# arnold117/PrimeKG-RGCN-LinkPrediction

Hardware: AMD Instinct MI355X
Metric: edges/sec per RGCN layer (fwd+bwd), PrimeKG 30.9k nodes/849k edges/3 rels (higher is better)
Workload: dtype f32; 1 GPU; C2: PrimeKG-shaped synthetic graph, 30926 nodes / 849456 edge columns / 3 relations, encoder 64->128->128, 2 layers fwd+bwd, full graph per step, dropout 0; parallelism=1 GPU, launch=hipGraph replay

## Files before the change

include/rgcn_hip.h:

```cpp
#ifndef RGCN_HIP_H
#define RGCN_HIP_H

#include <stddef.h>
#include <stdint.h>

#ifdef __cplusplus
extern "C" {
#endif

#define RGCN_ABI_VERSION 38

enum {
  RGCN_OK = 0,
  RGCN_ERR_ARG = -1,
  RGCN_ERR_RANGE = -2,
  RGCN_ERR_HIP = -3,
  RGCN_ERR_UNSUPPORTED = -4,
  RGCN_ERR_WORKSPACE = -5,
  RGCN_ERR_ALIGN = -6
};

int rgcn_abi_version(void);
const char* rgcn_strerror(int code);

typedef struct rgcn_graph rgcn_graph;

int rgcn_graph_create(const int64_t* edge_index, const int64_t* edge_type, int64_t num_edges,
                      int64_t num_nodes, int64_t num_relations, void* stream,
                      rgcn_graph** out);
int rgcn_graph_create_bipartite(const int64_t* key_node, const int64_t* other_node,
                                const int64_t* edge_type, int64_t num_edges, int64_t num_key_nodes,
                                int64_t num_other_nodes, int64_t num_relations,
                                const float* edge_weight, void* stream, rgcn_graph** out);
void rgcn_graph_destroy(rgcn_graph* g);

int64_t rgcn_graph_num_edges(const rgcn_graph* g);
int64_t rgcn_graph_num_nodes(const rgcn_graph* g);
int64_t rgcn_graph_num_relations(const rgcn_graph* g);
float rgcn_graph_weight_bound(const rgcn_graph* g, int transposed);
int rgcn_graph_num_levels(const rgcn_graph* g, int transposed);

const uint32_t* rgcn_graph_tile_mask(const rgcn_graph* g, int transposed, int64_t* num_row_tiles);

int rgcn_graph_arrays(const rgcn_graph* g, int transposed, const int32_t** rowptr,
                      const int32_t** col, const int64_t** perm, const float** val);
int rgcn_graph_export(const rgcn_graph* g, int transposed, int32_t* rowptr, int32_t* col,
                      int64_t* perm, float* val, void* stream);

int rgcn_graph_import(int64_t num_edges, int64_t num_nodes, int64_t num_relations,
                      const int32_t* rowptr, const int32_t* col, const int64_t* perm, const float* cnt,
                      const int32_t* rowptr_t, const int32_t* col_t, const int64_t* perm_t,
                      const float* w_t, void* stream, rgcn_graph** out);

typedef struct rgcn_slab_job {
  const float* slab;
  const float* bias_part;
  int32_t splits, K1, Kc, N;
  float* grad_weight;
  float* grad_root;
  float* grad_bias;
} rgcn_slab_job;

#define RGCN_AMAX_FLOATS 2048
size_t rgcn_aggregate_workspace_bytes(const rgcn_graph* g, int transposed, int64_t d);
int rgcn_aggregate_deferrable(const rgcn_graph* g, int transposed, int64_t d);
int rgcn_aggregate(const rgcn_graph* g, int transposed, const float* x, int64_t d, float* agg,
                   void* workspace, size_t workspace_bytes, void* stream);
int rgcn_aggregate_ex(const rgcn_graph* g, int transposed, const void* x, int x_f16, int64_t d, float* agg,
                      void* workspace, size_t workspace_bytes, int first_level, int last_level ,
                      const rgcn_slab_job* job , float* amax , void* stream);

int rgcn_transform_fwd(const float* agg, const float* x, const float* weight, const float* root,
                       const float* bias, int relu, const uint32_t* tile_mask, int64_t num_nodes,
                       int64_t num_relations, int64_t d_in, int64_t d_out, float* out, void* stream);

size_t rgcn_transform_fwd_f16_workspace_bytes(int64_t num_relations, int64_t d_in, int64_t d_out);
int rgcn_transform_fwd_f16(const float* agg, const float* x, const float* weight, const float* root,
                           const float* bias, int relu, const uint32_t* tile_mask, int64_t num_nodes,
                           int64_t num_relations, int64_t d_in, int64_t d_out, float* out,
                           void* workspace, size_t workspace_bytes, void* stream);

int rgcn_transform_bwd_input(const float* gagg, const float* g, const float* weight,
                             const float* root, const float* relu_mask, const uint32_t* tile_mask,
                             int64_t num_nodes, int64_t num_relations, int64_t d_in, int64_t d_out,
                             float* grad_x, void* stream);

size_t rgcn_transform_bwd_params_workspace_bytes(int64_t num_nodes, int64_t num_relations,
                                                 int64_t d_in, int64_t d_out);
int rgcn_transform_bwd_params(const float* agg, const float* x, const float* g,
                              const uint32_t* tile_mask, int64_t num_nodes, int64_t num_relations,
                              int64_t d_in, int64_t d_out, float* grad_weight, float* grad_root,
                              float* grad_bias, void* workspace, size_t workspace_bytes, void* stream);

int rgcn_transform_bwd_params_begin(const float* agg, const float* x, const float* g,
                                    const uint32_t* tile_mask, int64_t num_nodes, int64_t num_relations,
                                    int64_t d_in, int64_t d_out, float* grad_weight, float* grad_root,
                                    float* grad_bias, void* workspace, size_t workspace_bytes, void* stream,
                                    rgcn_slab_job* job);
int rgcn_slab_reduce(const rgcn_slab_job* job, void* stream);

int rgcn_absmax(const float* x, int64_t n, float* out, float* zero_buffers, int zero_count, void* stream);
int rgcn_absmax_multi(int count, const float* const* tensors, const int64_t* numels, float* const* outs,
                      float* zero_buffers, int zero_count, void* stream);
size_t rgcn_weights_split_bytes(int64_t num_relations, int64_t d_in, int64_t d_out);
int rgcn_weights_split_pack(const float* weight, const float* root, int64_t num_relations, int64_t d_in,
                            int64_t d_out, void* packed, size_t packed_bytes, void* stream);
int rgcn_weights_split_pack_multi(int count, const float* const* weights, const float* const* roots,
                                  const int64_t* num_relations, const int64_t* d_in, const int64_t* d_out,
                                  const float* const* w_amax, const float* const* r_amax, void* const* packed,
                                  const size_t* packed_bytes, float* zero_buffers, int zero_count, void* stream);
int rgcn_absmax_pack(const float* x, int64_t numel, float* x_amax, float* zero_buffers, int zero_count, int count,
                     const float* const* weights, const float* const* roots, const int64_t* num_relations,
                     const int64_t* d_in, const int64_t* d_out, void* const* packed, const size_t* packed_bytes,
                     void* stream);
size_t rgcn_transform_split_workspace_bytes(int64_t num_relations, int64_t d_in, int64_t d_out);
int rgcn_transform_fwd_split(const float* agg, const float* x, const float* weight, const float* root,
// ... 145 lines not shown
```

primekg_rgcn_linkprediction_amd/_lib.py:

```python
from __future__ import annotations

import ctypes
import os
from ctypes import c_double, c_float, POINTER, c_char_p, c_int, c_int64, c_size_t, c_void_p

import torch

ABI_VERSION = 38
LIB_NAME = "librgcn_hip.so"
LIB_PATH = os.path.join(os.path.dirname(os.path.abspath(__file__)), LIB_NAME)

RGCN_OK = 0
RGCN_ERR_ARG = -1
RGCN_ERR_RANGE = -2
RGCN_ERR_HIP = -3
RGCN_ERR_UNSUPPORTED = -4
RGCN_ERR_WORKSPACE = -5
RGCN_ERR_ALIGN = -6

_P = c_void_p
_I64 = c_int64

class SlabJob(ctypes.Structure):
    _fields_ = [("slab", c_void_p), ("bias_part", c_void_p), ("splits", ctypes.c_int32), ("K1", ctypes.c_int32),
# ... 131 lines not shown
    "rgcn_kmeans_update": (c_int, [_P, _I64, _I64, _P, _I64, _I64,
                                   _P, _P, _P, _P, _P, _P, c_float, _P, c_size_t, _P]),
    "rgcn_kmeans_inertia": (c_int, [_P, _I64, _I64, _P, _I64, _I64, _P, _P, _P, c_size_t, _P]),
    "rgcn_silhouette_workspace_bytes": (c_size_t, [_I64, _I64, _I64, _I64]),
    "rgcn_silhouette_samples": (c_int, [_P, _P, _P, _P, _P, _P, _I64, _I64, _I64, _I64, _I64, _P, _P, _P, c_size_t, _P]),
}

TSNE_PROTOTYPES = {
    "rgcn_knn_refine": (c_int, [_P, _I64, _I64, _P, _I64, _P, _P, _P]),
    "rgcn_tsne_affinities": (c_int, [_P, _I64, _I64, c_double, _P, _P, _P]),
    "rgcn_tsne_workspace_bytes": (c_size_t, [_I64, _I64]),
    "rgcn_tsne_gradient": (c_int, [_P, _I64, _P, _P, _P, _I64, c_float, _I64, c_int,
                                   _P, _P, _P, _P, c_size_t, _P]),
    "rgcn_tsne_update": (c_int, [_P, _I64, c_float, c_float, c_float, _P, _P, _P, _P, _P, c_size_t, _P]),
}

NEIGHBORHOOD_PROTOTYPES = {
    "rgcn_neighborhood_max_nodes": (_I64, []),
    "rgcn_pair_neighborhood": (c_int, [_P, _P, _P, _P, _I64, _I64,
                                       _P, _P, _I64, c_int,
                                       _P, c_int, c_int,
                                       _P, _P, _P, _P, _P, _P, _P, _P]),
}

TRANSE_PROTOTYPES = {
    "rgcn_transe_step_workspace_bytes": (c_size_t, [_I64, _I64, _I64]),
    "rgcn_transe_step": (c_int, [_P, _I64, _P, _I64, _I64,
                                 _P, _P, _P, _I64, c_float, c_float,
                                 _P, _P, _P, _P, c_size_t, _P]),
}

RESAMPLE_PROTOTYPES = {
    "rgcn_resample_weights": (c_int, [_I64, _I64, _I64, _P, _P]),
    "rgcn_resample_curves": (c_int, [_P, _P, _P, _I64, _I64, _I64, _I64, _I64,
                                     _P, _P, _P, _P, _P, _P, _P]),
    "rgcn_resample_ranks": (c_int, [_P, _P, _I64, _P, c_int, _I64, _I64, _I64,
                                    _P, _P, _P, _P, _P]),
}
RESAMPLE_TILE = 1024
RESAMPLE_MAX_SAMPLES = 1 << 28
RESAMPLE_MAX_REPLICATES = 65535
RESAMPLE_MAX_K = 8

COMPLEX_PROTOTYPES = {
    "complex_fwd": (c_int, [_P, _P, _I64, _P, _P, _I64, _P, _P, _I64, _I64, _I64, _P, _P]),
    "complex_bce_fwd": (c_int, [_P, _P, _I64, _P, _P, _I64, _P, _P, _I64, _P, _I64, _I64, _P, _P, _P]),
    "complex_bwd_workspace_bytes": (c_size_t, [_I64, _I64, _I64]),
    "complex_bwd": (c_int, [_P, _P, _P, _I64, _P, _P, _I64, _P, _P, _I64, _I64, _I64, _P, _P, _P, _P, c_size_t, c_int, _P]),
    "complex_bce_bwd": (c_int, [_P, _P, _P, _P, _P, _I64, _P, _P, _I64, _P, _P, _I64, _I64, _I64, _P, _P, _P, _P,
                                c_size_t, c_int, _P]),
    "rgcn_complex_query": (c_int, [c_int, _P, _P, _I64, _P, _P, _I64, _I64, _I64, _P, _P]),
}

_lib = None


class RGCNLibraryError(RuntimeError):
    """The HIP library is missing / unloadable / of the wrong ABI."""


def load() -> ctypes.CDLL:
    global _lib
    if _lib is not None:
        return _lib
    if not os.path.exists(LIB_PATH):
        raise RGCNLibraryError(
            f"{LIB_PATH} not found: build it with `python -c 'import __graft_entry__ as g; "
            f"g.build()'` (or `make -C primekg_rgcn_linkprediction_amd/csrc`). There is no "
            f"CPU/PyTorch fallback for the R-GCN path.")
    try:
        lib = ctypes.CDLL(LIB_PATH, mode=ctypes.RTLD_GLOBAL)
    except OSError as exc:
        raise RGCNLibraryError(f"cannot load {LIB_PATH}: {exc}") from exc
    for name, (restype, argtypes) in list(PROTOTYPES.items()) + list(SAMPLING_PROTOTYPES.items()) + list(PATHS_PROTOTYPES.items()) + list(CLUSTER_PROTOTYPES.items()) + list(TSNE_PROTOTYPES.items()) + list(NEIGHBORHOOD_PROTOTYPES.items()) + list(TRANSE_PROTOTYPES.items()) + list(RESAMPLE_PROTOTYPES.items()) + list(COMPLEX_PROTOTYPES.items()):
        try:
            fn = getattr(lib, name)
        except AttributeError as exc:
            raise RGCNLibraryError(f"{LIB_PATH} does not export {name}") from exc
        fn.restype = restype
        fn.argtypes = argtypes
    got = lib.rgcn_abi_version()
    if got != ABI_VERSION:
        raise RGCNLibraryError(f"{LIB_PATH} has ABI version {got}, host code expects {ABI_VERSION}")
    _lib = lib
    return lib


def available() -> bool:
    try:
        load()
        return True
    except RGCNLibraryError:
        return False


def strerror(code: int) -> str:
    return load().rgcn_strerror(code).decode()


def check(code: int, what: str) -> None:
    if code == RGCN_OK:
        return
    msg = f"{what}: {strerror(code)} (code {code})"
    if code == RGCN_ERR_RANGE:
        raise IndexError(msg)
    if code in (RGCN_ERR_ARG, RGCN_ERR_UNSUPPORTED):
        raise ValueError(msg)
    if code == RGCN_ERR_ALIGN:
        raise ValueError(f"{what}: a tensor's base address is not aligned: {strerror(code)} (code {code}). Every tensor "
                         f"torch allocates qualifies, and so do row slices of a table whose width is a multiple of 4; a "
                         f"view that starts some elements into a flat buffer does not - pass tensor.clone()")
    raise RuntimeError(msg)
```

primekg_rgcn_linkprediction_amd/conv.py:

```python
from __future__ import annotations

import math
from typing import Optional, Tuple, Union

import torch
import torch.nn as nn
from torch import Tensor

from . import ops


def _glorot(t: Optional[Tensor]) -> None:
    if t is not None:
        bound = math.sqrt(6.0 / (t.size(-2) + t.size(-1)))
        t.data.uniform_(-bound, bound)


def _table(x: Tensor, gather_dtype) -> Tensor:
    if gather_dtype in (None, torch.float32):
        return x
    ops.guard_torch_op("fp16 copy of the feature table")
    return x.to(gather_dtype)


# ... 5 lines not shown
        ctx.save_for_backward(comp, basis)
        return ops.basis_compose(comp, basis)

    @staticmethod
    def backward(ctx, gw: Tensor):
        comp, basis = ctx.saved_tensors
        return ops.basis_compose_bwd(gw.contiguous(), comp, basis, ctx.needs_input_grad[0], ctx.needs_input_grad[1])


class _Scales:

    def __init__(self, t: Tensor, slots: int = 2, layers=(), given=None):
        self._own, self._next, self.first = None, 0, None
        self.packed = [None] * len(layers)
        if ops.GEMM_PRECISION == "split":
            if given is not None:
                self.first = given[0]
                if slots > 1:
                    self._own = ops._empty(slots - 1, ops.AMAX_FLOATS, dtype=torch.float32, device=t.device)
                self.packed = ops.split_weights_many(list(layers), amax=list(given[1]), clear=self._own)
                return
            buf = ops._empty(slots, ops.AMAX_FLOATS, dtype=torch.float32, device=t.device)
            self.first, self._own = buf[0], buf[1:slots]
            if layers:
                self.packed = ops.absmax_and_split(t, self.first, self._own, list(layers))
            else:
                ops.absmax(t, self.first, self._own)

    def slot(self) -> Optional[Tensor]:
        if self._own is None:
            return None
        self._next += 1
        return self._own[self._next - 1]


import os as _os
_TRANSFORM_FIRST_RATIO = 2.0


def _fused_backward(graph, g, r, d_in, d_out, g_amax, packed, precision) -> bool:
    fused = _TRAIN_FUSED == "1" or (_TRAIN_FUSED == "auto" and g.size(0) * r * d_out * 4 >= _TRAIN_FUSED_MIN_BYTES)
    return (fused and precision is None and packed is not None and g_amax is not None and not graph.bipartite
            and ops.GEMM_PRECISION == "split" and ops.fused_bwd_supported(r, d_in, d_out))


def _from_packed(weight: Tensor, packed, precision) -> bool:
    return packed is not None and ops.GEMM_PRECISION == "split" and precision is None and weight.size(2) % 32 == 0


def _transform_first(graph: "ops.BucketedGraph", weight: Tensor, root: Optional[Tensor], packed, precision) -> bool:
    r, d_in, d_out = weight.shape
    ratio = _TRANSFORM_FIRST_RATIO if _from_packed(weight, packed, precision) else max(_TRANSFORM_FIRST_RATIO, 4.0)
    return d_out >= ratio * d_in and root is not None and not graph.bipartite


def _gagg_scale(graph: "ops.BucketedGraph", gagg_amax: Optional[Tensor], g_amax: Optional[Tensor]):
    if gagg_amax is not None:
        return (gagg_amax, g_amax), 1.0
    return (g_amax, g_amax), graph.weight_bound(True)


def _input_grad(graph: "ops.BucketedGraph", g: Tensor, weight: Tensor, root: Optional[Tensor],
                tail: Optional["ops.PendingParamGrads"] = None, g_amax: Optional[Tensor] = None,
                scales: Optional[_Scales] = None, packed: Optional["ops.SplitWeights"] = None,
                precision: Optional[str] = None, t_first: Optional[Tensor] = None, *,
                relu_mask: Optional[Tensor] = None, out_scale: float = 1.0, amax_out: Optional[Tensor] = None,
                lower=None):
    r, d_in, d_out = weight.shape
    extras = relu_mask is not None or amax_out is not None or out_scale != 1.0
    merged = (graph.merged_transposed()
              if not extras and _transform_first(graph, weight, root, packed, precision) else None)
    t = None
    if merged is not None:
        if t_first is None and _from_packed(weight, packed, precision):
            t_first = ops.transform_first(g.contiguous(), packed, g_amax)
        elif t_first is None:
            ops.guard_torch_op("weight concatenation of the transform-first input gradient")
            wcat = torch.cat([weight.reshape(r * d_in, d_out), root]).view(1, (r + 1) * d_in, d_out)
            t_first = ops.transform_bwd_input(g, g, wcat, None, amax=(g_amax, None), precision=precision)
        gx = ops.aggregate(merged, t_first.view(-1, d_in), tail=tail)
    else:
        gagg_amax = scales.slot() if scales is not None else None
        if _fused_backward(graph, g, r, d_in, d_out, g_amax, packed, precision):
            gx = ops.layer_bwd_input_fused(graph, g, packed, relu_mask, g_amax, amax_out=amax_out, tail=tail,
                                           inline_limit=_EVAL_INLINE_LIMIT, out_scale=out_scale, gagg_amax=gagg_amax)
        else:
            gagg = ops.aggregate(graph, g, transposed=True, tail=tail, amax_out=gagg_amax)
            amax, mul = _gagg_scale(graph, gagg_amax, g_amax)
            if (lower is not None and packed is not None and g_amax is not None
                    and _from_packed(lower[0], lower[2], precision) and _transform_first(graph, *lower, precision)
                    and ops.chain_supported(weight, lower[0])):
                gx, t = ops.transform_bwd_input_chain(gagg, g, weight, root, relu_mask, packed, lower[2], graph=graph,
                                                      amax=amax, amax_mul=mul, amax_out=amax_out, out_scale=out_scale)
            else:
                gx = ops.transform_bwd_input(gagg, g, weight, root, relu_mask=relu_mask, graph=graph, amax=amax,
                                             amax_mul=mul, amax_out=amax_out, packed=packed, precision=precision,
                                             out_scale=out_scale)
    return (gx, t) if lower is not None else gx


def _backward_scales(g: Tensor, layers: int) -> _Scales:
    return _Scales(g, slots=2 * layers)


def _deferred_params(graph: "ops.BucketedGraph", agg, x, g, x_amax, g_amax, has_root: bool, has_bias: bool, prec):
    return ops.transform_bwd_params(agg, x, g, graph.num_relations, want_root=has_root, want_bias=has_bias, graph=graph,
                                    defer=True, amax=(x_amax, x_amax, g_amax), precision=prec)


_TRAIN_FUSED = _os.environ.get("RGCN_TRAIN_FUSED", "auto")
_TRAIN_FUSED_MIN_BYTES = 256 << 20


def _defer_hubs(half: bool, packed, amax, k: int, n_out: int) -> bool:
    return (_DEFER_HUBS and not half and packed is not None and amax is not None and ops.GEMM_PRECISION == "split"
            and k in (64, 128) and n_out <= 128)


_DEFER_HUBS = True


def _train_fused(graph, n, r, d_in, d_out, half) -> bool:
    fused = _TRAIN_FUSED == "1" or (_TRAIN_FUSED == "auto" and n * r * d_in * 4 >= _TRAIN_FUSED_MIN_BYTES)
    return bool(fused and not half and not graph.weighted_shard and n == graph.num_other_nodes
                and ops.GEMM_PRECISION == "split" and ops.fused_supported(r, d_in, d_out))


def _layer_train_forward(graph: "ops.BucketedGraph", x: Tensor, gather_dtype, weight, root, bias, relu: bool,
                         half: bool, x_amax, amax_out, packed):
    n, r, d_in, d_out = x.size(0), graph.num_relations, x.size(1), weight.size(2)
    if (_train_fused(graph, n, r, d_in, d_out, half) and packed is not None and x_amax is not None):
        agg = ops._empty(n, r * d_in, dtype=torch.float32, device=x.device)
        out = ops.layer_fwd_fused(graph, x, packed, bias, relu, x_amax, amax_out, inline_limit=_EVAL_INLINE_LIMIT,
                                  agg_out=agg)
        return agg, out
    if _defer_hubs(half, packed, x_amax, d_in, d_out):
        agg, hubs = ops.aggregate_deferred(graph, x)
    else:
        agg, hubs = ops.aggregate(graph, _table(x, gather_dtype)), None
    out = ops.transform_fwd(agg, x, weight, root, bias, relu=relu, graph=graph, half=half, amax=(x_amax, x_amax),
                            amax_out=amax_out, packed=packed, hubs=hubs)
    return agg, out


def _packs(bufs, layers):
    return [ops.SplitWeights(b, w, root) if b is not None else None for b, (w, root) in zip(bufs, layers)]


def _conv_forward(x, weight, root, bias, *, graph, relu, gather_dtype, half):
    scales = _Scales(x, slots=1, layers=[(weight, root)])
    x_amax = scales.first
    packed = scales.packed[0]
    agg, out = _layer_train_forward(graph, x, gather_dtype, weight, root, bias, relu, half, x_amax, None,
                                    packed)
    return out, agg, x_amax, (packed.buf if packed is not None else None)


def _conv_backward(x, agg, weight, root, x_amax, pkbuf, g, *, graph, has_root, has_bias, need_x, need_p, prec):
    packed = _packs([pkbuf], [(weight, root)])[0]
    scales = _backward_scales(g, 1)
    pending = _deferred_params(graph, agg, x, g, x_amax, scales.first, has_root, has_bias, prec) if need_p else None
    gx = _input_grad(graph, g, weight, root, pending, scales.first, scales, packed, prec) if need_x else None
    if pending is None:
        return gx, None, None, None
    pending.finish()
    return (gx, *pending.grads)


_R_CONV_FORWARD = ops.Region("conv.forward", _conv_forward)
_R_CONV_BACKWARD = ops.Region("conv.backward", _conv_backward)


def _contiguous(*tensors):
    return tuple(t.contiguous() if t is not None else None for t in tensors)


def _bwd_precision(gather_dtype, half_backward: bool) -> Optional[str]:
    return "half" if (gather_dtype == torch.float16 and half_backward and ops.GEMM_PRECISION == "split") else None


class _RGCNConvFunction(torch.autograd.Function):

    @staticmethod
    def forward(ctx, x: Tensor, weight: Tensor, root: Optional[Tensor], bias: Optional[Tensor],
                graph: ops.BucketedGraph, relu: bool = False, gather_dtype=None, half_backward: bool = False) -> Tensor:
        x, weight, root, bias = _contiguous(x, weight, root, bias)
        ctx.bwd_precision = _bwd_precision(gather_dtype, half_backward)
        key = (tuple(x.shape), tuple(weight.shape), root is not None, bias is not None, gather_dtype, bool(relu),
               _policy_key())
        out, agg, x_amax, pkbuf = _R_CONV_FORWARD.run(graph, key, (x, weight, root, bias),
                                                      dict(graph=graph, relu=relu, gather_dtype=gather_dtype,
                                                           half=gather_dtype == torch.float16), want={0})
        ctx.graph, ctx.relu, ctx.key = graph, relu, key
        ctx.has_root, ctx.has_bias = root is not None, bias is not None
        ctx.save_for_backward(x, weight, root, out if relu else None)
        ctx.kept = (agg, x_amax, pkbuf)
        return out

    @staticmethod
    def backward(ctx, g: Tensor):
        x, weight, root, out = ctx.saved_tensors
        agg, x_amax, pkbuf = ctx.kept
        if ctx.relu:
            g = g * (out > 0)
        g = g.contiguous()
        need_x, need_w, need_root, need_bias = ctx.needs_input_grad[:4]
        need_p = bool(need_w or (need_root and ctx.has_root) or (need_bias and ctx.has_bias))
        static = dict(graph=ctx.graph, has_root=ctx.has_root, has_bias=ctx.has_bias, need_x=bool(need_x), need_p=need_p,
                      prec=ctx.bwd_precision)
        gx, gw, groot, gbias = _R_CONV_BACKWARD.run(ctx.graph, (ctx.key, bool(need_x), need_p, ctx.bwd_precision),
                                                    (x, agg, weight, root, x_amax, pkbuf, g), static,
                                                    want={0, 1, 2, 3})
        return gx, gw, groot, gbias, None, None, None, None


def _enc2_layer1(x, w1, root1, b1, w2, root2, xa=None, w1a=None, r1a=None, w2a=None, r2a=None, *, graph, gather_dtype, half):
    given = (xa, [(w1a, r1a), (w2a, r2a)]) if xa is not None else None
    scales = _Scales(x, layers=[(w1, root1), (w2, root2)], given=given)
    x_amax, h_amax = scales.first, scales.slot()
    pk1, pk2 = scales.packed
    agg1, h = _layer_train_forward(graph, x, gather_dtype, w1, root1, b1, True, half, x_amax, h_amax, pk1)
    return h, agg1, x_amax, h_amax, (pk1.buf if pk1 is not None else None), (pk2.buf if pk2 is not None else None)


def _enc2_layer2(h, w2, root2, b2, h_amax, pk2buf, *, graph, gather_dtype, half):
    pk2 = _packs([pk2buf], [(w2, root2)])[0]
    agg2, out = _layer_train_forward(graph, h, gather_dtype, w2, root2, b2, False, half, h_amax, None, pk2)
    return out, agg2


def _enc2_forward(x, w1, root1, b1, w2, root2, b2, xa=None, w1a=None, r1a=None, w2a=None, r2a=None, *, graph, gather_dtype,
                  half):
    h, agg1, x_amax, h_amax, pk1buf, pk2buf = _enc2_layer1(x, w1, root1, b1, w2, root2, xa, w1a, r1a, w2a, r2a, graph=graph,
                                                           gather_dtype=gather_dtype, half=half)
    out, agg2 = _enc2_layer2(h, w2, root2, b2, h_amax, pk2buf, graph=graph, gather_dtype=gather_dtype, half=half)
    return out, h, agg1, agg2, x_amax, h_amax, pk1buf, pk2buf


def _enc2_backward(x, agg1, h, agg2, w1, root1, w2, root2, x_amax, h_amax, pk1buf, pk2buf, g, *, graph, flags, p,
                   prec, need_x):
    has_root1, has_b1, has_root2, has_b2 = flags
    pk1, pk2 = _packs([pk1buf, pk2buf], [(w1, root1), (w2, root2)])
    scales = _backward_scales(g, 2)
    g_amax, gz_amax = scales.first, scales.slot()
    red2 = _deferred_params(graph, agg2, h, g, h_amax, g_amax, has_root2, has_b2, prec)
    gz = _input_grad(graph, g, w2, root2, red2, g_amax, scales, pk2, prec, relu_mask=h,
                     out_scale=1.0 / (1.0 - p) if p > 0 else 1.0, amax_out=gz_amax,
                     lower=(w1, root1, pk1) if need_x else None)
    gz, t_first = gz if need_x else (gz, None)
    red1 = _deferred_params(graph, agg1, x, gz, x_amax, gz_amax, has_root1, has_b1, prec)
    gx = _input_grad(graph, gz, w1, root1, red1, gz_amax, scales, pk1, prec, t_first) if need_x else None
    red2.finish()
    red1.finish()
    return (gx, *red1.grads, *red2.grads)


_R_LAYER1 = ops.Region("encoder2.layer1", _enc2_layer1)
_R_LAYER2 = ops.Region("encoder2.layer2", _enc2_layer2)
_R_FORWARD = ops.Region("encoder2.forward", _enc2_forward)
_R_BACKWARD = ops.Region("encoder2.backward", _enc2_backward)


def _policy_key():
    return (_TRAIN_FUSED, _DEFER_HUBS, _TRANSFORM_FIRST_RATIO, _EVAL_INLINE_LIMIT, _TRAIN_FUSED_MIN_BYTES)


def _enc2_train_forward(graph, params, gather_dtype, half_backward: bool, hints, p: float = 0.0):
    x, w1, root1, b1, w2, root2, b2 = params = _contiguous(*params)
    hinted = hints is not None and ops.GEMM_PRECISION == "split"
    hint_list = list(hints) if hinted else []
    key = (tuple(x.shape), tuple(w1.shape), tuple(w2.shape), root1 is not None, b1 is not None, root2 is not None,
           b2 is not None, gather_dtype, hinted, _policy_key())
    static = dict(graph=graph, gather_dtype=gather_dtype, half=gather_dtype == torch.float16)
    if p > 0:
        h, agg1, x_amax, h_amax, pk1buf, pk2buf = _R_LAYER1.run(graph, key, [x, w1, root1, b1, w2, root2] + hint_list,
                                                                static, want={0, 3})
        h = torch.native_dropout(h, p, True)[0]
        h_amax = ops.materialize(h_amax) * (1.0 / (1.0 - p)) if h_amax is not None else None
        out, agg2 = _R_LAYER2.run(graph, key, (h, w2, root2, b2, h_amax, pk2buf), static, want={0})
    else:
        out, h, agg1, agg2, x_amax, h_amax, pk1buf, pk2buf = _R_FORWARD.run(graph, key, list(params) + hint_list, static,
                                                                            want={0})
    flags = (root1 is not None, b1 is not None, root2 is not None, b2 is not None)
    kept = (agg1, h, agg2, x_amax, h_amax, pk1buf, pk2buf)
    return out, params, (graph, key, flags, p, _bwd_precision(gather_dtype, half_backward), kept)


def _enc2_train_backward(state, inputs, g: Tensor, need_x: bool):
    graph, key, flags, p, prec, (agg1, h, agg2, x_amax, h_amax, pk1buf, pk2buf) = state
    x, w1, root1, w2, root2 = inputs
    return _R_BACKWARD.run(graph, (key, p, need_x, prec),
                           (x, agg1, h, agg2, w1, root1, w2, root2, x_amax, h_amax, pk1buf, pk2buf, g.contiguous()),
                           dict(graph=graph, flags=flags, p=p, prec=prec, need_x=need_x), want={0, 1, 2, 3, 4, 5, 6})


class _Encoder2Function(torch.autograd.Function):

    @staticmethod
    def forward(ctx, x, w1, root1, b1, w2, root2, b2, graph, gather_dtype=None, p: float = 0.0,
                half_backward: bool = False, hints=None):
        out, (x, w1, root1, _, w2, root2, _), ctx.state = _enc2_train_forward(
            graph, (x, w1, root1, b1, w2, root2, b2), gather_dtype, half_backward, hints, p)
        ctx.save_for_backward(x, w1, root1, w2, root2)
        return out

    @staticmethod
    def backward(ctx, g):
        grads = _enc2_train_backward(ctx.state, ctx.saved_tensors, g, bool(ctx.needs_input_grad[0]))
        return (*grads, None, None, None, None, None)


_EVAL_BLOCK_BYTES = 1 << 30


_EVAL_FUSED = _os.environ.get("RGCN_EVAL_FUSED", "auto")


# ... 210 lines not shown
```

primekg_rgcn_linkprediction_amd/csrc/rgcn_aggregate.hip:

```cpp
#include <algorithm>
#include <cstdlib>
#include <type_traits>

#include <hip/hip_fp16.h>

#include "rgcn_common.h"
#include "rgcn_slab_reduce.h"
#include "rgcn_hub_finish.h"

namespace {

constexpr int kThreads = 256;
constexpr int kUnroll = RGCN_HEAD;
#ifndef RGCN_REDUCE_UNROLL
#define RGCN_REDUCE_UNROLL 16
#endif
#ifndef RGCN_ZERO_ROWS
#define RGCN_ZERO_ROWS 64
#endif

__device__ inline float4 f4zero() { return make_float4(0.f, 0.f, 0.f, 0.f); }
__device__ inline float f4amax(const float4& a) { return fmaxf(fmaxf(fabsf(a.x), fabsf(a.y)), fmaxf(fabsf(a.z), fabsf(a.w))); }

__device__ inline void f4add(float4& a, const float4& b) { a.x += b.x; a.y += b.y; a.z += b.z; a.w += b.w; }
// ... 254 lines not shown
      for (int u = 0; u < kUnroll; ++u) {
        v[u] = make_uint4(0u, 0u, 0u, 0u);
        if (idx[u] >= 0) v[u] = *reinterpret_cast<const uint4*>(src + (size_t)idx[u] * d + c8);
      }
#pragma unroll
      for (int u = 0; u < kUnroll; ++u) {
        const int en = e + kUnroll + u;
        const bool ok = en < it.end;
        idx_n[u] = ok ? col[en] : -1;
        wt_n[u] = (WEIGHTED && ok) ? w[en] : 0.f;
      }
      accumulate(v, wt);
    }
  }
  if (has_packs) {
    red[2 * threadIdx.x] = make_float4(acc[0], acc[1], acc[2], acc[3]);
    red[2 * threadIdx.x + 1] = make_float4(acc[4], acc[5], acc[6], acc[7]);
    __syncthreads();
    if (it.flags & (RGCN_ITEM_MEMBER | RGCN_ITEM_SKIP)) return;
    const int followers = (it.flags >> RGCN_ITEM_FOLLOW_SHIFT) & (RGCN_PACK - 1);
    for (int f = 1; f <= followers; ++f) {
      const float4 a = red[2 * (threadIdx.x + f * G)], b = red[2 * (threadIdx.x + f * G) + 1];
      acc[0] += a.x; acc[1] += a.y; acc[2] += a.z; acc[3] += a.w;
      acc[4] += b.x; acc[5] += b.y; acc[6] += b.z; acc[7] += b.w;
    }
  }
  if (!live) return;
  float* out = (it.flags & RGCN_ITEM_FINAL) ? agg : partial;
  if ((it.flags & RGCN_ITEM_FINAL) && cnt) {
    const float c = cnt[it.dst];
#pragma unroll
    for (int k = 0; k < 8; ++k) acc[k] /= c;
  }
  float4* o4 = reinterpret_cast<float4*>(out + (size_t)it.dst * d + c8);
  o4[0] = make_float4(acc[0], acc[1], acc[2], acc[3]);
  o4[1] = make_float4(acc[4], acc[5], acc[6], acc[7]);
}

template <int G>
__global__ __launch_bounds__(kThreads) void k_reduce_partials(const rgcn_item* __restrict__ items,
                                                              const float* __restrict__ cnt,
                                                              float* __restrict__ agg, float* partial, int d,
                                                              unsigned* __restrict__ amax_out) {
  __shared__ float4 red[kThreads];
  const float lmax = rgcn_reduce_item<G>(items[blockIdx.x], cnt, agg, partial, d, (int)blockIdx.y * G, red);
  if (amax_out && (int)threadIdx.x < G && (((int)threadIdx.x + (int)blockIdx.y * G) * 4 < d) &&
      (items[blockIdx.x].flags & RGCN_ITEM_FINAL))
    rgcn_amax_publish(amax_out, lmax);
}

template <int G>
void launch_level(const rgcn_csr* c, int level, bool weighted, const float* x, const float* cnt, float* agg,
                  float* partial, int d, hipStream_t stream, const rgcn_slab_job* tail = nullptr,
                  unsigned* amax_out = nullptr) {
  const int64_t nitems = c->num_items[level];
  if (nitems == 0) return;
  const unsigned gy = (unsigned)ceil_div64(d, 4 * G);
  if (level == 0) {
    const int64_t slots = kThreads / G;
    const int64_t walked = gy == 1 ? std::min(nitems, ceil_div64(nitems - c->empty_items0, slots) * slots) : nitems;
    const unsigned gather_blocks = (unsigned)ceil_div64(walked, slots);
    const unsigned zero_blocks = (unsigned)ceil_div64(nitems - walked, zero_rows<G>());
    const rgcn_slab_job job = tail ? *tail : rgcn_slab_job{};
    dim3 grid(gather_blocks + zero_blocks + (tail ? (unsigned)rgcn_slab_reduce_blocks(job) : 0u), gy);
    if (weighted)
      k_aggregate<G, true><<<grid, kThreads, 0, stream>>>(x, c->items[0], nitems, c->col, c->val, cnt, agg, partial, d,
                                                          c->head_col, c->head_w, job, (int)gather_blocks,
                                                          (int)zero_blocks, amax_out);
    else
      k_aggregate<G, false><<<grid, kThreads, 0, stream>>>(x, c->items[0], nitems, c->col, nullptr, cnt, agg, partial, d,
                                                           c->head_col, nullptr, job, (int)gather_blocks,
                                                           (int)zero_blocks, amax_out);
  } else {
    dim3 grid((unsigned)nitems, gy);
    k_reduce_partials<G><<<grid, kThreads, 0, stream>>>(c->items[level], cnt, agg, partial, d, amax_out);
  }
}

template <int G>
void launch_level0_h(const rgcn_csr* c, bool weighted, const __half* x, const float* cnt, float* agg, float* partial,
                     int d, hipStream_t stream) {
  const int64_t nitems = c->num_items[0];
  if (nitems == 0) return;
  dim3 grid((unsigned)ceil_div64(nitems, kThreads / G), (unsigned)ceil_div64(d, 8 * G));
  if (weighted)
    k_aggregate_h<G, true><<<grid, kThreads, 0, stream>>>(x, c->items[0], nitems, c->col, c->val, cnt, agg, partial, d,
                                                            c->head_col, c->head_w);
  else
    k_aggregate_h<G, false><<<grid, kThreads, 0, stream>>>(x, c->items[0], nitems, c->col, nullptr, cnt, agg, partial, d,
                                                             c->head_col, nullptr);
}

int aggregate_levels(const rgcn_graph* g, int transposed, int first, int last, const float* x, int64_t d,
                     float* agg, void* workspace, size_t workspace_bytes, void* stream_, bool half_in,
                     const rgcn_slab_job* tail, float* amax) {
  if (!g) return RGCN_ERR_ARG;
  const rgcn_csr* c = &g->dir[transposed ? 1 : 0];
  hipStream_t stream = (hipStream_t)stream_;
  if (!tail || !tail->slab) tail = nullptr;
  if (tail && (!tail->grad_weight || tail->splits <= 0 || tail->Kc <= 0 || tail->N <= 0 || (tail->N & 3)))
    return RGCN_ERR_ARG;
  if (tail && c->rowptr && c->n_key == 0) {
    RGCN_ALIGN_TRY(16, tail->slab, tail->bias_part, tail->grad_weight, tail->grad_root, tail->grad_bias);
    k_slab_reduce<<<(unsigned)rgcn_slab_reduce_blocks(*tail), 256, 0, stream>>>(*tail);
    RGCN_HIP_TRY(hipGetLastError());
    return RGCN_OK;
  }
  if (!agg || d <= 0 || (d & 3) || (half_in && (d & 7))) return RGCN_ERR_ARG;
  if (!c->rowptr) return RGCN_ERR_ARG;
  if (c->n_key == 0) return RGCN_OK;
  if (!x) return RGCN_ERR_ARG;
  if (d > (1 << 20)) return RGCN_ERR_UNSUPPORTED;
  if (first < 0 || last > c->num_levels || first > last) return RGCN_ERR_ARG;
  if (c->num_partials > 0 &&
      (!workspace || workspace_bytes < (size_t)c->num_partials * (size_t)d * sizeof(float)))
    return RGCN_ERR_WORKSPACE;
  float* partial = (float*)workspace;
  unsigned* amax_out = reinterpret_cast<unsigned*>(amax);
  if (amax && half_in) return RGCN_ERR_UNSUPPORTED;
  RGCN_ALIGN_TRY(16, x, agg, workspace);
  RGCN_ALIGN_TRY(4, amax);
  if (tail) RGCN_ALIGN_TRY(16, tail->slab, tail->bias_part, tail->grad_weight, tail->grad_root, tail->grad_bias);
  const float* cnt = c->weighted ? nullptr : c->val;
  const bool weighted = c->weighted;
  const int q = (int)(d / 4);
  const bool can_ride = !half_in && first == 0 && last > 0 && d <= 256 && c->num_items[0] > 0;
  if (tail && !can_ride) {
    k_slab_reduce<<<(unsigned)rgcn_slab_reduce_blocks(*tail), 256, 0, stream>>>(*tail);
    tail = nullptr;
  }
  for (int l = first; l < last; ++l) {
    const rgcn_slab_job* t0 = l == 0 ? tail : nullptr;
    if (l == 0 && half_in) {
      const __half* xh = reinterpret_cast<const __half*>(x);
      const int q8 = (int)(d / 8);
      if (q8 <= 1) launch_level0_h<1>(c, weighted, xh, cnt, agg, partial, (int)d, stream);
      else if (q8 <= 2) launch_level0_h<2>(c, weighted, xh, cnt, agg, partial, (int)d, stream);
      else if (q8 <= 4) launch_level0_h<4>(c, weighted, xh, cnt, agg, partial, (int)d, stream);
      else if (q8 <= 8) launch_level0_h<8>(c, weighted, xh, cnt, agg, partial, (int)d, stream);
      else if (q8 <= 16) launch_level0_h<16>(c, weighted, xh, cnt, agg, partial, (int)d, stream);
      else if (q8 <= 32) launch_level0_h<32>(c, weighted, xh, cnt, agg, partial, (int)d, stream);
      else launch_level0_h<64>(c, weighted, xh, cnt, agg, partial, (int)d, stream);
      continue;
    }
    if (q <= 1) launch_level<1>(c, l, weighted, x, cnt, agg, partial, (int)d, stream, t0, amax_out);
    else if (q <= 2) launch_level<2>(c, l, weighted, x, cnt, agg, partial, (int)d, stream, t0, amax_out);
    else if (q <= 4) launch_level<4>(c, l, weighted, x, cnt, agg, partial, (int)d, stream, t0, amax_out);
    else if (q <= 8) launch_level<8>(c, l, weighted, x, cnt, agg, partial, (int)d, stream, t0, amax_out);
    else if (q <= 16) launch_level<16>(c, l, weighted, x, cnt, agg, partial, (int)d, stream, t0, amax_out);
    else if (q <= 32) launch_level<32>(c, l, weighted, x, cnt, agg, partial, (int)d, stream, t0, amax_out);
    else launch_level<64>(c, l, weighted, x, cnt, agg, partial, (int)d, stream, t0, amax_out);
  }
  RGCN_HIP_TRY(hipGetLastError());
  return RGCN_OK;
}

}

extern "C" {

size_t rgcn_aggregate_workspace_bytes(const rgcn_graph* g, int transposed, int64_t d) {
  if (!g || d <= 0) return 0;
  return (size_t)g->dir[transposed ? 1 : 0].num_partials * (size_t)d * sizeof(float);
}

int rgcn_aggregate_ex(const rgcn_graph* g, int transposed, const void* x, int x_f16, int64_t d, float* agg,
                      void* workspace, size_t workspace_bytes, int first_level, int last_level, const rgcn_slab_job* job,
                      float* amax, void* stream) {
  if (!g) return RGCN_ERR_ARG;
  return aggregate_levels(g, transposed, first_level, last_level < 0 ? g->dir[transposed ? 1 : 0].num_levels : last_level,
                          reinterpret_cast<const float*>(x), d, agg, workspace, workspace_bytes, stream, x_f16 != 0, job,
                          amax);
}

int rgcn_aggregate(const rgcn_graph* g, int transposed, const float* x, int64_t d, float* agg,
                   void* workspace, size_t workspace_bytes, void* stream) {
  return rgcn_aggregate_ex(g, transposed, x, 0, d, agg, workspace, workspace_bytes, 0, -1, nullptr, nullptr, stream);
}

int rgcn_aggregate_deferrable(const rgcn_graph* g, int transposed, int64_t d) {
  if (!g) return 0;
  const rgcn_csr& c = g->dir[transposed ? 1 : 0];
  return (c.num_levels == 2 && c.fin_ptr && (d == 64 || d == 128 || d == 256)) ? 1 : 0;
}

}
```

primekg_rgcn_linkprediction_amd/csrc/rgcn_common.h:

```cpp
#pragma once
#include <hip/hip_runtime.h>
#include <stddef.h>
#include <stdint.h>
#include "../../include/rgcn_hip.h"
#include "rgcn_plan.h"

#define RGCN_HIP_TRY(expr)                       \
  do {                                           \
    hipError_t err__ = (expr);                   \
    if (err__ != hipSuccess) return RGCN_ERR_HIP; \
  } while (0)

template <class... P>
static inline bool rgcn_aligned(uintptr_t a, P... p) {
  uintptr_t bits = 0;
  ((bits |= (uintptr_t)(const void*)p), ...);
  return (bits & (a - 1)) == 0;
}
#define RGCN_ALIGN_TRY(a, ...)                                       \
  do {                                                               \
    if (!rgcn_aligned((a), __VA_ARGS__)) return RGCN_ERR_ALIGN;      \
  } while (0)

constexpr int kCUs = 256;
// ... 6 lines not shown
static inline rgcn_slicing rgcn_slice_tiles(int64_t tiles, int64_t want, int64_t cap) {
  const int64_t most = tiles < cap ? tiles : cap;
  want = want < most ? want : most;
  want = want > 1 ? want : 1;
  const int64_t per = (tiles + want - 1) / want;
  return {(int)per, (int)((tiles + per - 1) / per)};
}

template <class K>
static inline int raise_lds(K kernel, int bytes, bool (&raised)[64]) {
  int dev = 0;
  RGCN_HIP_TRY(hipGetDevice(&dev));
  if (dev < 0 || dev >= 64 || !raised[dev]) {
    RGCN_HIP_TRY(hipFuncSetAttribute(reinterpret_cast<const void*>(kernel), hipFuncAttributeMaxDynamicSharedMemorySize, bytes));
    if (dev >= 0 && dev < 64) raised[dev] = true;
  }
  return RGCN_OK;
}

static inline int rgcn_zero_param_grads(float* grad_weight, float* grad_root, float* grad_bias, int64_t R, int64_t d_in,
                                        int64_t d_out, hipStream_t stream) {
  RGCN_HIP_TRY(hipMemsetAsync(grad_weight, 0, (size_t)(R * d_in) * d_out * sizeof(float), stream));
  if (grad_root) RGCN_HIP_TRY(hipMemsetAsync(grad_root, 0, (size_t)d_in * d_out * sizeof(float), stream));
  if (grad_bias) RGCN_HIP_TRY(hipMemsetAsync(grad_bias, 0, (size_t)d_out * sizeof(float), stream));
  return RGCN_OK;
}

constexpr int RGCN_HEAD = 8;

struct rgcn_csr {
  int32_t* rowptr = nullptr;
  int32_t* col = nullptr;
  int64_t* perm = nullptr;
  float* val = nullptr;
  bool weighted = false;
  int64_t n_key = 0;
  int64_t n_other = 0;
  int num_levels = 0;
  int32_t empty_items0 = 0;
  rgcn_item* items[RGCN_MAX_LEVELS] = {};
  int64_t num_items[RGCN_MAX_LEVELS] = {};
  int64_t num_partials = 0;
  int32_t* head_col = nullptr;
  float* head_w = nullptr;
  uint32_t* tile_mask = nullptr;
  int64_t num_row_tiles = 0;
  int32_t* fin_ptr = nullptr;
  int64_t num_fin_tiles = 0;
  float weight_bound = 1.f;
};

static_assert(offsetof(rgcn_csr, items) == offsetof(rgcn_csr, num_levels) + 8, "empty_items0 sits behind num_levels");

struct rgcn_graph {
  int64_t E = 0, N = 0, R = 0;
  rgcn_csr dir[2];
};

__attribute__((visibility("hidden"))) int* rgcn_index_error_flag();

constexpr int RGCN_AMAX_SLOTS = 64, RGCN_AMAX_STRIDE = 32;
constexpr int RGCN_AMAX_HEADS = 256, RGCN_AMAX_HEAD_STRIDE = 8;
static_assert(RGCN_AMAX_SLOTS * RGCN_AMAX_STRIDE == RGCN_AMAX_FLOATS, "amax buffer layout (include/rgcn_hip.h)");
static_assert(RGCN_AMAX_HEADS * RGCN_AMAX_HEAD_STRIDE == RGCN_AMAX_FLOATS && RGCN_AMAX_STRIDE % RGCN_AMAX_HEAD_STRIDE == 0,
              "amax buffer layout");

#if defined(__HIPCC__)
__device__ inline int64_t clamp64(int64_t v, int64_t lo, int64_t hi) { return v < lo ? lo : (v > hi ? hi : v); }
__device__ inline int lane_int(int v, int src) { return __builtin_amdgcn_readfirstlane(__shfl(v, src)); }
__device__ inline float lane_float(float v, int src) { return __int_as_float(lane_int(__float_as_int(v), src)); }
__device__ inline int64_t lane_i64(int64_t v, int src) {
  const unsigned lo = (unsigned)lane_int((int)(unsigned)(v & 0xffffffffll), src);
  const int hi = lane_int((int)(v >> 32), src);
  return ((int64_t)hi << 32) | (int64_t)lo;
}
__device__ inline float rgcn_relu(float v) {
  const float r = fmaxf(v, 0.f);
  return v != v ? v : r;
}
extern "C" __device__ unsigned __ockl_wfred_max_u32(unsigned);
__device__ inline unsigned rgcn_amax_peek(const unsigned* __restrict__ amax) {
  return amax ? amax[(blockIdx.x & (RGCN_AMAX_SLOTS - 1)) * RGCN_AMAX_STRIDE] : 0u;
}
__device__ inline void rgcn_amax_publish(unsigned* __restrict__ amax, float lane_max, unsigned seen = 0u) {
  const unsigned m = __ockl_wfred_max_u32(__float_as_uint(fmaxf(lane_max, 0.f)));
  if (m <= seen) return;
  unsigned* slot = amax + (blockIdx.x & (RGCN_AMAX_SLOTS - 1)) * RGCN_AMAX_STRIDE;
  const unsigned long long act = __ballot(1);
  if ((int)(threadIdx.x & 63) == __ffsll((long long)act) - 1) atomicMax(slot, m);
}
__device__ inline float rgcn_amax_value(const float* __restrict__ amax, int lane) {
  float v[RGCN_AMAX_HEADS / 64];
#pragma unroll
  for (int j = 0; j < RGCN_AMAX_HEADS / 64; ++j) v[j] = amax[(lane + 64 * j) * RGCN_AMAX_HEAD_STRIDE];
  float m = v[0];
#pragma unroll
  for (int j = 1; j < RGCN_AMAX_HEADS / 64; ++j) m = fmaxf(m, v[j]);
#pragma unroll
  for (int o = 32; o > 0; o >>= 1) m = fmaxf(m, __shfl_xor(m, o));
  return m;
}
__device__ inline float rgcn_partials_max(const float* __restrict__ p, int count, int lane) {
  float v[4];
#pragma unroll
  for (int j = 0; j < 4; ++j) v[j] = (lane + 64 * j < count) ? p[lane + 64 * j] : 0.f;
  float m = fmaxf(fmaxf(v[0], v[1]), fmaxf(v[2], v[3]));
// ... 6 lines not shown
```

primekg_rgcn_linkprediction_amd/csrc/rgcn_graph.hip:

```cpp
#include <hipcub/hipcub.hpp>

#include <algorithm>
#include <cmath>
#include <new>
#include <vector>

#include "rgcn_common.h"

namespace {

constexpr int kThreads = 256;

__global__ void k_validate(const int64_t* __restrict__ key_node, const int64_t* __restrict__ other_node,
                           const int64_t* __restrict__ edge_type, int64_t E, int64_t n_key, int64_t n_other,
                           int64_t R, int* __restrict__ flag) {
  int64_t e = (int64_t)blockIdx.x * blockDim.x + threadIdx.x;
  if (e >= E) return;
  int64_t k = key_node[e], o = other_node[e], t = edge_type[e];
  if (k < 0 || k >= n_key || o < 0 || o >= n_other || t < 0 || t >= R) atomicOr(flag, 1);
}

__global__ void k_make_keys(const int64_t* __restrict__ key_node, const int64_t* __restrict__ edge_type,
                            int64_t E, int64_t R, uint32_t* __restrict__ keys, uint32_t* __restrict__ ids) {
  int64_t e = (int64_t)blockIdx.x * blockDim.x + threadIdx.x;
  if (e >= E) return;
  keys[e] = (uint32_t)(key_node[e] * R + edge_type[e]);
  ids[e] = (uint32_t)e;
}

__global__ void k_rowptr(const uint32_t* __restrict__ skeys, int64_t E, int64_t NR,
                         int32_t* __restrict__ rowptr) {
  int64_t e = (int64_t)blockIdx.x * blockDim.x + threadIdx.x;
  if (e > E) return;
  int64_t lo = (e == 0) ? 0 : (int64_t)skeys[e - 1] + 1;
  int64_t hi = (e == E) ? NR : (int64_t)skeys[e];
  for (int64_t k = lo; k <= hi; ++k) rowptr[k] = (int32_t)e;
}

__global__ void k_fill_edges(const int64_t* __restrict__ other_node, int64_t E,
                             const uint32_t* __restrict__ sids, int32_t* __restrict__ col,
                             int64_t* __restrict__ perm) {
  int64_t e = (int64_t)blockIdx.x * blockDim.x + threadIdx.x;
  if (e >= E) return;
  uint32_t p = sids[e];
  perm[e] = (int64_t)p;
  col[e] = (int32_t)other_node[p];
}

__global__ void k_counts(const int32_t* __restrict__ rowptr, int64_t NR, float* __restrict__ cnt) {
  int64_t s = (int64_t)blockIdx.x * blockDim.x + threadIdx.x;
  if (s >= NR) return;
  int deg = rowptr[s + 1] - rowptr[s];
  cnt[s] = (float)(deg < 1 ? 1 : deg);
}

__global__ void k_edge_weights(const uint32_t* __restrict__ skeys_t, const int32_t* __restrict__ col_t,
                               const float* __restrict__ cnt, int64_t E, int64_t R,
                               float* __restrict__ w) {
  int64_t e = (int64_t)blockIdx.x * blockDim.x + threadIdx.x;
  if (e >= E) return;
// ... 90 lines not shown
                    int64_t n_key, int64_t n_other, int64_t R, int slot, Scratch& sc, hipStream_t stream,
                    rgcn_csr* c) {
  const int64_t NR = n_key * R;
  c->n_key = n_key;
  c->n_other = n_other;
  RGCN_HIP_TRY(hipMalloc((void**)&c->rowptr, (NR + 1) * sizeof(int32_t)));
  if (E <= 0) {
    RGCN_HIP_TRY(hipMemsetAsync(c->rowptr, 0, (NR + 1) * sizeof(int32_t), stream));
    return RGCN_OK;
  }
  int end_bit = 1;
  while (end_bit < 32 && ((int64_t)1 << end_bit) < NR) ++end_bit;
  RGCN_HIP_TRY(hipMalloc((void**)&c->col, E * sizeof(int32_t)));
  RGCN_HIP_TRY(hipMalloc((void**)&c->perm, E * sizeof(int64_t)));
  k_make_keys<<<grid_for(E), kThreads, 0, stream>>>(key_node, edge_type, E, R, sc.keys, sc.ids);
  size_t tmp_bytes = 0;
  RGCN_HIP_TRY(hipcub::DeviceRadixSort::SortPairs(nullptr, tmp_bytes, sc.keys, sc.skeys[slot], sc.ids, sc.sids,
                                                   (int)E, 0, end_bit, stream));
  if (tmp_bytes > sc.sort_tmp_bytes) {
    RGCN_HIP_TRY(hipStreamSynchronize(stream));
    (void)hipFree(sc.sort_tmp);
    sc.sort_tmp = nullptr;
    RGCN_HIP_TRY(hipMalloc(&sc.sort_tmp, tmp_bytes + 256));
    sc.sort_tmp_bytes = tmp_bytes;
  }
  RGCN_HIP_TRY(hipcub::DeviceRadixSort::SortPairs(sc.sort_tmp, tmp_bytes, sc.keys, sc.skeys[slot], sc.ids, sc.sids,
                                                   (int)E, 0, end_bit, stream));
  k_rowptr<<<grid_for(E + 1), kThreads, 0, stream>>>(sc.skeys[slot], E, NR, c->rowptr);
  k_fill_edges<<<grid_for(E), kThreads, 0, stream>>>(other_node, E, sc.sids, c->col, c->perm);
  return RGCN_OK;
}

#define TRY_PLAN(expr) do { int rc__ = (expr); if (rc__ != RGCN_OK) return rc__; } while (0)

__global__ void k_item_heads(const rgcn_item* __restrict__ items, int64_t nitems, const int32_t* __restrict__ col,
                             const float* __restrict__ w, int32_t* __restrict__ head_col,
                             float* __restrict__ head_w) {
  const int64_t i = (int64_t)blockIdx.x * blockDim.x + threadIdx.x;
  if (i >= nitems * RGCN_HEAD) return;
  const rgcn_item it = items[i / RGCN_HEAD];
  const int e = it.begin + (int)(i % RGCN_HEAD);
  const bool ok = e < it.end;
  head_col[i] = ok ? col[e] : -1;
  if (head_w) head_w[i] = ok ? w[e] : 0.f;
}

int plan_structure(rgcn_csr* c, int64_t R, hipStream_t stream) {
  const int64_t NR = c->n_key * R;
  std::vector<int32_t> rp((size_t)NR + 1);
  RGCN_HIP_TRY(hipMemcpyAsync(rp.data(), c->rowptr, (NR + 1) * sizeof(int32_t), hipMemcpyDeviceToHost, stream));
  RGCN_HIP_TRY(hipStreamSynchronize(stream));
  if (R <= 32 && c->n_key > 0) {
    c->num_row_tiles = ceil_div64(c->n_key, 32);
    std::vector<uint32_t> mask((size_t)c->num_row_tiles, 0u);
    for (int64_t i = 0; i < c->n_key; ++i)
      for (int64_t r = 0; r < R; ++r)
        if (rp[i * R + r + 1] > rp[i * R + r]) mask[(size_t)(i >> 5)] |= 1u << r;
    RGCN_HIP_TRY(hipMalloc((void**)&c->tile_mask, mask.size() * sizeof(uint32_t)));
    RGCN_HIP_TRY(hipMemcpy(c->tile_mask, mask.data(), mask.size() * sizeof(uint32_t), hipMemcpyHostToDevice));
  }
  TRY_PLAN(build_plan(rp, NR, R, c));
  c->weight_bound = 1.f;
  if (c->weighted && NR > 0 && rp[(size_t)NR] > 0) {
    std::vector<float> w((size_t)rp[(size_t)NR]);
    RGCN_HIP_TRY(hipMemcpyAsync(w.data(), c->val, w.size() * sizeof(float), hipMemcpyDeviceToHost, stream));
    RGCN_HIP_TRY(hipStreamSynchronize(stream));
    double best = 0.0;
    for (int64_t s = 0; s < NR; ++s) {
      double sum = 0.0;
      for (int32_t e = rp[(size_t)s]; e < rp[(size_t)s + 1]; ++e) sum += std::fabs((double)w[(size_t)e]);
      best = std::max(best, sum);
    }
    c->weight_bound = (float)(best * (1.0 + 1e-6)) + 1e-30f;
  }
  const int64_t n0 = c->num_items[0];
  if (n0 > 0) {
    RGCN_HIP_TRY(hipMalloc((void**)&c->head_col, (size_t)n0 * RGCN_HEAD * sizeof(int32_t)));
    if (c->weighted) RGCN_HIP_TRY(hipMalloc((void**)&c->head_w, (size_t)n0 * RGCN_HEAD * sizeof(float)));
    k_item_heads<<<grid_for(n0 * RGCN_HEAD), kThreads, 0, stream>>>(c->items[0], n0, c->col,
                                                                   c->weighted ? c->val : nullptr, c->head_col,
                                                                   c->head_w);
    RGCN_HIP_TRY(hipGetLastError());
  }
  return RGCN_OK;
}

int mean_counts(rgcn_csr* c, int64_t R, hipStream_t stream) {
  const int64_t NR = c->n_key * R;
  RGCN_HIP_TRY(hipMalloc((void**)&c->val, std::max<int64_t>(NR, 1) * sizeof(float)));
  if (NR > 0) k_counts<<<grid_for(NR), kThreads, 0, stream>>>(c->rowptr, NR, c->val);
  c->weighted = false;
  return RGCN_OK;
}

#define TRY_RC(expr) do { int rc__ = (expr); if (rc__ != RGCN_OK) return rc__; } while (0)

int create_impl(const int64_t* edge_index, const int64_t* edge_type, int64_t E, int64_t N, int64_t R,
                hipStream_t stream, rgcn_graph* g) {
  g->E = E; g->N = N; g->R = R;
  const int64_t* src = edge_index;
  const int64_t* dst = edge_index + E;
  Scratch sc;
  TRY_RC(sc.alloc(E));
  TRY_RC(validate(dst, src, edge_type, E, N, N, R, sc, stream));
  TRY_RC(build_structure(dst, src, edge_type, E, N, N, R, 0, sc, stream, &g->dir[0]));
  TRY_RC(build_structure(src, dst, edge_type, E, N, N, R, 1, sc, stream, &g->dir[1]));
  TRY_RC(mean_counts(&g->dir[0], R, stream));
  g->dir[1].weighted = true;
  if (E > 0) {
    RGCN_HIP_TRY(hipMalloc((void**)&g->dir[1].val, E * sizeof(float)));
// ... 149 lines not shown
  if (num_nodes * num_relations > 0 && !cnt) return RGCN_ERR_ARG;
  if (num_edges > 0 && (!col || !perm || !col_t || !perm_t || !w_t)) return RGCN_ERR_ARG;
  if (too_big(num_nodes, num_nodes, num_relations, num_edges)) return RGCN_ERR_UNSUPPORTED;
  RGCN_ALIGN_TRY(8, perm, perm_t);
  RGCN_ALIGN_TRY(4, rowptr, col, cnt, rowptr_t, col_t, w_t);
  hipStream_t stream = (hipStream_t)stream_;
  rgcn_graph* g = new (std::nothrow) rgcn_graph();
  if (!g) return RGCN_ERR_HIP;
  g->E = num_edges; g->N = num_nodes; g->R = num_relations;
  int* flag = nullptr;
  int rc = hipMalloc((void**)&flag, sizeof(int)) == hipSuccess ? RGCN_OK : RGCN_ERR_HIP;
  if (rc == RGCN_OK)
    rc = import_csr(rowptr, col, perm, cnt, false, num_edges, num_nodes, num_relations, flag, stream, &g->dir[0]);
  if (rc == RGCN_OK)
    rc = import_csr(rowptr_t, col_t, perm_t, w_t, true, num_edges, num_nodes, num_relations, flag, stream,
                    &g->dir[1]);
  if (rc == RGCN_OK && hipStreamSynchronize(stream) != hipSuccess) rc = RGCN_ERR_HIP;
  (void)hipFree(flag);
  if (rc != RGCN_OK) {
    rgcn_graph_destroy(g);
    return rc;
  }
  *out = g;
  return RGCN_OK;
}

void rgcn_graph_destroy(rgcn_graph* g) {
  if (!g) return;
  free_csr(&g->dir[0]);
  free_csr(&g->dir[1]);
  delete g;
}

int64_t rgcn_graph_num_edges(const rgcn_graph* g) { return g ? g->E : -1; }
int64_t rgcn_graph_num_nodes(const rgcn_graph* g) { return g ? g->N : -1; }
int64_t rgcn_graph_num_relations(const rgcn_graph* g) { return g ? g->R : -1; }
float rgcn_graph_weight_bound(const rgcn_graph* g, int transposed) {
  if (!g) return 0.f;
  const rgcn_csr* c = &g->dir[transposed ? 1 : 0];
  return c->rowptr ? c->weight_bound : 0.f;
}

int rgcn_graph_num_levels(const rgcn_graph* g, int transposed) {
  return g ? g->dir[transposed ? 1 : 0].num_levels : -1;
}

const uint32_t* rgcn_graph_tile_mask(const rgcn_graph* g, int transposed, int64_t* num_row_tiles) {
  if (!g) return nullptr;
  const rgcn_csr* c = &g->dir[transposed ? 1 : 0];
  if (num_row_tiles) *num_row_tiles = c->num_row_tiles;
  return c->tile_mask;
}

int rgcn_graph_arrays(const rgcn_graph* g, int transposed, const int32_t** rowptr, const int32_t** col,
                      const int64_t** perm, const float** val) {
  if (!g) return RGCN_ERR_ARG;
  const rgcn_csr* c = &g->dir[transposed ? 1 : 0];
  if (rowptr) *rowptr = c->rowptr;
  if (col) *col = c->col;
  if (perm) *perm = c->perm;
  if (val) *val = c->val;
  return RGCN_OK;
}

int rgcn_graph_export(const rgcn_graph* g, int transposed, int32_t* rowptr, int32_t* col, int64_t* perm,
                      float* val, void* stream_) {
  if (!g) return RGCN_ERR_ARG;
  hipStream_t stream = (hipStream_t)stream_;
  const rgcn_csr* c = &g->dir[transposed ? 1 : 0];
  if (!c->rowptr) return RGCN_ERR_ARG;
  RGCN_ALIGN_TRY(8, perm);
  RGCN_ALIGN_TRY(4, rowptr, col, val);
  const size_t nr = (size_t)(c->n_key * g->R), e = (size_t)g->E;
  if (rowptr) RGCN_HIP_TRY(hipMemcpyAsync(rowptr, c->rowptr, (nr + 1) * sizeof(int32_t), hipMemcpyDeviceToDevice, stream));
  if (col && e) RGCN_HIP_TRY(hipMemcpyAsync(col, c->col, e * sizeof(int32_t), hipMemcpyDeviceToDevice, stream));
  if (perm && e) RGCN_HIP_TRY(hipMemcpyAsync(perm, c->perm, e * sizeof(int64_t), hipMemcpyDeviceToDevice, stream));
  const size_t nval = c->weighted ? e : nr;
  if (val && nval) RGCN_HIP_TRY(hipMemcpyAsync(val, c->val, nval * sizeof(float), hipMemcpyDeviceToDevice, stream));
  return RGCN_OK;
}

}
```

primekg_rgcn_linkprediction_amd/csrc/rgcn_transform_split.hip:

```cpp
#include <algorithm>
#include <cstdlib>
#include <type_traits>

#include <hip/hip_fp16.h>

#include "rgcn_common.h"
#include "rgcn_slab_reduce.h"
#include "rgcn_hub_finish.h"
#include "rgcn_split.h"
#include "rgcn_transform_host.h"

#ifdef RGCN_STAMPS
__device__ unsigned long long g_rgcn_stamps[8192 * 4];
#define RGCN_STAMP(i)                                                                                               \
  do {                                                                                                              \
    if (threadIdx.x == 0) g_rgcn_stamps[((blockIdx.y * gridDim.x + blockIdx.x) & 8191) * 4 + (i)] = __builtin_amdgcn_s_memrealtime(); \
  } while (0)
#else
#define RGCN_STAMP(i)
#endif

#include "rgcn_prep.h"


// ... 62 lines not shown
  }
  return q;
}
#define RGCN_AMAX_WAIT(a, b, c, younger)                                                                             \
  asm volatile("s_waitcnt vmcnt(%12)"                                                                                 \
               : "+v"(a.v[0]), "+v"(a.v[1]), "+v"(a.v[2]), "+v"(a.v[3]), "+v"(b.v[0]), "+v"(b.v[1]), "+v"(b.v[2]),     \
                 "+v"(b.v[3]), "+v"(c.v[0]), "+v"(c.v[1]), "+v"(c.v[2]), "+v"(c.v[3])                                  \
               : "n"(younger)                                                                                         \
               : "memory")
#define RGCN_AMAX_WAIT2(a, b, younger)                                                                                \
  asm volatile("s_waitcnt vmcnt(%8)"                                                                                  \
               : "+v"(a.v[0]), "+v"(a.v[1]), "+v"(a.v[2]), "+v"(a.v[3]), "+v"(b.v[0]), "+v"(b.v[1]), "+v"(b.v[2]),     \
                 "+v"(b.v[3])                                                                                         \
               : "n"(younger)                                                                                         \
               : "memory")
__device__ inline float amax_reduce(const amax_loads& q) {
  float m = fmaxf(fmaxf(q.v[0], q.v[1]), fmaxf(q.v[2], q.v[3]));
#pragma unroll
  for (int o = 32; o > 0; o >>= 1) m = fmaxf(m, __shfl_xor(m, o));
  return m;
}

constexpr int kPackThreads = 1024, kPackJobs = RGCN_PACK_JOBS;
using pack_job = rgcn_pack_job;
using pack_jobs = rgcn_pack_jobs;
__device__ inline void pack_body(const pack_job& J, float* red, int nblocks, int bid) {
  rgcn_pack_body<kPackThreads>(J, red, nblocks, bid);
}

__global__ __launch_bounds__(kPackThreads) void k_pack_split(const pack_jobs JJ, float* __restrict__ zero, int zero_count) {
  __shared__ float red[kPackThreads / 64];
  if (blockIdx.y == 0 && (int)threadIdx.x < zero_count)
    for (int h = (int)blockIdx.x; h < RGCN_AMAX_HEADS; h += (int)gridDim.x)
      zero[(size_t)threadIdx.x * RGCN_AMAX_FLOATS + h * RGCN_AMAX_HEAD_STRIDE] = 0.f;
  pack_body(JJ.j[blockIdx.y], red, (int)gridDim.x, (int)blockIdx.x);
}

struct hub_fin {
  const int32_t* ptr;
  const rgcn_item* items;
  const float* cnt;
  float* partial;
  int d, tiles;
};

struct nt_chain {
  const __half* Ch;
  const __half* Cl;
  const float* c_inv_scale;
  float* T;
  int N2;
};

template <int WM, int WN, int TN, int EPI, bool LO, bool CHAIN = false>
__global__ __launch_bounds__(64 * WM * WN) void k_gemm_nt_split(const float* __restrict__ A1, int K1,
                                                            const float* __restrict__ A2, int K2,
                                                            const __half* __restrict__ Bh,
                                                            const __half* __restrict__ Bl,
                                                            const float* __restrict__ b_inv_scale,
                                                            amax_ref amax1, float a1_mul, amax_ref amax2,
                                                            const float* __restrict__ bias,
                                                            const float* __restrict__ mask, float* __restrict__ C,
                                                            int M, int N, const uint32_t* __restrict__ tile_mask,
                                                            int kseg, unsigned* __restrict__ amax_out,
                                                            const hub_fin fin, float out_scale, const nt_chain chain) {
  static_assert(!CHAIN || (WM == 2 && WN == 2 && TN == 2 && LO), "the chained product is built for the 64 x 128 tile");
  constexpr int WAVES = WM * WN;
  constexpr int BM = 32 * WM, BN = 32 * TN * WN, NBUF = WM == 2 ? 3 : 4, D = NBUF - 1;
  constexpr int PARTS = LO ? 2 : 1;
  constexpr int A_BYTES = BM * BK * 4, B_BYTES = BN * BK * 2, BUF_BYTES = A_BYTES + PARTS * B_BYTES;
  constexpr int A_PW = BM / (8 * WAVES);
  constexpr int B_PW = BN / (16 * WAVES);
  constexpr int P = A_PW + PARTS * B_PW;
  static_assert(A_PW >= 1 && B_PW >= 1 && A_PW * 8 * WAVES == BM && B_PW * 16 * WAVES == BN, "tile / wave layout");
  __shared__ __attribute__((aligned(16))) char lds[NBUF * BUF_BYTES];

  const int K = K1 + K2;
  const int m0 = blockIdx.x * BM, n0 = blockIdx.y * BN;
  const int tid = threadIdx.x, lane = tid & 63;
  const int wave = __builtin_amdgcn_readfirstlane(tid >> 6);
  const int wm = wave / WN, wn = wave % WN;
  const int li = lane & 31, lh = lane >> 5;
  RGCN_STAMP(0);
  amax_loads q1 = amax_request(amax1, lane), q2 = amax_request(amax2.slots ? amax2 : amax1, lane);
  const unsigned seen = rgcn_amax_peek(amax_out);
  unsigned rel_mask = 0xffffffffu;
  if (tile_mask) {
    const int t32 = m0 >> 5;
    rel_mask = 0u;
#pragma unroll
    for (int q = 0; q < WM; ++q)
      if ((t32 + q) * 32 < M) rel_mask |= tile_mask[t32 + q];
    rel_mask = __builtin_amdgcn_readfirstlane(rel_mask);
  }
  int fin_b = 0, fin_e = 0;
  if (WAVES == 4 && fin.ptr) {
    fin_b = fin.ptr[min(m0 >> 5, fin.tiles)];
    fin_e = fin.ptr[min((m0 >> 5) + WM, fin.tiles)];
  }
  RGCN_AMAX_WAIT2(q1, q2, 0);
  const float amax1_v = amax_reduce(q1) * a1_mul;
  const float amax2_v = amax2.slots ? amax_reduce(q2) : 0.f;

  if (WAVES == 4 && fin.ptr) {
    const int jb = __builtin_amdgcn_readfirstlane(fin_b), je = __builtin_amdgcn_readfirstlane(fin_e);
    if (je > jb) {
      float4* red = reinterpret_cast<float4*>(lds);
      float* agg = const_cast<float*>(A1);
      for (int j = jb; j < je; ++j) {
        float4* scratch = red + ((j - jb) & 1) * 256;
        const rgcn_item it = fin.items[j];
        if (fin.d == 64) rgcn_reduce_item<16>(it, fin.cnt, agg, fin.partial, 64, 0, scratch);
        else if (fin.d == 128) rgcn_reduce_item<32>(it, fin.cnt, agg, fin.partial, 128, 0, scratch);
        else rgcn_reduce_item<64>(it, fin.cnt, agg, fin.partial, 256, 0, scratch);
      }
      __threadfence_block();
      asm volatile("s_waitcnt vmcnt(0)" ::: "memory");
      __syncthreads();
    }
  }

  floatx16 acc[TN];
#pragma unroll
  for (int b = 0; b < TN; ++b)
#pragma unroll
    for (int r = 0; r < 16; ++r) acc[b][r] = 0.f;

  int a_m[A_PW], a_c4[A_PW];
#pragma unroll
  for (int j = 0; j < A_PW; ++j) {
    const int row = (wave * A_PW + j) * 8 + (lane >> 3);
    a_m[j] = min(m0 + row, M - 1);
    a_c4[j] = ((lane & 7) ^ ((row >> 1) & 7)) * 4;
  }
  size_t b_off[B_PW];
#pragma unroll
  for (int j = 0; j < B_PW; ++j) {
    const int row = (wave * B_PW + j) * 16 + (lane >> 2);
    const int n = min(n0 + row, N - 1);
    const int chunk = (lane & 3) ^ ((row >> 1) & 3);
    b_off[j] = (size_t)n * K + chunk * 8;
  }

  auto stage = [&](int kt, int buf) {
    char* sA = lds + buf * BUF_BYTES;
    char* sBh = sA + A_BYTES;
    char* sBl = sBh + B_BYTES;
    const bool first = kt < K1;
    const float* abase = first ? A1 + kt : A2 + (kt - K1);
    const int lda = first ? K1 : K2;
#pragma unroll
    for (int j = 0; j < A_PW; ++j)
      glds16(abase + ((size_t)a_m[j] * lda + a_c4[j]), sA + (wave * A_PW + j) * 8 * BK * 4);
#pragma unroll
    for (int j = 0; j < B_PW; ++j) {
      glds16(Bh + kt + b_off[j], sBh + (wave * B_PW + j) * 16 * BK * 2);
      if (LO) glds16(Bl + kt + b_off[j], sBl + (wave * B_PW + j) * 16 * BK * 2);
    }
  };

  auto next_kt = [&](int kt) {
    kt += BK;
    while (kt < K1 && !((rel_mask >> (kt / kseg)) & 1u)) kt = (kt / kseg + 1) * kseg;
    return min(kt, K);
  };
  int ktq[D];
  ktq[0] = next_kt(-BK);
#pragma unroll
  for (int j = 1; j < D; ++j) ktq[j] = ktq[j - 1] < K ? next_kt(ktq[j - 1]) : K;
#pragma unroll
  for (int j = 0; j < D; ++j)
    if (ktq[j] < K) stage(ktq[j], j);

  const int ea1 = scale_exponent(amax1_v);
  const int ea2 = amax2.slots ? scale_exponent(amax2_v) : ea1;
  const float sa1 = pow2f(ea1), sa2 = pow2f(ea2);

  const int arow = wm * 32 + li;
  unsigned a_addr[2][2], b_addr[TN][2];
#pragma unroll
  for (int s = 0; s < 2; ++s) {
#pragma unroll
    for (int h = 0; h < 2; ++h)
      a_addr[s][h] = (unsigned)(arow * BK * 4 + (((4 * s + 2 * lh + h) ^ ((arow >> 1) & 7)) << 4));
#pragma unroll
    for (int b = 0; b < TN; ++b) {
      const int brow = (wn * TN + b) * 32 + li;
      b_addr[b][s] = (unsigned)(A_BYTES + brow * BK * 2 + (((2 * s + lh) ^ ((brow >> 1) & 3)) << 4));
    }
  }

  int t = 0;
  auto k_tile = [&](const float sa) {
    if (D == 3 && ktq[D - 1] < K) asm volatile("s_waitcnt vmcnt(%0)" ::"n"(2 * P) : "memory");
    else if (ktq[1] < K) asm volatile("s_waitcnt vmcnt(%0)" ::"n"(P) : "memory");
    else asm volatile("s_waitcnt vmcnt(0)" ::: "memory");
    __builtin_amdgcn_s_barrier();
    const unsigned buf = (unsigned)((t % NBUF) * BUF_BYTES);
    f32x4 fa[2][2], fh[2][TN], fl[2][TN];
#pragma unroll
    for (int s = 0; s < 2; ++s) {
      asm volatile("ds_read_b128 %0, %1" : "=v"(fa[s][0]) : "v"(a_addr[s][0] + buf));
      asm volatile("ds_read_b128 %0, %1" : "=v"(fa[s][1]) : "v"(a_addr[s][1] + buf));
#pragma unroll
      for (int b = 0; b < TN; ++b) {
        asm volatile("ds_read_b128 %0, %1" : "=v"(fh[s][b]) : "v"(b_addr[b][s] + buf));
// ... 263 lines not shown
          if (EPI == EPI_RELU) v = rgcn_relu(v);
          if (EPI == EPI_MASK) v = mask[(size_t)m * N + n] > 0.f ? v : 0.f;
          cmax = fmaxf(cmax, fabsf(v));
          C[(size_t)m * N + n] = v;
        }
      }
    }
  }
  if (amax_out) rgcn_amax_publish(amax_out, cmax, seen);
#ifdef RGCN_STAMPS
  asm volatile("s_waitcnt vmcnt(0)" ::: "memory");
#endif
  RGCN_STAMP(3);
}

constexpr int kPrepTensors = RGCN_PREP_TENSORS;
using absmax_multi_job = rgcn_absmax_multi_job;
template <int THREADS>
__device__ inline void absmax_body(const absmax_multi_job& J, float* __restrict__ zero, int zero_count, float* red,
                                   int bid, int nblocks) {
  rgcn_absmax_body<THREADS>(J, zero, zero_count, red, bid, nblocks);
}

__global__ __launch_bounds__(kPackThreads) void k_absmax_multi(const absmax_multi_job J, float* __restrict__ zero,
                                                               int zero_count) {
  __shared__ float red[kPackThreads / 64];
  absmax_body<kPackThreads>(J, zero, zero_count, red, (int)blockIdx.x, (int)gridDim.x);
}

__global__ __launch_bounds__(kPackThreads) void k_absmax_pack(const absmax_multi_job J, float* __restrict__ zero,
                                                              int zero_count, const pack_jobs JJ, int pack_blocks,
                                                              int layers) {
  __shared__ float red[kPackThreads / 64];
  const int b = (int)blockIdx.x, npack = pack_blocks * layers;
  RGCN_STAMP(0);
  if (b < npack) pack_body(JJ.j[b / pack_blocks], red, pack_blocks, b % pack_blocks);
  else absmax_body<kPackThreads>(J, zero, zero_count, red, b - npack, RGCN_AMAX_HEADS);
#ifdef RGCN_STAMPS
  if (b >= npack) { RGCN_STAMP(1); RGCN_STAMP(2); }
  asm volatile("s_waitcnt vmcnt(0)" ::: "memory");
#endif
  RGCN_STAMP(3);
}

constexpr int TN_TKC = 128;
template <bool LO>
__global__ __launch_bounds__(2 * kThreads) void k_gemm_tn_coop(const float* __restrict__ A1, int K1,
                                                               const float* __restrict__ A2, int K2,
                                                               const float* __restrict__ G, int M, int N,
                                                               int n_tiles, int rows_per_split,
                                                               amax_ref amax1, float a1_mul, amax_ref amax2, amax_ref gmax,
                                                               float* __restrict__ slab,
                                                               float* __restrict__ bias_part,
                                                               const uint32_t* __restrict__ tile_mask, int kseg) {
  constexpr int TKC = TN_TKC, RING = 3, A_FLOATS = 32 * TKC, G_FLOATS = 32 * 128;
  constexpr int SLOT_BYTES = (A_FLOATS + G_FLOATS) * 4;
  constexpr int PLANE = 4 * 128 * 16;
  constexpr int PBUF_BYTES = 4 * PLANE;
  constexpr int A_PW = 2, G_PW = 2, P = A_PW + G_PW;
  __shared__ __attribute__((aligned(16))) char lds[RING * SLOT_BYTES + 2 * PBUF_BYTES];
  const int Kc = K1 + K2;
  int bx = blockIdx.x, split = blockIdx.y;
  {
    const int gx = (int)gridDim.x, full = ((int)gridDim.y >> 3) << 3;
    const int lin = blockIdx.y * gx + blockIdx.x;
    if (lin < gx * full) {
      const int q = lin >> 3;
      bx = q % gx;
      split = (q / gx) * 8 + (lin & 7);
    }
  }
  const int kc_tile = bx / n_tiles, kc_tiles = (int)gridDim.x / n_tiles;
  const int kc0 = kc_tile * TKC, n0 = (bx % n_tiles) * 128;
  const int mbeg = split * rows_per_split;
  const int mend = min(M, mbeg + rows_per_split);
  const int tid = threadIdx.x, lane = tid & 63;
  const int wave = __builtin_amdgcn_readfirstlane(tid >> 6);
  const int wk = wave >> 1, wn = wave & 1;
  const int li = lane & 31, lh = lane >> 5;
  const bool bias_block = (bias_part != nullptr) && (kc_tile == (K2 > 0 ? kc_tiles - 1 : 0));
  const bool do_bias = bias_block && (tid < 128);
  RGCN_STAMP(0);
  amax_loads q1 = amax_request(amax1, lane), q2 = amax_request(amax2.slots ? amax2 : amax1, lane),
             qg = amax_request(gmax, lane);
  unsigned rel_bits = 0u;
  if (tile_mask != nullptr && !bias_block && kc0 + TKC <= K1)
    for (int c = kc0; c < kc0 + TKC; c += kseg) rel_bits |= 1u << (c / kseg);
  const bool sparse = rel_bits != 0u;
  auto next_mt = [&](int mt) {
    mt += 32;
    while (sparse && mt < mend && !(tile_mask[mt >> 5] & rel_bits)) mt += 32;
    return min(mt, mend + 31);
  };

  floatx16 acc[2];
#pragma unroll
  for (int b = 0; b < 2; ++b)
#pragma unroll
    for (int r = 0; r < 16; ++r) acc[b][r] = 0.f;
  float bsum = 0.f;

  const int d_row = lane >> 5, d_col = (lane & 31) * 4;
  const int acol = min(kc0 + d_col, Kc - 4);
  const bool a_first = acol < K1;
  const float* a_src = a_first ? A1 + acol : A2 + (acol - K1);
  const int lda = a_first ? K1 : K2;
  const int gcol = min(n0 + d_col, N - 4);
  auto stage = [&](int mt, int slot) {
    char* sA = lds + slot * SLOT_BYTES;
    char* sG = sA + A_FLOATS * 4;
#pragma unroll
    for (int j = 0; j < A_PW; ++j) {
      const int r0 = (wave * A_PW + j) * 2;
      const int m = min(mt + r0 + d_row, M - 1);
      glds16(a_src + (size_t)m * lda, sA + r0 * TKC * 4);
    }
#pragma unroll
    for (int j = 0; j < G_PW; ++j) {
      const int r0 = (wave * G_PW + j) * 2;
      const int m = min(mt + r0 + d_row, M - 1);
      glds16(G + (size_t)m * N + gcol, sG + r0 * 128 * 4);
    }
  };

  int cur = next_mt(mbeg - 32);
  stage(cur, 0);
  int nxt = cur < mend ? next_mt(cur) : mend;
  stage(nxt, 1);
  int aft = nxt < mend ? next_mt(nxt) : mend;
  stage(aft, 2);

  const bool conv_a = wave < 4;
  const int cp = tid & 63, mg = (tid >> 6) & 3;
  RGCN_AMAX_WAIT(q1, q2, qg, 3 * P);
  const float amax_a1 = amax_reduce(q1) * a1_mul;
  const float amax_a2 = amax2.slots ? amax_reduce(q2) : amax_a1;
  const int ea1 = scale_exponent(amax_a1), ea2 = scale_exponent(amax_a2), eg = scale_exponent(amax_reduce(qg));
  const bool cfirst = kc0 + 2 * cp < K1 || !amax2.slots;
  const float sconv = conv_a ? pow2f(cfirst ? ea1 : ea2) : pow2f(eg);
  const bool w_first = kc0 + wk * 32 < K1 || !amax2.slots;
  const int ea = w_first ? ea1 : ea2;

  const unsigned cv_src = (unsigned)((conv_a ? 0 : A_FLOATS * 4) + (8 * mg * 128 + 2 * cp) * 4);
  const unsigned cv_dst = (unsigned)((conv_a ? 0 : 2 * PLANE) + (mg * 128 + 2 * cp) * 16);
  const unsigned fa = (unsigned)((lh * 128 + wk * 32 + li) * 16);
  const unsigned fg = (unsigned)(2 * PLANE + (lh * 128 + wn * 64 + li) * 16);
  constexpr unsigned kPlanes = RING * SLOT_BYTES;

  auto convert = [&](int mt, int slot, int pb) {
    const unsigned src = (unsigned)(slot * SLOT_BYTES) + cv_src;
    float2v v[8];
#pragma unroll
    for (int j = 0; j < 8; ++j) asm volatile("ds_read_b64 %0, %1 offset:%2" : "=v"(v[j]) : "v"(src), "n"(j * 128 * 4));
    float bv[32];
    if (do_bias) {
      const unsigned baddr = (unsigned)(slot * SLOT_BYTES + A_FLOATS * 4) + (unsigned)tid * 4u;
#pragma unroll
      for (int mm = 0; mm < 32; ++mm) asm volatile("ds_read_b32 %0, %1 offset:%2" : "=v"(bv[mm]) : "v"(baddr), "n"(mm * 128 * 4));
    }
    asm volatile("s_waitcnt lgkmcnt(0)"
                 : "+v"(v[0]), "+v"(v[1]), "+v"(v[2]), "+v"(v[3]), "+v"(v[4]), "+v"(v[5]), "+v"(v[6]), "+v"(v[7]));
    if (do_bias) {
      asm volatile("" : "+v"(bv[0]), "+v"(bv[1]), "+v"(bv[2]), "+v"(bv[3]), "+v"(bv[4]), "+v"(bv[5]), "+v"(bv[6]), "+v"(bv[7]),
                        "+v"(bv[8]), "+v"(bv[9]), "+v"(bv[10]), "+v"(bv[11]), "+v"(bv[12]), "+v"(bv[13]), "+v"(bv[14]), "+v"(bv[15]));
      asm volatile("" : "+v"(bv[16]), "+v"(bv[17]), "+v"(bv[18]), "+v"(bv[19]), "+v"(bv[20]), "+v"(bv[21]), "+v"(bv[22]), "+v"(bv[23]),
                        "+v"(bv[24]), "+v"(bv[25]), "+v"(bv[26]), "+v"(bv[27]), "+v"(bv[28]), "+v"(bv[29]), "+v"(bv[30]), "+v"(bv[31]));
#pragma unroll
      for (int mm = 0; mm < 32; ++mm) bsum += (mt + mm < mend) ? bv[mm] : 0.f;
    }
    half8 h0, l0, h1, l1;
#pragma unroll
    for (int j = 0; j < 8; ++j) {
      const bool live = mt + 8 * mg + j < mend;
      const float x0 = live ? v[j][0] * sconv : 0.f, x1 = live ? v[j][1] * sconv : 0.f;
      const _Float16 a = (_Float16)x0, b = (_Float16)x1;
      h0[j] = a;
      h1[j] = b;
      if (LO) {
        l0[j] = (_Float16)(x0 - (float)a);
        l1[j] = (_Float16)(x1 - (float)b);
      }
    }
    const unsigned dst = kPlanes + (unsigned)(pb * PBUF_BYTES) + cv_dst;
    asm volatile("ds_write_b128 %0, %1" ::"v"(dst), "v"(__builtin_bit_cast(f32x4, h0)) : "memory");
    asm volatile("ds_write_b128 %0, %1 offset:16" ::"v"(dst), "v"(__builtin_bit_cast(f32x4, h1)) : "memory");
    if (LO) {
      asm volatile("ds_write_b128 %0, %1 offset:%2" ::"v"(dst), "v"(__builtin_bit_cast(f32x4, l0)), "n"(PLANE) : "memory");
      asm volatile("ds_write_b128 %0, %1 offset:%2" ::"v"(dst), "v"(__builtin_bit_cast(f32x4, l1)), "n"(PLANE + 16) : "memory");
    }
  };

  int t = 0;
  if (cur < mend) {
    asm volatile("s_waitcnt vmcnt(%0)" ::"n"(2 * P) : "memory");
    __builtin_amdgcn_s_barrier();
    convert(cur, 0, 0);
  }
  RGCN_STAMP(1);
  for (; cur < mend; ++t) {
    if (aft < mend) asm volatile("s_waitcnt vmcnt(%0) lgkmcnt(0)" ::"n"(P) : "memory");
    else asm volatile("s_waitcnt vmcnt(0) lgkmcnt(0)" ::: "memory");
    __builtin_amdgcn_s_barrier();
    const int fut = aft < mend ? next_mt(aft) : mend;
    if (fut < mend) stage(fut, t % RING);
    const unsigned pl = kPlanes + (unsigned)((t & 1) * PBUF_BYTES);
    f32x4 qa[2][2], qg[2][2][2];
#pragma unroll
    for (int s = 0; s < 2; ++s) {
      asm volatile("ds_read_b128 %0, %1 offset:%2" : "=v"(qa[s][0]) : "v"(pl + fa), "n"(s * 2 * 128 * 16));
      if (LO) asm volatile("ds_read_b128 %0, %1 offset:%2" : "=v"(qa[s][1]) : "v"(pl + fa), "n"(s * 2 * 128 * 16 + PLANE));
#pragma unroll
      for (int b = 0; b < 2; ++b) {
        asm volatile("ds_read_b128 %0, %1 offset:%2" : "=v"(qg[s][b][0]) : "v"(pl + fg), "n"(s * 2 * 128 * 16 + b * 32 * 16));
        if (LO) asm volatile("ds_read_b128 %0, %1 offset:%2" : "=v"(qg[s][b][1]) : "v"(pl + fg), "n"(s * 2 * 128 * 16 + b * 32 * 16 + PLANE));
      }
    }
    if (LO) {
      asm volatile("s_waitcnt lgkmcnt(0)"
                   : "+v"(qa[0][0]), "+v"(qa[0][1]), "+v"(qg[0][0][0]), "+v"(qg[0][0][1]), "+v"(qg[0][1][0]), "+v"(qg[0][1][1]),
                     "+v"(qa[1][0]), "+v"(qa[1][1]), "+v"(qg[1][0][0]), "+v"(qg[1][0][1]), "+v"(qg[1][1][0]), "+v"(qg[1][1][1]));
    } else {
      asm volatile("s_waitcnt lgkmcnt(0)"
                   : "+v"(qa[0][0]), "+v"(qg[0][0][0]), "+v"(qg[0][1][0]), "+v"(qa[1][0]), "+v"(qg[1][0][0]), "+v"(qg[1][1][0]));
    }
#pragma unroll
    for (int s = 0; s < 2; ++s) {
      const half8 ah = __builtin_bit_cast(half8, qa[s][0]);
#pragma unroll
      for (int b = 0; b < 2; ++b) {
        const half8 gh = __builtin_bit_cast(half8, qg[s][b][0]);
        if (LO) {
          const half8 al = __builtin_bit_cast(half8, qa[s][1]);
          const half8 gl = __builtin_bit_cast(half8, qg[s][b][1]);
          acc[b] = __builtin_amdgcn_mfma_f32_32x32x16_f16(al, gh, acc[b], 0, 0, 0);
          acc[b] = __builtin_amdgcn_mfma_f32_32x32x16_f16(ah, gl, acc[b], 0, 0, 0);
        }
        acc[b] = __builtin_amdgcn_mfma_f32_32x32x16_f16(ah, gh, acc[b], 0, 0, 0);
      }
    }
    if (nxt < mend) convert(nxt, (t + 1) % RING, (t + 1) & 1);
    cur = nxt;
    nxt = aft;
    aft = fut;
  }

  RGCN_STAMP(2);
  asm volatile("s_waitcnt vmcnt(0)" ::: "memory");
  const float ia = pow2f(-ea), ig = pow2f(-eg);
  float* out = slab + (size_t)split * Kc * N;
  if (kc0 + TKC <= Kc && n0 + 128 <= N) {
    __builtin_amdgcn_s_barrier();
    float* tr = reinterpret_cast<float*>(lds) + wave * (32 * 64);
#pragma unroll
    for (int b = 0; b < 2; ++b)
#pragma unroll
      for (int r = 0; r < 16; ++r) tr[((r & 3) + 8 * (r >> 2) + 4 * lh) * 64 + b * 32 + li] = acc[b][r];
    const int trow = lane >> 4, tc4 = (lane & 15) * 4;
#pragma unroll
    for (int q = 0; q < 8; ++q) {
      const float4 a = *reinterpret_cast<const float4*>(tr + (q * 4 + trow) * 64 + tc4);
      float4 v;
      v.x = a.x * ia * ig; v.y = a.y * ia * ig; v.z = a.z * ia * ig; v.w = a.w * ia * ig;
      *reinterpret_cast<float4*>(out + (size_t)(kc0 + wk * 32 + q * 4 + trow) * N + n0 + wn * 64 + tc4) = v;
    }
  } else {
#pragma unroll
    for (int b = 0; b < 2; ++b) {
      const int nn = n0 + (wn * 2 + b) * 32 + li;
      if (nn >= N) continue;
#pragma unroll
      for (int r = 0; r < 16; ++r) {
        const int kc = kc0 + wk * 32 + (r & 3) + 8 * (r >> 2) + 4 * lh;
        if (kc < Kc) out[(size_t)kc * N + nn] = acc[b][r] * ia * ig;
      }
    }
  }
  if (do_bias && n0 + tid < N) bias_part[(size_t)split * N + n0 + tid] = bsum;
#ifdef RGCN_STAMPS
  asm volatile("s_waitcnt vmcnt(0)" ::: "memory");
#endif
  RGCN_STAMP(3);
}

struct PackedWeights {
  __half *Bh_f, *Bl_f, *Bh_b, *Bl_b;
  __half *Fh_f, *Fl_f, *Fh_b, *Fl_b;
  __half *Bh_n, *Bl_n;
  float *inv_scale, *partials;
};
size_t packed_bytes(int64_t R, int64_t d_in, int64_t d_out) {
  return 10 * align256((size_t)(R + 1) * d_in * d_out * sizeof(__half)) + 256 + 2 * kMaxSlots * sizeof(float);
}
PackedWeights packed_view(void* base, int64_t R, int64_t d_in, int64_t d_out) {
  const size_t img = align256((size_t)(R + 1) * d_in * d_out * sizeof(__half));
  char* p = (char*)base;
  PackedWeights v;
// ... 3 lines not shown
  v.Bl_b = (__half*)(p + 3 * img);
  v.Fh_f = (__half*)(p + 4 * img);
  v.Fl_f = (__half*)(p + 5 * img);
  v.Fh_b = (__half*)(p + 6 * img);
  v.Fl_b = (__half*)(p + 7 * img);
  v.Bh_n = (__half*)(p + 8 * img);
  v.Bl_n = (__half*)(p + 9 * img);
  v.inv_scale = (float*)(p + 10 * img);
  v.partials = v.inv_scale + 64;
  return v;
}

pack_job make_pack_job(const float* weight, const float* root, int64_t R, int64_t d_in, int64_t d_out, void* packed,
                       const float* w_amax, const float* r_amax) {
  const PackedWeights v = packed_view(packed, R, d_in, d_out);
  pack_job j{};
  j.W = weight; j.Rt = root;
  j.R = (int)R; j.d_in = (int)d_in; j.d_out = (int)d_out;
  j.w_amax = w_amax; j.r_amax = root ? r_amax : nullptr;
  if (root && !r_amax) j.w_amax = nullptr;
  j.Bh_f = v.Bh_f; j.Bl_f = v.Bl_f; j.Bh_b = v.Bh_b; j.Bl_b = v.Bl_b;
  j.Fh_f = v.Fh_f; j.Fl_f = v.Fl_f; j.Fh_b = v.Fh_b; j.Fl_b = v.Fl_b;
  j.Bh_n = v.Bh_n; j.Bl_n = v.Bl_n;
  j.scale_out = v.inv_scale;
  return j;
}

int pack_weights(const float* weight, const float* root, int64_t R, int64_t d_in, int64_t d_out, void* packed,
                 hipStream_t stream) {
  pack_jobs JJ{};
  JJ.j[0] = make_pack_job(weight, root, R, d_in, d_out, packed, nullptr, nullptr);
  const int64_t total = (R + (root ? 1 : 0)) * d_in * d_out;
  dim3 grid((unsigned)std::min<int64_t>(64, ceil_div64(total, kPackThreads)), 1);
  k_pack_split<<<grid, kPackThreads, 0, stream>>>(JJ, nullptr, 0);
  RGCN_HIP_TRY(hipGetLastError());
  return RGCN_OK;
}

size_t nt_workspace_bytes(int64_t R, int64_t d_in, int64_t d_out) {
  return packed_bytes(R, d_in, d_out) + 2 * kMaxSlots * sizeof(float);
}

struct nt_call {
  const float *A1 = nullptr, *A2 = nullptr;
  int K1 = 0, K2 = 0;
  const __half *Bh = nullptr, *Bl = nullptr;
  const float* b_inv = nullptr;
  const float *bias = nullptr, *mask = nullptr;
  int epi = EPI_NONE;
  float* C = nullptr;
  int M = 0, N = 0;
  const uint32_t* tile_mask = nullptr;
  int kseg = 0;
  const float *a1_amax = nullptr, *a2_amax = nullptr;
  float a1_mul = 1.f, out_scale = 1.f;
  float* c_amax = nullptr;
  float* scan_slots = nullptr;
  bool half = false;
  hub_fin fin{};
  bool chained = false;
  nt_chain chain{};
  hipStream_t stream = nullptr;
  amax_ref r1{}, r2{};
};

template <int TN, int EPI, bool LO, bool CHAIN>
void nt_launch(const nt_call& c) {
  const dim3 grid((unsigned)ceil_div64(c.M, 64), CHAIN ? 1u : (unsigned)ceil_div64(c.N, 64 * TN));
  k_gemm_nt_split<2, 2, TN, EPI, LO, CHAIN><<<grid, 256, 0, c.stream>>>(
      c.A1, c.K1, c.A2, c.K2, c.Bh, c.Bl, c.b_inv, c.r1, c.a1_mul, c.r2, c.bias, c.mask, c.C, c.M, c.N, c.tile_mask, c.kseg,
      reinterpret_cast<unsigned*>(c.c_amax), c.fin, c.out_scale, CHAIN ? c.chain : nt_chain{});
}

int launch_nt_split(nt_call c) {
  const nt_chain& chain = c.chain;
  if (c.chained && (c.half || c.N != 128 || c.bias || c.epi == EPI_RELU || !chain.Ch || !chain.Cl || !chain.c_inv_scale ||
                    !chain.T || chain.N2 <= 0 || (chain.N2 & 3)))
    return RGCN_ERR_UNSUPPORTED;
  const hub_fin& fin = c.fin;
  if (fin.ptr && fin.d != 64 && fin.d != 128 && fin.d != 256) return RGCN_ERR_UNSUPPORTED;
  if (fin.ptr && (!c.a1_amax || fin.d != c.kseg)) return RGCN_ERR_ARG;
  const int K1 = c.K1, K2 = c.K2;
  if (K1 % BK || K2 % BK || K1 + K2 <= 0) return RGCN_ERR_UNSUPPORTED;
  const bool scan1 = K1 && !c.a1_amax, scan2 = K2 && !c.a2_amax;
  if (scan1 || scan2) {
    absmax_job J{};
    if (scan1) { J.p[0] = c.A1; J.n[0] = (int64_t)c.M * K1; }
    if (scan2) { J.p[1] = c.A2; J.n[1] = (int64_t)c.M * K2; }
    k_absmax<<<kMaxSlots, kThreads, 0, c.stream>>>(J, c.scan_slots);
  }
  c.r1 = !K1 ? amax_ref{nullptr, 0} : (scan1 ? amax_ref{c.scan_slots, kMaxSlots} : amax_ref{c.a1_amax, 0});
  c.r2 = !K2 ? amax_ref{nullptr, 0} : (scan2 ? amax_ref{c.scan_slots + kMaxSlots, kMaxSlots} : amax_ref{c.a2_amax, 0});
  if (scan1 || !(c.a1_mul > 0.f)) c.a1_mul = 1.f;
  if (!c.r1.slots) { c.r1 = c.r2; c.r2 = amax_ref{nullptr, 0}; c.a1_mul = 1.f; }
  if (c.kseg <= 0 || c.kseg % BK != 0) c.tile_mask = nullptr;
  auto with_epi = [&](auto launch) {
    if (c.epi == EPI_RELU) launch(std::integral_constant<int, EPI_RELU>{});
    else if (c.epi == EPI_MASK) launch(std::integral_constant<int, EPI_MASK>{});
    else launch(std::integral_constant<int, EPI_NONE>{});
  };
  auto plain = [&](auto tn) {
    with_epi([&](auto epi) {
      if (c.half) nt_launch<decltype(tn)::value, decltype(epi)::value, false, false>(c);
      else nt_launch<decltype(tn)::value, decltype(epi)::value, true, false>(c);
    });
  };
  if (c.chained)
    with_epi([&](auto epi) {
      if constexpr (decltype(epi)::value != EPI_RELU) nt_launch<2, decltype(epi)::value, true, true>(c);
    });
  else if (c.N <= 64) plain(std::integral_constant<int, 1>{});
  else plain(std::integral_constant<int, 2>{});
  RGCN_HIP_TRY(hipGetLastError());
  return RGCN_OK;
}

int make_hub_fin(const rgcn_graph* g, int transposed, float* partial, int64_t N, int64_t R, int64_t d, hub_fin* out) {
  *out = hub_fin{};
  if (!g) return 0;
  const rgcn_csr& c = g->dir[transposed ? 1 : 0];
  if (!c.rowptr || c.n_key != N || g->R != R) return RGCN_ERR_ARG;
  if (c.num_levels < 2) return 0;
  if (!c.fin_ptr || c.num_levels != 2 || !partial) return RGCN_ERR_ARG;
  out->ptr = c.fin_ptr;
  out->items = c.items[1];
  out->cnt = c.weighted ? nullptr : c.val;
  out->partial = partial;
  out->d = (int)d;
  out->tiles = (int)c.num_fin_tiles;
  return 1;
}

int nt_prepare(nt_call* c, PackedWeights* w, const float* weight, const float* root, const void* packed, int64_t N,
               int64_t R, int64_t d_in, int64_t d_out, int64_t dk, void* workspace, size_t workspace_bytes,
// ... 103 lines not shown
  if (R <= 0 || d_in <= 0 || d_out <= 0) return 0;
  return packed_bytes(R, d_in, d_out);
}

int rgcn_weights_split_pack(const float* weight, const float* root, int64_t R, int64_t d_in, int64_t d_out,
                            void* packed, size_t packed_bytes_, void* stream_) {
  const int rc = rgcn_pack_layer_check(R, d_in, d_out, 1, weight, packed, packed_bytes_, packed_bytes(R, d_in, d_out));
  if (rc != RGCN_OK) return rc;
  RGCN_ALIGN_TRY(16, weight, root, packed);
  return pack_weights(weight, root, R, d_in, d_out, packed, (hipStream_t)stream_);
}

int rgcn_weights_split_pack_multi(int count, const float* const* weights, const float* const* roots,
                                  const int64_t* R, const int64_t* d_in, const int64_t* d_out,
                                  const float* const* w_amax, const float* const* r_amax, void* const* packed,
                                  const size_t* packed_bytes_, float* zero_buffers, int zero_count, void* stream_) {
  if (count < 1 || count > kPackJobs || !weights || !roots || !R || !d_in || !d_out || !packed || !packed_bytes_)
    return RGCN_ERR_ARG;
  if (zero_count < 0 || zero_count > kPackThreads || (zero_count > 0 && !zero_buffers)) return RGCN_ERR_ARG;
  pack_jobs JJ{};
  int64_t most = 0;
  for (int l = 0; l < count; ++l) {
    const int rc = rgcn_pack_layer_check(R[l], d_in[l], d_out[l], 4, weights[l], packed[l], packed_bytes_[l],
                                         packed_bytes(R[l], d_in[l], d_out[l]));
    if (rc != RGCN_OK) return rc;
    JJ.j[l] = make_pack_job(weights[l], roots[l], R[l], d_in[l], d_out[l], packed[l], w_amax ? w_amax[l] : nullptr,
                            r_amax ? r_amax[l] : nullptr);
    most = std::max<int64_t>(most, (R[l] + (roots[l] ? 1 : 0)) * d_in[l] * d_out[l]);
  }
  for (int l = 0; l < count; ++l) {
    RGCN_ALIGN_TRY(16, weights[l], roots[l], packed[l]);
    RGCN_ALIGN_TRY(4, w_amax ? w_amax[l] : nullptr, r_amax ? r_amax[l] : nullptr);
  }
  RGCN_ALIGN_TRY(4, zero_buffers);
  dim3 grid((unsigned)std::min<int64_t>(64, ceil_div64(most, kPackThreads)), (unsigned)count);
  k_pack_split<<<grid, kPackThreads, 0, (hipStream_t)stream_>>>(JJ, zero_buffers, zero_count);
  RGCN_HIP_TRY(hipGetLastError());
  return RGCN_OK;
}

size_t rgcn_transform_split_workspace_bytes(int64_t R, int64_t d_in, int64_t d_out) {
  if (R <= 0 || d_in <= 0 || d_out <= 0) return 0;
  return nt_workspace_bytes(R, d_in, d_out);
}

int rgcn_transform_fwd_split(const float* agg, const float* x, const float* weight, const float* root,
                             const void* packed, const float* bias, int relu, const uint32_t* tile_mask, int64_t N,
                             int64_t R, int64_t d_in, int64_t d_out, const float* agg_amax, float agg_amax_mul,
                             const float* x_amax, int half, float* out, float* out_amax, void* workspace,
                             size_t workspace_bytes, void* stream_, const rgcn_graph* hub_graph, int hub_transposed,
                             float* hub_partial) {
  if (rgcn_layer_bad_dims(N, R, d_in, d_out) || !out) return RGCN_ERR_ARG;
  if (N == 0) return RGCN_OK;
  if (!agg || !x || !weight) return RGCN_ERR_ARG;
  if (d_in % BK) return RGCN_ERR_UNSUPPORTED;
  if (rgcn_gemm_out_of_range(N, (R + 1) * d_in, d_out)) return RGCN_ERR_UNSUPPORTED;
  nt_call c;
  PackedWeights v;
  const bool aligned = rgcn_aligned(16, agg, x, bias, out) && rgcn_aligned(4, tile_mask, agg_amax, x_amax, out_amax);
  const int rc = nt_prepare(&c, &v, weight, root, packed, N, R, d_in, d_out, d_in, workspace, workspace_bytes, hub_graph,
                            hub_transposed, hub_partial, stream_, aligned);
  if (rc != RGCN_OK) return rc;
  c.A1 = agg; c.a1_amax = agg_amax; c.a1_mul = agg_amax_mul; c.tile_mask = tile_mask;
  c.A2 = x; c.a2_amax = x_amax;
  c.Bh = v.Bh_f; c.Bl = v.Bl_f; c.b_inv = v.inv_scale;
  c.bias = bias; c.epi = relu ? EPI_RELU : EPI_NONE;
  c.C = out; c.N = (int)d_out; c.c_amax = out_amax;
  c.half = half != 0;
  return launch_nt_split(c);
}

int rgcn_transform_bwd_input_split(const float* gagg, const float* g, const float* weight, const float* root,
                                   const void* packed, const float* relu_mask, const uint32_t* tile_mask, int64_t N,
                                   int64_t R, int64_t d_in, int64_t d_out, const float* gagg_amax,
                                   float gagg_amax_mul, const float* g_amax, int half, float* grad_x,
                                   float* grad_x_amax, void* workspace, size_t workspace_bytes, void* stream_,
                                   const rgcn_graph* hub_graph, int hub_transposed, float* hub_partial,
                                   float out_scale) {
  if (rgcn_layer_bad_dims(N, R, d_in, d_out) || !grad_x || !(out_scale > 0.f)) return RGCN_ERR_ARG;
  if (N == 0) return RGCN_OK;
  if (!gagg || !g || !weight) return RGCN_ERR_ARG;
  if (d_out % BK) return RGCN_ERR_UNSUPPORTED;
  if (rgcn_gemm_out_of_range(N, (R + 1) * d_out, d_in)) return RGCN_ERR_UNSUPPORTED;
  nt_call c;
  PackedWeights v;
  const bool aligned = rgcn_aligned(16, gagg, g, relu_mask, grad_x) && rgcn_aligned(4, tile_mask, gagg_amax, g_amax, grad_x_amax);
  const int rc = nt_prepare(&c, &v, weight, root, packed, N, R, d_in, d_out, d_out, workspace, workspace_bytes, hub_graph,
                            hub_transposed, hub_partial, stream_, aligned);
  if (rc != RGCN_OK) return rc;
  c.A1 = gagg; c.a1_amax = gagg_amax; c.a1_mul = gagg_amax_mul; c.tile_mask = tile_mask;
  c.A2 = g; c.a2_amax = g_amax;
  c.Bh = v.Bh_b; c.Bl = v.Bl_b; c.b_inv = v.inv_scale;
  c.mask = relu_mask; c.epi = relu_mask ? EPI_MASK : EPI_NONE;
  c.C = grad_x; c.N = (int)d_in; c.c_amax = grad_x_amax; c.out_scale = out_scale;
  c.half = half != 0;
  return launch_nt_split(c);
}

int rgcn_transform_bwd_input_chain_supported(int64_t R, int64_t d_in, int64_t d_out, int64_t R1, int64_t d_in1) {
  if (R <= 0 || R1 <= 0 || d_in != 128 || d_out <= 0 || (d_out % BK) || d_in1 <= 0 || (d_in1 & 3)) return 0;
  return 1;
}

int rgcn_transform_bwd_input_chain_split(const float* gagg, const float* g, const float* weight, const float* root,
                                         const void* packed, const float* relu_mask, const uint32_t* tile_mask, int64_t N,
                                         int64_t R, int64_t d_in, int64_t d_out, const float* gagg_amax,
                                         float gagg_amax_mul, const float* g_amax, float* grad_x, float* grad_x_amax,
                                         void* workspace, size_t workspace_bytes, void* stream_,
                                         const rgcn_graph* hub_graph, int hub_transposed, float* hub_partial,
                                         float out_scale, const void* packed1, int has_root1, int64_t R1, int64_t d_in1,
                                         float* t_out) {
  if (rgcn_layer_bad_dims(N, R, d_in, d_out) || !grad_x || !t_out || !packed || !packed1 || !(out_scale > 0.f))
    return RGCN_ERR_ARG;
  if (!rgcn_transform_bwd_input_chain_supported(R, d_in, d_out, R1, d_in1)) return RGCN_ERR_UNSUPPORTED;
  if (N == 0) return RGCN_OK;
  if (!gagg || !g || !weight || !gagg_amax || !g_amax) return RGCN_ERR_ARG;
  if (rgcn_gemm_out_of_range(N, (R + 1) * d_out, (R1 + 1) * d_in1)) return RGCN_ERR_UNSUPPORTED;
  nt_call c;
  PackedWeights v;
  const bool aligned = rgcn_aligned(16, gagg, g, relu_mask, grad_x, packed1, t_out) &&
                       rgcn_aligned(4, tile_mask, gagg_amax, g_amax, grad_x_amax);
  const int rc = nt_prepare(&c, &v, weight, root, packed, N, R, d_in, d_out, d_out, workspace, workspace_bytes, hub_graph,
                            hub_transposed, hub_partial, stream_, aligned);
  if (rc != RGCN_OK) return rc;
  const PackedWeights v1 = packed_view(const_cast<void*>(packed1), R1, d_in1, d_in);
  c.A1 = gagg; c.a1_amax = gagg_amax; c.a1_mul = gagg_amax_mul; c.tile_mask = tile_mask;
  c.A2 = g; c.a2_amax = g_amax;
  c.Bh = v.Bh_b; c.Bl = v.Bl_b; c.b_inv = v.inv_scale;
  c.mask = relu_mask; c.epi = relu_mask ? EPI_MASK : EPI_NONE;
  c.C = grad_x; c.N = (int)d_in; c.c_amax = grad_x_amax; c.out_scale = out_scale;
  c.chained = true;
  c.chain = nt_chain{v1.Bh_n, v1.Bl_n, v1.inv_scale, t_out, (int)((R1 + (has_root1 ? 1 : 0)) * d_in1)};
  return launch_nt_split(c);
}

int rgcn_transform_first_split(const float* g, const void* packed, int has_root, int64_t N, int64_t R, int64_t d_in,
                               int64_t d_out, const float* g_amax, int half, float* t_out, void* workspace,
                               size_t workspace_bytes, void* stream_) {
  if (rgcn_layer_bad_dims(N, R, d_in, d_out) || !t_out || !packed) return RGCN_ERR_ARG;
  if (N == 0) return RGCN_OK;
  if (!g) return RGCN_ERR_ARG;
  if (d_out % BK) return RGCN_ERR_UNSUPPORTED;
  const int64_t cols = (R + (has_root ? 1 : 0)) * d_in;
  if (rgcn_gemm_out_of_range(N, d_out, cols)) return RGCN_ERR_UNSUPPORTED;
  if (!workspace || workspace_bytes < 2 * kMaxSlots * sizeof(float)) return RGCN_ERR_WORKSPACE;
  RGCN_ALIGN_TRY(16, g, packed, t_out, workspace);
  RGCN_ALIGN_TRY(4, g_amax);
  const PackedWeights v = packed_view(const_cast<void*>(packed), R, d_in, d_out);
  nt_call c;
  c.A1 = g; c.K1 = (int)d_out; c.a1_amax = g_amax;
  c.Bh = v.Bh_n; c.Bl = v.Bl_n; c.b_inv = v.inv_scale;
  c.C = t_out; c.M = (int)N; c.N = (int)cols;
  c.scan_slots = (float*)workspace;
  c.half = half != 0;
  c.stream = (hipStream_t)stream_;
  return launch_nt_split(c);
}

size_t rgcn_transform_bwd_params_split_workspace_bytes(int64_t N, int64_t R, int64_t d_in, int64_t d_out) {
  if (N < 0 || R <= 0 || d_in <= 0 || d_out <= 0) return 0;
  const int64_t Kc = (R + 1) * d_in;
  return tn_workspace_bytes(rgcn_slab_layout_of(rgcn_tn_plan(N, Kc, d_out, TN_TKC, kTnBlocks), Kc, d_out));
}

int rgcn_transform_bwd_params_split_begin(const float* agg, const float* x, const float* g,
                                          const uint32_t* tile_mask, int64_t N, int64_t R, int64_t d_in,
                                          int64_t d_out, const float* agg_amax, float agg_amax_mul,
                                          const float* x_amax, const float* g_amax, int half, float* grad_weight,
                                          float* grad_root,
                                          float* grad_bias, void* workspace, size_t workspace_bytes, void* stream_,
                                          rgcn_slab_job* job) {
  const int rc = rgcn_params_begin_check(job, agg, x, g, N, R, d_in, d_out, grad_weight, 64);
  if (rc != RGCN_OK) return rc;
  rgcn_tn_split p = rgcn_tn_plan(N, (R + 1) * d_in, d_out, TN_TKC, kTnBlocks);
  const rgcn_slab_layout lay = rgcn_slab_layout_of(p, (R + 1) * d_in, d_out);
  if (!workspace || workspace_bytes < tn_workspace_bytes(lay)) return RGCN_ERR_WORKSPACE;
  RGCN_ALIGN_TRY(16, agg, x, g, grad_weight, grad_root, grad_bias, workspace);
  RGCN_ALIGN_TRY(4, tile_mask, agg_amax, x_amax, g_amax);
  hipStream_t stream = (hipStream_t)stream_;
  if (N == 0) return rgcn_zero_param_grads(grad_weight, grad_root, grad_bias, R, d_in, d_out, stream);
  const int K1 = (int)(R * d_in), K2 = grad_root ? (int)d_in : 0, Kc = K1 + K2;
  p.kc_tiles = (int)ceil_div64(Kc, TN_TKC);
  float* slab = (float*)workspace;
  float* bias_part = slab + lay.slab_floats;
  float* slots = (float*)((char*)workspace + align256(lay.bytes()));
  absmax_job J{};
  const bool scan1 = !agg_amax, scan2 = K2 && !x_amax, scang = !g_amax;
  if (scan1) { J.p[0] = agg; J.n[0] = N * (int64_t)K1; }
  if (scan2) { J.p[1] = x; J.n[1] = N * (int64_t)K2; }
  if (scang) { J.p[2] = g; J.n[2] = N * d_out; }
  if (scan1 || scan2 || scang) k_absmax<<<kMaxSlots, kThreads, 0, stream>>>(J, slots);
  const amax_ref r1 = scan1 ? amax_ref{slots, kMaxSlots} : amax_ref{agg_amax, 0};
  const amax_ref r2 = !K2 ? amax_ref{nullptr, 0} : (scan2 ? amax_ref{slots + kMaxSlots, kMaxSlots} : amax_ref{x_amax, 0});
  const amax_ref rg = scang ? amax_ref{slots + 2 * kMaxSlots, kMaxSlots} : amax_ref{g_amax, 0};
  const float a1_mul = (scan1 || !(agg_amax_mul > 0.f)) ? 1.f : agg_amax_mul;
  dim3 grid((unsigned)(p.kc_tiles * p.n_tiles), (unsigned)p.splits);
  const uint32_t* tmask = (d_in % 64 == 0) ? tile_mask : nullptr;
  float* bp = grad_bias ? bias_part : nullptr;
#define RGCN_TN_LAUNCH(KERNEL, LO_)                                                                              \
  KERNEL<LO_><<<grid, 2 * kThreads, 0, stream>>>(agg, K1, x, K2, g, (int)N, (int)d_out, p.n_tiles, p.rows_per_split, \
                                                 r1, a1_mul, r2, rg, slab, bp, tmask, (int)d_in)
  if (half) RGCN_TN_LAUNCH(k_gemm_tn_coop, false);
  else RGCN_TN_LAUNCH(k_gemm_tn_coop, true);
#undef RGCN_TN_LAUNCH
  RGCN_HIP_TRY(hipGetLastError());
  rgcn_slab_job_fill(job, workspace, lay, p.splits, K1, Kc, d_out, grad_weight, grad_root, grad_bias);
  return RGCN_OK;
}

}
```

primekg_rgcn_linkprediction_amd/ops.py:

```python
from __future__ import annotations

import ctypes
import os
import pickle
import time
from collections import OrderedDict
from typing import NamedTuple, Optional, Tuple

import torch

from . import _lib


_raw_stream = getattr(torch._C, "_cuda_getCurrentRawStream", None)
_REC = None


def _empty(*shape, dtype, device) -> torch.Tensor:
    if _REC is None:
        return torch.empty(*shape, dtype=dtype, device=device)
    return _REC.alloc(shape[0] if len(shape) == 1 and isinstance(shape[0], (tuple, list, torch.Size)) else shape, dtype, device)


def _L():
# ... 380 lines not shown

    @classmethod
    def from_state(cls, state: dict, device) -> "BucketedGraph":
        if state.get("format") != cls.SIDECAR_FORMAT:
            raise ValueError(f"not a {cls.SIDECAR_FORMAT} file")
        device = torch.device(device)
        if device.type != "cuda":
            raise RuntimeError("BucketedGraph lives on an MI355X device; no CPU fallback")
        e, n, r = int(state["num_edges"]), int(state["num_nodes"]), int(state["num_relations"])
        want = {"rowptr": (torch.int32, n * r + 1), "col": (torch.int32, e), "perm": (torch.int64, e),
                "cnt": (torch.float32, n * r), "rowptr_t": (torch.int32, n * r + 1), "col_t": (torch.int32, e),
                "perm_t": (torch.int64, e), "w_t": (torch.float32, e)}
        dev = {}
        for k, (dt, size) in want.items():
            t = state[k]
            if t.dtype != dt or t.dim() != 1 or t.numel() != size:
                raise ValueError(f"{k} must be {dt}[{size}], got {t.dtype}{tuple(t.shape)}")
            dev[k] = t.to(device).contiguous()
        self = cls.__new__(cls)
        self._handle = None
        self.device = device
        self.num_nodes, self.num_relations, self.num_other_nodes, self.num_edges = n, r, n, e
        self.bipartite = self.weighted_shard = False
        handle = ctypes.c_void_p()
        with _on(device):
            rc = _L().rgcn_graph_import(e, n, r, *(_ptr(dev[k]) for k in want), _stream(),
                                               ctypes.byref(handle))
        _lib.check(rc, "rgcn_graph_import")
        self._handle = handle
        return self

    def save(self, path) -> None:
        torch.save(self.state(), path)

    @classmethod
    def load(cls, path, device) -> "BucketedGraph":
        return cls.from_state(torch.load(path, weights_only=True), device)

    @property
    def handle(self) -> ctypes.c_void_p:
        if self._handle is None:
            raise RuntimeError("BucketedGraph was destroyed")
        return self._handle

    def tile_mask_ptr(self, transposed: bool) -> Optional[int]:
        if self.bipartite and transposed:
            raise ValueError("a shard structure has one direction only (transposed=False)")
        handle = self.handle
        cache = self.__dict__.setdefault("_mask_ptrs", {})
        if transposed not in cache:
            cache[transposed] = _L().rgcn_graph_tile_mask(handle, int(transposed), None) or None
        return cache[transposed]

    def workspace_bytes(self, transposed: bool, d: int) -> int:
        handle = self.handle
        cache = self.__dict__.setdefault("_ws_bytes", {})
        key = (bool(transposed), int(d))
        if key not in cache:
            cache[key] = _L().rgcn_aggregate_workspace_bytes(handle, int(transposed), int(d))
        return cache[key]

    def num_levels(self, transposed: bool) -> int:
        handle = self.handle
        cache = self.__dict__.setdefault("_levels", {})
        if transposed not in cache:
            cache[transposed] = _L().rgcn_graph_num_levels(handle, int(transposed))
        return cache[transposed]

    def deferrable(self, transposed: bool, d: int) -> bool:
        handle = self.handle
        cache = self.__dict__.setdefault("_deferrable", {})
        key = (bool(transposed), int(d))
        if key not in cache:
            cache[key] = bool(_L().rgcn_aggregate_deferrable(handle, int(transposed), int(d)))
        return cache[key]

    def weight_bound(self, transposed: bool) -> float:
        handle = self.handle
        cache = self.__dict__.setdefault("_wbound", {})
        key = bool(transposed and not self.bipartite)
        if key not in cache:
            cache[key] = float(_L().rgcn_graph_weight_bound(handle, int(key)))
        return cache[key]

    def arrays(self, transposed: bool) -> Tuple[torch.Tensor, torch.Tensor, torch.Tensor, torch.Tensor]:
        lib = _L()
        nr, e = self.num_nodes * self.num_relations, self.num_edges
        with _on(self.device):
            rowptr = _empty(nr + 1, dtype=torch.int32, device=self.device)
            col = _empty(e, dtype=torch.int32, device=self.device)
            perm = _empty(e, dtype=torch.int64, device=self.device)
            val = _empty(e if transposed or self.weighted_shard else nr, dtype=torch.float32, device=self.device)
            rc = lib.rgcn_graph_export(self.handle, int(transposed), _ptr(rowptr), _ptr(col), _ptr(perm),
                                       _ptr(val), _stream())
        _lib.check(rc, "rgcn_graph_export")
        return rowptr, col, perm, val

    def row_blocks(self, block_rows: int):
        if self.bipartite:
            raise ValueError("row blocks are cut from a whole graph")
        block_rows = max(32, (int(block_rows) + 31) // 32 * 32)
        cache = self.__dict__.setdefault("_row_blocks", {})
        if block_rows not in cache:
            n, r = self.num_nodes, self.num_relations
            rowptr, col, _, _ = self.arrays(False)
            rp = rowptr.long()
# ... 134 lines not shown
    _GRAPH_CACHE[key] = (g, edge_index, edge_type)
    while len(_GRAPH_CACHE) > _GRAPH_CACHE_SIZE:
        _GRAPH_CACHE.popitem(last=False)
    return g


def clear_graph_cache() -> None:
    _GRAPH_CACHE.clear()


GATHER_EVENTS = None
GEMM_EVENTS = None


class _GemmBracket:

    def __new__(cls, *info):
        return _NO_GUARD if GEMM_EVENTS is None else super().__new__(cls)

    def __init__(self, kind: str, m: int, k: int, n: int, precision: str):
        self.info = (kind, m, k, n, precision)

    def __enter__(self):
        if GEMM_EVENTS is not None:
            self.beg, self.end = torch.cuda.Event(enable_timing=True), torch.cuda.Event(enable_timing=True)
            self.beg.record()
        return self

    def __exit__(self, *exc):
        if GEMM_EVENTS is not None and exc[0] is None:
            self.end.record()
            GEMM_EVENTS.append(self.info + (self.beg, self.end))
        return False


class PendingParamGrads:

    def __init__(self, grads, job, workspace):
        self.grads, self.job, self._workspace, self.done = grads, job, workspace, False

    def finish(self) -> None:
        if not self.done:
            dev = self.grads[0].device
            with _on(dev):
                rc = _L().rgcn_slab_reduce(ctypes.byref(self.job), _stream())
            _lib.check(rc, "rgcn_slab_reduce")
            self._launched()

    def _launched(self) -> None:
        self.done, self._workspace = True, None


def _gather(graph: BucketedGraph, x: torch.Tensor, transposed: bool, tail: Optional[PendingParamGrads],
            amax_out: Optional[torch.Tensor], out: Optional[torch.Tensor], levels=(0, -1)):
    half_in = isinstance(x, torch.Tensor) and x.dtype == torch.float16
    _need_gpu("x", x, torch.float16 if half_in else torch.float32)
    if graph.bipartite and transposed:
        raise ValueError("a shard structure has one direction only (transposed=False)")
    if x.dim() != 2 or x.size(0) != graph.num_other_nodes:
        raise ValueError(f"x must be [{graph.num_other_nodes}, d], got {tuple(x.shape)}")
    if x.device != graph.device:
        raise RuntimeError("x and the bucketed graph are on different devices")
    d = x.size(1)
    if d % (8 if half_in else 4):
        raise ValueError(f"feature dim {d} must be a multiple of {8 if half_in else 4}")
    _check_amax("amax_out", amax_out, x.device)
    if amax_out is not None and half_in:
        raise ValueError("amax_out goes with the fp32 gather (the fp16 path's transform needs no scale)")
    lib = _L()
    if out is not None:
        _need_gpu("out", out, torch.float32)
        if tuple(out.shape) != (graph.num_nodes, graph.num_relations * d) or out.device != x.device:
            raise ValueError(f"out must be [{graph.num_nodes}, {graph.num_relations * d}] on x's device")
    measure = GATHER_EVENTS is not None and not half_in
    with _on(x.device):
        if out is None:
            out = _empty(graph.num_nodes, graph.num_relations * d, dtype=torch.float32, device=x.device)
        nbytes = graph.workspace_bytes(transposed, d)
        ws = _workspace(nbytes, x.device)
        if measure and tail is not None:
            tail.finish()
        job = tail.job if tail is not None and not tail.done else None
        rc = 0
        for first, last in ([(l, l + 1) for l in range(graph.num_levels(transposed))] if measure else [levels]):
            if measure and first == 0:
                beg, end = torch.cuda.Event(enable_timing=True), torch.cuda.Event(enable_timing=True)
                beg.record()
            rc = rc or lib.rgcn_aggregate_ex(graph.handle, int(transposed), _ptr(x), int(half_in), d, _ptr(out), _ptr(ws),
                                             nbytes, first, last, ctypes.byref(job) if job is not None else None,
                                             _ptr(amax_out), _stream())
            if measure and first == 0:
                end.record()
                weighted = bool(transposed) or (graph.bipartite and graph.weighted_shard)
                GATHER_EVENTS.append((weighted, d, graph.num_edges, graph.num_nodes * graph.num_relations,
                                      graph.num_other_nodes, beg, end))
        if rc == 0 and job is not None:
            tail._launched()
    _lib.check(rc, "rgcn_aggregate")
    return out, ws


def aggregate(graph: BucketedGraph, x: torch.Tensor, transposed: bool = False,
              tail: Optional[PendingParamGrads] = None, amax_out: Optional[torch.Tensor] = None,
              out: Optional[torch.Tensor] = None) -> torch.Tensor:
    return _gather(graph, x, transposed, tail, amax_out, out)[0]


def fused_bwd_supported(num_relations: int, d_in: int, d_out: int) -> bool:
    return GEMM_PRECISION != "fp32" and bool(_query("rgcn_layer_bwd_input_fused_supported", int(num_relations), int(d_in), int(d_out)))


FUSED_EVENTS = None


def layer_fwd_fused(graph: BucketedGraph, x: torch.Tensor, packed: SplitWeights, bias: Optional[torch.Tensor],
                    relu: bool, amax: torch.Tensor, amax_out: Optional[torch.Tensor] = None,
                    inline_limit: int = 16, out: Optional[torch.Tensor] = None,
                    agg_out: Optional[torch.Tensor] = None) -> torch.Tensor:
    _need_gpu("x", x, torch.float32)
    if graph.weighted_shard:
        raise ValueError("the fused layer covers mean structures only")
    if x.dim() != 2 or x.size(0) != graph.num_other_nodes or x.device != graph.device:
        raise ValueError(f"x must be [{graph.num_other_nodes}, d] on the graph's device, got {tuple(x.shape)}")
    r, d_in, d_out = packed.shape
    if r != graph.num_relations or d_in != x.size(1):
        raise ValueError(f"packed weights are [{r}, {d_in}, {d_out}]; graph has {graph.num_relations} relations, x width {x.size(1)}")
    if bias is not None:
        _need_gpu("bias", bias, torch.float32)
        if tuple(bias.shape) != (d_out,):
            raise ValueError(f"bias must be [{d_out}]")
    _check_amax("amax", amax, x.device)
    if amax is None:
        raise ValueError("amax (the amax buffer of x) is required")
    _check_amax("amax_out", amax_out, x.device)
    if agg_out is not None:
        _need_gpu("agg_out", agg_out, torch.float32)
        if tuple(agg_out.shape) != (graph.num_nodes, r * d_in) or agg_out.device != x.device or not agg_out.is_contiguous():
            raise ValueError(f"agg_out must be a contiguous [{graph.num_nodes}, {r * d_in}] on x's device")
    plan = graph.fused_plan(min(int(inline_limit), d_in // 4))
    hub_agg = aggregate(plan.hub, x) if plan.hub is not None else None
    tile_mask = graph.tile_mask_ptr(False) if graph.num_relations <= 32 else None
    lib = _L()
    with _on(x.device):
        if out is None:
            out = _empty(graph.num_nodes, d_out, dtype=torch.float32, device=x.device)
        elif tuple(out.shape) != (graph.num_nodes, d_out) or out.dtype != torch.float32 or out.device != x.device:
            raise ValueError(f"out must be float32 [{graph.num_nodes}, {d_out}] on x's device")
        if FUSED_EVENTS is not None:
            beg, end = torch.cuda.Event(enable_timing=True), torch.cuda.Event(enable_timing=True)
            beg.record()
        rc = lib.rgcn_layer_fwd_fused(_ptr(plan.rowptr), _ptr(plan.col), tile_mask, graph.num_nodes, r, _ptr(hub_agg),
                                      _ptr(x), _ptr(packed.buf), int(packed.has_root), _ptr(bias),
                                      int(bool(relu)), d_in, d_out, _ptr(amax), _ptr(out), _ptr(amax_out), _ptr(agg_out),
                                      _stream())
        if FUSED_EVENTS is not None:
            end.record()
            FUSED_EVENTS.append(("fwd+store" if agg_out is not None else "fwd", graph.num_nodes, graph.num_relations,
                                 graph.num_edges - plan.hub_edges, plan.hub_rows, d_in, d_out, beg, end))
# ... 70 lines not shown
    return hubs.graph.handle, int(hubs.transposed), _ptr(hubs.partial)


def _check_layer(agg, x, weight, root, bias):
    _need_gpu("x", x, torch.float32)
    _need_gpu("agg", agg, torch.float32)
    _need_gpu("weight", weight, torch.float32)
    if weight.dim() != 3:
        raise ValueError("weight must be [R, d_in, d_out]")
    r, d_in, d_out = weight.shape
    n = x.size(0)
    if x.dim() != 2 or x.size(1) != d_in:
        raise ValueError(f"x must be [N, {d_in}], got {tuple(x.shape)}")
    if tuple(agg.shape) != (n, r * d_in):
        raise ValueError(f"agg must be [{n}, {r * d_in}], got {tuple(agg.shape)}")
    if root is not None:
        _need_gpu("root", root, torch.float32)
        if tuple(root.shape) != (d_in, d_out):
            raise ValueError(f"root must be [{d_in}, {d_out}]")
    if bias is not None:
        _need_gpu("bias", bias, torch.float32)
        if tuple(bias.shape) != (d_out,):
            raise ValueError(f"bias must be [{d_out}]")
    if d_in % 4 or d_out % 4:
        raise ValueError("in/out channels must be multiples of 4")
    return n, r, d_in, d_out


def _check_bwd_input(gagg, g, weight, root, relu_mask):
    _need_gpu("g", g, torch.float32)
    _need_gpu("gagg", gagg, torch.float32)
    _need_gpu("weight", weight, torch.float32)
    r, d_in, d_out = weight.shape
    n = g.size(0)
    if tuple(g.shape) != (n, d_out) or tuple(gagg.shape) != (n, r * d_out):
        raise ValueError("g must be [N, d_out] and gagg [N, R*d_out]")
    if root is not None:
        _need_gpu("root", root, torch.float32)
    if relu_mask is not None:
        _need_gpu("relu_mask", relu_mask, torch.float32)
        if tuple(relu_mask.shape) != (n, d_in):
            raise ValueError(f"relu_mask must be [{n}, {d_in}]")
    return n, r, d_in, d_out


def _mask_for(graph: Optional[BucketedGraph], transposed: bool, n: int, r: int) -> Optional[int]:
    if graph is None:
        return None
    if graph.num_nodes != n or graph.num_relations != r:
        raise ValueError("graph does not match the operand shapes")
    return graph.tile_mask_ptr(transposed and not graph.bipartite)


def transform_fwd(agg, x, weight, root=None, bias=None, relu: bool = False,
                  graph: Optional[BucketedGraph] = None, half: bool = False, amax=None,
                  amax_out: Optional[torch.Tensor] = None, precision: Optional[str] = None,
                  packed: Optional[SplitWeights] = None, amax_mul: float = 1.0,
                  out: Optional[torch.Tensor] = None, hubs: Optional[DeferredHubs] = None) -> torch.Tensor:
    n, r, d_in, d_out = _check_layer(agg, x, weight, root, bias)
    lib = _L()
    _check_amax("amax_out", amax_out, x.device)
    if out is not None:
        _need_gpu("out", out, torch.float32)
        if tuple(out.shape) != (n, d_out) or out.device != x.device:
            raise ValueError(f"out must be [{n}, {d_out}] on x's device")
    split = 0 if half else _use_split(precision, d_in, 32)
    if not n:
        split = 0
    if split:
        a1, a2 = _pair(amax, 2)
        _check_amax("agg_amax", a1, x.device)
        _check_amax("x_amax", a2, x.device)
        if packed is not None and not packed.matches(weight, root):
            raise ValueError("packed does not belong to these weights")
    elif hubs is not None:
        raise ValueError("deferred hub tails need the split-precision transform (finish them with aggregate instead)")
    k = (r + (root is not None)) * d_in
    with _on(x.device):
        if out is None:
            out = _empty(n, d_out, dtype=torch.float32, device=x.device)
        if split:
            name = "rgcn_transform_fwd_split"
            nbytes = _query("rgcn_transform_split_workspace_bytes", r, d_in, d_out)
            ws = _workspace(nbytes, x.device)
            with _GemmBracket("fwd", n, k, d_out, _split_label(split)):
                rc = lib.rgcn_transform_fwd_split(_ptr(agg), _ptr(x), _ptr(weight), _ptr(root),
                                                  _ptr(packed.buf) if packed is not None else None, _ptr(bias),
                                                  int(relu), _mask_for(graph, False, n, r), n, r, d_in, d_out,
                                                  _ptr(a1), float(amax_mul), _ptr(a2), int(split == 2), _ptr(out),
                                                  _ptr(amax_out), _ptr(ws), nbytes, _stream(), *_hub_args(hubs, n, r))
        elif half and d_in % 32 == 0:
            name = "rgcn_transform_fwd_f16"
            nbytes = lib.rgcn_transform_fwd_f16_workspace_bytes(r, d_in, d_out)
            ws = _workspace(nbytes, x.device)
            with _GemmBracket("fwd", n, k, d_out, "f16"):
                rc = lib.rgcn_transform_fwd_f16(_ptr(agg), _ptr(x), _ptr(weight), _ptr(root), _ptr(bias), int(relu),
                                                _mask_for(graph, False, n, r), n, r, d_in, d_out, _ptr(out), _ptr(ws),
                                                nbytes, _stream())
        else:
            name = "rgcn_transform_fwd"
            with _GemmBracket("fwd", n, k, d_out, "fp32"):
                rc = lib.rgcn_transform_fwd(_ptr(agg), _ptr(x), _ptr(weight), _ptr(root), _ptr(bias), int(relu),
                                            _mask_for(graph, False, n, r), n, r, d_in, d_out, _ptr(out), _stream())
    _lib.check(rc, name)
    if not split and amax_out is not None:
        absmax(out, amax_out)
    return out


def transform_bwd_input(gagg, g, weight, root=None, relu_mask=None,
                        graph: Optional[BucketedGraph] = None, amax=None, amax_out: Optional[torch.Tensor] = None,
                        precision: Optional[str] = None, packed: Optional[SplitWeights] = None,
                        amax_mul: float = 1.0, hubs: Optional[DeferredHubs] = None,
                        out_scale: float = 1.0) -> torch.Tensor:
    n, r, d_in, d_out = _check_bwd_input(gagg, g, weight, root, relu_mask)
    lib = _L()
    _check_amax("amax_out", amax_out, g.device)
    if d_in % 4 or d_out % 4:
        raise ValueError("in/out channels must be multiples of 4")
    split = _use_split(precision, d_out, 32)
    if split and n > 0:
        a1, a2 = _pair(amax, 2)
        _check_amax("gagg_amax", a1, g.device)
        _check_amax("g_amax", a2, g.device)
        if packed is not None and not packed.matches(weight, root):
            raise ValueError("packed does not belong to these weights")
        with _on(g.device):
            gx = _empty(n, d_in, dtype=torch.float32, device=g.device)
            nbytes = _query("rgcn_transform_split_workspace_bytes", r, d_in, d_out)
            ws = _workspace(nbytes, g.device)
            with _GemmBracket("bwd_input", n, (r + (root is not None)) * d_out, d_in, _split_label(split)):
                rc = lib.rgcn_transform_bwd_input_split(_ptr(gagg), _ptr(g), _ptr(weight), _ptr(root),
                                                        _ptr(packed.buf) if packed is not None else None,
                                                        _ptr(relu_mask), _mask_for(graph, True, n, r), n, r, d_in,
                                                        d_out, _ptr(a1), float(amax_mul), _ptr(a2), int(split == 2),
                                                        _ptr(gx), _ptr(amax_out), _ptr(ws), nbytes, _stream(),
                                                        *_hub_args(hubs, n, r), float(out_scale))
        _lib.check(rc, "rgcn_transform_bwd_input_split")
        return gx
    if hubs is not None:
        raise ValueError("deferred hub tails need the split-precision transform (finish them with aggregate instead)")
    if out_scale != 1.0:
        weight = weight * out_scale
        root = root * out_scale if root is not None else None
    with _on(g.device):
        gx = _empty(n, d_in, dtype=torch.float32, device=g.device)
        with _GemmBracket("bwd_input", n, (r + (root is not None)) * d_out, d_in, "fp32"):
            rc = lib.rgcn_transform_bwd_input(_ptr(gagg), _ptr(g), _ptr(weight), _ptr(root), _ptr(relu_mask),
                                              _mask_for(graph, True, n, r), n, r, d_in, d_out, _ptr(gx), _stream())
    _lib.check(rc, "rgcn_transform_bwd_input")
    if amax_out is not None:
        absmax(gx, amax_out)
    return gx


def chain_supported(weight: torch.Tensor, weight1: torch.Tensor) -> bool:
    r, d_in, d_out = weight.shape
    r1, d_in1, d_out1 = weight1.shape
    return bool(GEMM_PRECISION == "split" and d_out1 == d_in and
                _query("rgcn_transform_bwd_input_chain_supported", r, d_in, d_out, r1, d_in1))


def transform_bwd_input_chain(gagg, g, weight, root, relu_mask, packed: SplitWeights, packed1: SplitWeights,
                              graph: Optional[BucketedGraph] = None, amax=None, amax_out: Optional[torch.Tensor] = None,
                              amax_mul: float = 1.0, hubs: Optional[DeferredHubs] = None, out_scale: float = 1.0):
    n, r, d_in, d_out = _check_bwd_input(gagg, g, weight, root, relu_mask)
    r1, d_in1, _ = packed1.shape
    if not packed.matches(weight, root) or packed1.shape[2] != d_in:
        raise ValueError("packed / packed1 do not belong to these layers")
    a1, a2 = _pair(amax, 2)
    _check_amax("gagg_amax", a1, g.device)
    _check_amax("g_amax", a2, g.device)
    _check_amax("amax_out", amax_out, g.device)
    if a1 is None or a2 is None:
        raise ValueError("the chained transform needs the operand maxima (amax=)")
    lib = _L()
    cols = (r1 + (1 if packed1.has_root else 0)) * d_in1
    with _on(g.device):
        gz = _empty(n, d_in, dtype=torch.float32, device=g.device)
        t = _empty(n, cols, dtype=torch.float32, device=g.device)
        nbytes = _query("rgcn_transform_split_workspace_bytes", r, d_in, d_out)
        ws = _workspace(nbytes, g.device)
        with _GemmBracket("bwd_input_chain", n, (r + (root is not None)) * d_out + cols, d_in, "split"):
            rc = lib.rgcn_transform_bwd_input_chain_split(_ptr(gagg), _ptr(g), _ptr(weight), _ptr(root), _ptr(packed.buf),
                                                          _ptr(relu_mask), _mask_for(graph, True, n, r), n, r, d_in, d_out,
                                                          _ptr(a1), float(amax_mul), _ptr(a2), _ptr(gz), _ptr(amax_out), _ptr(ws),
                                                          nbytes, _stream(), *_hub_args(hubs, n, r), float(out_scale),
                                                          _ptr(packed1.buf), int(packed1.has_root), r1, d_in1, _ptr(t))
    _lib.check(rc, "rgcn_transform_bwd_input_chain_split")
    return gz, t


def transform_first(g: torch.Tensor, packed: SplitWeights, amax: Optional[torch.Tensor] = None,
                    precision: Optional[str] = None) -> torch.Tensor:
    _need_gpu("g", g, torch.float32)
    r, d_in, d_out = packed.shape
    if g.dim() != 2 or g.size(1) != d_out or not g.is_contiguous() or g.device != packed.buf.device:
        raise ValueError(f"g must be a contiguous [N, {d_out}] on the weights' device")
    split = _use_split(precision, d_out, 32)
    if not split:
        raise ValueError("transform_first runs in split precision only")
    _check_amax("amax", amax, g.device)
    lib = _L()
    n = g.size(0)
    with _on(g.device):
        t = _empty(n, (r + int(packed.has_root)) * d_in, dtype=torch.float32, device=g.device)
        ws = _workspace(2048, g.device)
        with _GemmBracket("bwd_input", n, d_out, t.size(1), _split_label(split)):
            rc = lib.rgcn_transform_first_split(_ptr(g), _ptr(packed.buf), int(packed.has_root), n, r, d_in, d_out,
                                                _ptr(amax), int(split == 2), _ptr(t), _ptr(ws), 2048, _stream())
    _lib.check(rc, "rgcn_transform_first_split")
    return t


def transform_bwd_params(agg, x, g, num_relations: int, want_root: bool = True, want_bias: bool = True,
                         graph: Optional[BucketedGraph] = None, defer: bool = False, amax=None,
                         precision: Optional[str] = None, amax_mul: float = 1.0):
    _need_gpu("x", x, torch.float32)
    _need_gpu("agg", agg, torch.float32)
    _need_gpu("g", g, torch.float32)
    n, d_in = x.shape
    d_out = g.size(1)
    r = int(num_relations)
    if tuple(agg.shape) != (n, r * d_in) or g.size(0) != n:
        raise ValueError("agg must be [N, R*d_in] and g [N, d_out]")
    lib = _L()
    with _on(x.device):
        gw = _empty(r, d_in, d_out, dtype=torch.float32, device=x.device)
        groot = _empty(d_in, d_out, dtype=torch.float32, device=x.device) if want_root else None
        gbias = _empty(d_out, dtype=torch.float32, device=x.device) if want_bias else None
        split = _use_split(precision, d_in, 64)
        if split and n > 0:
            a1, a2, a3 = _pair(amax, 3)
            for nm, t in (("agg_amax", a1), ("x_amax", a2), ("g_amax", a3)):
                _check_amax(nm, t, x.device)
            nbytes = _query("rgcn_transform_bwd_params_split_workspace_bytes", n, r, d_in, d_out)
            ws = _workspace(nbytes, x.device)
            job = _lib.SlabJob()
            with _GemmBracket("bwd_params", (r + want_root) * d_in, n, d_out, _split_label(split)):
                rc = lib.rgcn_transform_bwd_params_split_begin(_ptr(agg), _ptr(x), _ptr(g),
                                                               _mask_for(graph, False, n, r), n, r, d_in, d_out,
                                                               _ptr(a1), float(amax_mul), _ptr(a2), _ptr(a3),
                                                               int(split == 2), _ptr(gw), _ptr(groot),
                                                               _ptr(gbias), _ptr(ws), nbytes, _stream(),
                                                               ctypes.byref(job))
            _lib.check(rc, "rgcn_transform_bwd_params_split_begin")
            pending = PendingParamGrads((gw, groot, gbias), job, ws)
            if defer:
                return pending
            pending.finish()
            return gw, groot, gbias
        nbytes = lib.rgcn_transform_bwd_params_workspace_bytes(n, r, d_in, d_out)
        ws = _workspace(nbytes, x.device)
        if defer:
            job = _lib.SlabJob()
            with _GemmBracket("bwd_params", (r + want_root) * d_in, n, d_out, "fp32"):
                rc = lib.rgcn_transform_bwd_params_begin(_ptr(agg), _ptr(x), _ptr(g), _mask_for(graph, False, n, r), n,
                                                         r, d_in, d_out, _ptr(gw), _ptr(groot), _ptr(gbias), _ptr(ws),
                                                         nbytes, _stream(), ctypes.byref(job))
            _lib.check(rc, "rgcn_transform_bwd_params_begin")
            return PendingParamGrads((gw, groot, gbias), job, ws)
        rc = lib.rgcn_transform_bwd_params(_ptr(agg), _ptr(x), _ptr(g), _mask_for(graph, False, n, r), n, r, d_in,
                                           d_out, _ptr(gw),
                                           _ptr(groot), _ptr(gbias), _ptr(ws), nbytes, _stream())
    _lib.check(rc, "rgcn_transform_bwd_params")
    return gw, groot, gbias


def _check_operand(name, mat, idx, batch):
    _need_gpu(name, mat, torch.float32)
    if mat.dim() != 2:
        raise ValueError(f"{name} must be 2-D")
    if idx is not None:
        _need_gpu(name + "_idx", idx, torch.int64)
        if idx.dim() != 1 or idx.size(0) != batch:
            raise ValueError(f"{name}_idx must be [{batch}]")
    elif mat.size(0) != batch:
        raise ValueError(f"{name} must have {batch} rows when no index is given")


def distmult_fwd(h, h_idx, t, t_idx, r, r_idx, batch: int) -> torch.Tensor:
    d = h.size(1)
    for name, m, i in (("head", h, h_idx), ("tail", t, t_idx), ("rel", r, r_idx)):
        _check_operand(name, m, i, batch)
        if m.size(1) != d:
            raise ValueError("head / tail / relation embedding dims differ")
    if d % 4:
        raise ValueError("embedding dim must be a multiple of 4")
    lib = _L()
    with _on(h.device):
        scores = _empty(batch, dtype=torch.float32, device=h.device)
        rc = lib.distmult_fwd(_ptr(h), _ptr(h_idx), h.size(0), _ptr(t), _ptr(t_idx), t.size(0), _ptr(r), _ptr(r_idx),
                              r.size(0), batch, d, _ptr(scores), _stream())
    _lib.check(rc, "distmult_fwd")
    return scores

# ... 1539 lines not shown
        for last, exaggeration, momentum, patience in stages:
            first = it
            best_error, best_iter = float("inf"), first
            for i in range(first, last):
                check = (i + 1) % TSNE_CHECK_EVERY == 0
                want_error = check or i == last - 1
                tsne_gradient(y, rowptr, col, val, exaggeration, slices, want_error, grad, z, stats[0:1], ws)
                tsne_update(grad, y, update, gains, momentum, lr, 0.01, stats[1:2], ws)
                it = i + 1
                if want_error:
                    error, norm2 = stats.cpu().tolist()
                if check:
                    if error < best_error:
                        best_error, best_iter = error, i
                    elif i - best_iter > patience:
                        break
                    if norm2 ** 0.5 <= float(min_grad_norm):
                        break
        lap("iterations")
    return TSNEResult(y, float(error), it)


def distmult_score_all_tails(head: torch.Tensor, rel: torch.Tensor, rel_idx: Optional[torch.Tensor],
                             emb: torch.Tensor):
    _need_gpu("head", head, torch.float32)
    _need_gpu("rel", rel, torch.float32)
    _need_gpu("emb", emb, torch.float32)
    b, d = head.shape
    if emb.dim() != 2 or emb.size(1) != d or rel.dim() != 2 or rel.size(1) != d:
        raise ValueError("head [B, d], rel [R, d], emb [N, d] expected")
    if rel_idx is not None:
        _need_gpu("rel_idx", rel_idx, torch.int64)
        if rel_idx.shape != (b,):
            raise ValueError("rel_idx [B] expected")
    elif rel.size(0) != b:
        raise ValueError("rel must hold one row per head row when no relation ids are given")
    if d % 32:
        raise ValueError("embedding dim must be a multiple of 32 for the score kernel")
    lib = _L()
    with _on(head.device):
        hr = _empty((b, d), dtype=torch.float32, device=head.device)
        scores = _empty((b, emb.size(0)), dtype=torch.float32, device=head.device)
        rc = lib.distmult_score_all_tails(_ptr(head), _ptr(rel), _ptr(rel_idx), rel.size(0), _ptr(emb), b, emb.size(0),
                                          d, _ptr(hr), _ptr(scores), _stream())
    _lib.check(rc, "distmult_score_all_tails")
    return scores, hr


class _NotRecordable(Exception):
    pass


_SEQ_INDEX = {name: i for i, name in enumerate(_lib.SEQ_FUNCTIONS)}
_SEQ_PURE = ("rgcn_graph_tile_mask", "rgcn_graph_num_levels", "rgcn_graph_weight_bound", "rgcn_aggregate_deferrable",
             "rgcn_graph_num_edges", "rgcn_graph_num_nodes", "rgcn_graph_num_relations", "rgcn_abi_version", "rgcn_strerror")
REGIONS = True


def guard_torch_op(what: str) -> None:
    if _REC is not None:
        raise _NotRecordable(what)


def _strides(shape):
    st, acc = [], 1
    for n in reversed(shape):
        st.append(acc)
        acc *= n
    return tuple(reversed(st))


def _nbytes(shape, dtype) -> int:
    n = 1
    for s in shape:
        n *= s
    return n * torch.empty((), dtype=dtype).element_size()


class Lazy:
    __slots__ = ("arena", "offset", "shape", "dtype", "_t", "alias")

    def __init__(self, arena, offset, shape, dtype, alias=None):
        self.arena, self.offset, self.shape, self.dtype, self._t, self.alias = arena, offset, shape, dtype, None, alias

    def data_ptr(self) -> int:
        return self.arena.data_ptr() + self.offset

    def tensor(self) -> torch.Tensor:
        if self._t is None:
            if self.dtype == torch.float32 and self.alias is not None and self.offset % 4 == 0:
                self._t = torch.as_strided(self.alias, self.shape, _strides(self.shape), self.offset // 4)
            else:
                nbytes = _nbytes(self.shape, self.dtype)
                self._t = self.arena[self.offset: self.offset + nbytes].view(self.dtype).view(self.shape)
        return self._t


def materialize(t):
    return t.tensor() if isinstance(t, Lazy) else t


def _signature(t):
    if t is None:
        return None
    if isinstance(t, Lazy):
        return (t.dtype, tuple(t.shape), t.arena.get_device())
    return (t.dtype, tuple(t.shape), t.get_device())
# ... 337 lines not shown
```

Measured before the change: 6.703 billion edges/s.

## Skip zeroing empty aggregate rows and mask them per-row in split transforms

Adds a per-row relation-occupancy mask to the graph's tile-mask buffer and a sparse-rows mode bit. In that mode the aggregate stops launching the zero-fill blocks for empty rows, and the split-precision transforms (forward, backward input, chained backward, parameter gradients) are told to consult the row mask instead of reading the unwritten agg rows. The aim is to avoid the memory traffic of writing and reading zeros for empty (node, relation) slots. In exchange the agg buffer holds garbage in empty rows, so every consumer must honour the mask, which adds a correctness dependency across kernels.

```diff
diff --git a/include/rgcn_hip.h b/include/rgcn_hip.h
--- a/include/rgcn_hip.h
+++ b/include/rgcn_hip.h
@@ -62,6 +62,7 @@
 } rgcn_slab_job;
 
 #define RGCN_AMAX_FLOATS 2048
+#define RGCN_MODE_SPARSE_ROWS 2
 size_t rgcn_aggregate_workspace_bytes(const rgcn_graph* g, int transposed, int64_t d);
 int rgcn_aggregate_deferrable(const rgcn_graph* g, int transposed, int64_t d);
 int rgcn_aggregate(const rgcn_graph* g, int transposed, const float* x, int64_t d, float* agg,
diff --git a/include/rgcn_sparse.h b/include/rgcn_sparse.h
--- /dev/null
+++ b/include/rgcn_sparse.h
@@ -0,0 +1,19 @@
+#ifndef RGCN_SPARSE_H
+#define RGCN_SPARSE_H
+
+#include "rgcn_hip.h"
+
+#ifdef __cplusplus
+extern "C" {
+#endif
+
+const uint32_t* rgcn_graph_row_mask(const rgcn_graph* g, int transposed, int64_t* num_rows);
+
+int64_t rgcn_occupancy_host(const int32_t* rowptr, int64_t num_rows, int64_t num_relations, uint32_t* words,
+                            int64_t* row_offset);
+
+#ifdef __cplusplus
+}
+#endif
+
+#endif
diff --git a/primekg_rgcn_linkprediction_amd/_lib.py b/primekg_rgcn_linkprediction_amd/_lib.py
--- a/primekg_rgcn_linkprediction_amd/_lib.py
+++ b/primekg_rgcn_linkprediction_amd/_lib.py
@@ -207,6 +207,12 @@
     "rgcn_complex_query": (c_int, [c_int, _P, _P, _I64, _P, _P, _I64, _I64, _I64, _P, _P]),
 }
 
+SPARSE_PROTOTYPES = {
+    "rgcn_graph_row_mask": (c_void_p, [c_void_p, c_int, POINTER(c_int64)]),
+    "rgcn_occupancy_host": (_I64, [_P, _I64, _I64, _P, POINTER(c_int64)]),
+}
+MODE_SPARSE_ROWS = 2
+
 _lib = None
 
 
@@ -227,7 +233,7 @@
         lib = ctypes.CDLL(LIB_PATH, mode=ctypes.RTLD_GLOBAL)
     except OSError as exc:
         raise RGCNLibraryError(f"cannot load {LIB_PATH}: {exc}") from exc
-    for name, (restype, argtypes) in list(PROTOTYPES.items()) + list(SAMPLING_PROTOTYPES.items()) + list(PATHS_PROTOTYPES.items()) + list(CLUSTER_PROTOTYPES.items()) + list(TSNE_PROTOTYPES.items()) + list(NEIGHBORHOOD_PROTOTYPES.items()) + list(TRANSE_PROTOTYPES.items()) + list(RESAMPLE_PROTOTYPES.items()) + list(COMPLEX_PROTOTYPES.items()):
+    for name, (restype, argtypes) in list(PROTOTYPES.items()) + list(SAMPLING_PROTOTYPES.items()) + list(PATHS_PROTOTYPES.items()) + list(CLUSTER_PROTOTYPES.items()) + list(TSNE_PROTOTYPES.items()) + list(NEIGHBORHOOD_PROTOTYPES.items()) + list(TRANSE_PROTOTYPES.items()) + list(RESAMPLE_PROTOTYPES.items()) + list(COMPLEX_PROTOTYPES.items()) + list(SPARSE_PROTOTYPES.items()):
         try:
             fn = getattr(lib, name)
         except AttributeError as exc:
diff --git a/primekg_rgcn_linkprediction_amd/conv.py b/primekg_rgcn_linkprediction_amd/conv.py
--- a/primekg_rgcn_linkprediction_amd/conv.py
+++ b/primekg_rgcn_linkprediction_amd/conv.py
@@ -81,6 +81,16 @@
     r, d_in, d_out = weight.shape
     ratio = _TRANSFORM_FIRST_RATIO if _from_packed(weight, packed, precision) else max(_TRANSFORM_FIRST_RATIO, 4.0)
     return d_out >= ratio * d_in and root is not None and not graph.bipartite
+
+
+_SPARSE_AGG = True
+
+
+def _sparse_agg(graph: "ops.BucketedGraph", transposed: bool, half: bool, packed, amax, d: int, precision=None) -> bool:
+    return bool(_SPARSE_AGG and not half and packed is not None and amax is not None and ops.GEMM_PRECISION == "split"
+                and precision in (None, "half") and d % 64 == 0 and d <= 256 and not graph.bipartite
+                and not graph.weighted_shard and graph.num_relations <= 32
+                and graph.row_mask_ptr(transposed) is not None)
 
 
 def _gagg_scale(graph: "ops.BucketedGraph", gagg_amax: Optional[Tensor], g_amax: Optional[Tensor]):
@@ -114,17 +124,22 @@
             gx = ops.layer_bwd_input_fused(graph, g, packed, relu_mask, g_amax, amax_out=amax_out, tail=tail,
                                            inline_limit=_EVAL_INLINE_LIMIT, out_scale=out_scale, gagg_amax=gagg_amax)
         else:
-            gagg = ops.aggregate(graph, g, transposed=True, tail=tail, amax_out=gagg_amax)
+            sparse = gagg_amax is not None and _sparse_agg(graph, True, False, packed, g_amax, d_out, precision)
+            if sparse:
+                gagg = ops.aggregate_sparse(graph, g, transposed=True, tail=tail, amax_out=gagg_amax)[0]
+            else:
+                gagg = ops.aggregate(graph, g, transposed=True, tail=tail, amax_out=gagg_amax)
             amax, mul = _gagg_scale(graph, gagg_amax, g_amax)
             if (lower is not None and packed is not None and g_amax is not None
                     and _from_packed(lower[0], lower[2], precision) and _transform_first(graph, *lower, precision)
                     and ops.chain_supported(weight, lower[0])):
                 gx, t = ops.transform_bwd_input_chain(gagg, g, weight, root, relu_mask, packed, lower[2], graph=graph,
-                                                      amax=amax, amax_mul=mul, amax_out=amax_out, out_scale=out_scale)
+                                                      amax=amax, amax_mul=mul, amax_out=amax_out, out_scale=out_scale,
+                                                      sparse=sparse)
             else:
                 gx = ops.transform_bwd_input(gagg, g, weight, root, relu_mask=relu_mask, graph=graph, amax=amax,
                                              amax_mul=mul, amax_out=amax_out, packed=packed, precision=precision,
-                                             out_scale=out_scale)
+                                             out_scale=out_scale, sparse=sparse)
     return (gx, t) if lower is not None else gx
 
 
@@ -132,9 +147,11 @@
     return _Scales(g, slots=2 * layers)
 
 
-def _deferred_params(graph: "ops.BucketedGraph", agg, x, g, x_amax, g_amax, has_root: bool, has_bias: bool, prec):
+def _deferred_params(graph: "ops.BucketedGraph", agg, x, g, x_amax, g_amax, has_root: bool, has_bias: bool, prec,
+                     packed=None):
+    sparse = _sparse_agg(graph, False, False, packed, x_amax, x.size(1), prec)
     return ops.transform_bwd_params(agg, x, g, graph.num_relations, want_root=has_root, want_bias=has_bias, graph=graph,
-                                    defer=True, amax=(x_amax, x_amax, g_amax), precision=prec)
+                                    defer=True, amax=(x_amax, x_amax, g_amax), precision=prec, sparse=sparse)
 
 
 _TRAIN_FUSED = _os.environ.get("RGCN_TRAIN_FUSED", "auto")
@@ -163,12 +180,15 @@
         out = ops.layer_fwd_fused(graph, x, packed, bias, relu, x_amax, amax_out, inline_limit=_EVAL_INLINE_LIMIT,
                                   agg_out=agg)
         return agg, out
-    if _defer_hubs(half, packed, x_amax, d_in, d_out):
+    sparse = n == graph.num_other_nodes and _sparse_agg(graph, False, half, packed, x_amax, d_in)
+    if sparse:
+        agg, hubs = ops.aggregate_sparse(graph, x, defer=_defer_hubs(half, packed, x_amax, d_in, d_out))
+    elif _defer_hubs(half, packed, x_amax, d_in, d_out):
         agg, hubs = ops.aggregate_deferred(graph, x)
     else:
         agg, hubs = ops.aggregate(graph, _table(x, gather_dtype)), None
     out = ops.transform_fwd(agg, x, weight, root, bias, relu=relu, graph=graph, half=half, amax=(x_amax, x_amax),
-                            amax_out=amax_out, packed=packed, hubs=hubs)
+                            amax_out=amax_out, packed=packed, hubs=hubs, sparse=sparse)
     return agg, out
 
 
@@ -188,7 +208,8 @@
 def _conv_backward(x, agg, weight, root, x_amax, pkbuf, g, *, graph, has_root, has_bias, need_x, need_p, prec):
     packed = _packs([pkbuf], [(weight, root)])[0]
     scales = _backward_scales(g, 1)
-    pending = _deferred_params(graph, agg, x, g, x_amax, scales.first, has_root, has_bias, prec) if need_p else None
+    pending = (_deferred_params(graph, agg, x, g, x_amax, scales.first, has_root, has_bias, prec, packed)
+               if need_p else None)
     gx = _input_grad(graph, g, weight, root, pending, scales.first, scales, packed, prec) if need_x else None
     if pending is None:
         return gx, None, None, None
@@ -272,12 +293,12 @@
     pk1, pk2 = _packs([pk1buf, pk2buf], [(w1, root1), (w2, root2)])
     scales = _backward_scales(g, 2)
     g_amax, gz_amax = scales.first, scales.slot()
-    red2 = _deferred_params(graph, agg2, h, g, h_amax, g_amax, has_root2, has_b2, prec)
+    red2 = _deferred_params(graph, agg2, h, g, h_amax, g_amax, has_root2, has_b2, prec, pk2)
     gz = _input_grad(graph, g, w2, root2, red2, g_amax, scales, pk2, prec, relu_mask=h,
                      out_scale=1.0 / (1.0 - p) if p > 0 else 1.0, amax_out=gz_amax,
                      lower=(w1, root1, pk1) if need_x else None)
     gz, t_first = gz if need_x else (gz, None)
-    red1 = _deferred_params(graph, agg1, x, gz, x_amax, gz_amax, has_root1, has_b1, prec)
+    red1 = _deferred_params(graph, agg1, x, gz, x_amax, gz_amax, has_root1, has_b1, prec, pk1)
     gx = _input_grad(graph, gz, w1, root1, red1, gz_amax, scales, pk1, prec, t_first) if need_x else None
     red2.finish()
     red1.finish()
@@ -291,7 +312,7 @@
 
 
 def _policy_key():
-    return (_TRAIN_FUSED, _DEFER_HUBS, _TRANSFORM_FIRST_RATIO, _EVAL_INLINE_LIMIT, _TRAIN_FUSED_MIN_BYTES)
+    return (_TRAIN_FUSED, _DEFER_HUBS, _TRANSFORM_FIRST_RATIO, _EVAL_INLINE_LIMIT, _TRAIN_FUSED_MIN_BYTES, _SPARSE_AGG)
 
 
 def _enc2_train_forward(graph, params, gather_dtype, half_backward: bool, hints, p: float = 0.0):
diff --git a/primekg_rgcn_linkprediction_amd/csrc/rgcn_aggregate.hip b/primekg_rgcn_linkprediction_amd/csrc/rgcn_aggregate.hip
--- a/primekg_rgcn_linkprediction_amd/csrc/rgcn_aggregate.hip
+++ b/primekg_rgcn_linkprediction_amd/csrc/rgcn_aggregate.hip
@@ -330,17 +330,19 @@
 template <int G>
 void launch_level(const rgcn_csr* c, int level, bool weighted, const float* x, const float* cnt, float* agg,
                   float* partial, int d, hipStream_t stream, const rgcn_slab_job* tail = nullptr,
-                  unsigned* amax_out = nullptr) {
-  const int64_t nitems = c->num_items[level];
+                  unsigned* amax_out = nullptr, bool sparse = false) {
+  int64_t nitems = c->num_items[level];
   if (nitems == 0) return;
   const unsigned gy = (unsigned)ceil_div64(d, 4 * G);
   if (level == 0) {
     const int64_t slots = kThreads / G;
     const int64_t walked = gy == 1 ? std::min(nitems, ceil_div64(nitems - c->empty_items0, slots) * slots) : nitems;
     const unsigned gather_blocks = (unsigned)ceil_div64(walked, slots);
-    const unsigned zero_blocks = (unsigned)ceil_div64(nitems - walked, zero_rows<G>());
+    if (sparse) nitems -= c->empty_items0;
+    const unsigned zero_blocks = sparse ? 0u : (unsigned)ceil_div64(nitems - walked, zero_rows<G>());
     const rgcn_slab_job job = tail ? *tail : rgcn_slab_job{};
     dim3 grid(gather_blocks + zero_blocks + (tail ? (unsigned)rgcn_slab_reduce_blocks(job) : 0u), gy);
+    if (grid.x == 0) return;
     if (weighted)
       k_aggregate<G, true><<<grid, kThreads, 0, stream>>>(x, c->items[0], nitems, c->col, c->val, cnt, agg, partial, d,
                                                           c->head_col, c->head_w, job, (int)gather_blocks,
@@ -371,7 +373,7 @@
 
 int aggregate_levels(const rgcn_graph* g, int transposed, int first, int last, const float* x, int64_t d,
                      float* agg, void* workspace, size_t workspace_bytes, void* stream_, bool half_in,
-                     const rgcn_slab_job* tail, float* amax) {
+                     const rgcn_slab_job* tail, float* amax, bool sparse) {
   if (!g) return RGCN_ERR_ARG;
   const rgcn_csr* c = &g->dir[transposed ? 1 : 0];
   hipStream_t stream = (hipStream_t)stream_;
@@ -396,6 +398,7 @@
   float* partial = (float*)workspace;
   unsigned* amax_out = reinterpret_cast<unsigned*>(amax);
   if (amax && half_in) return RGCN_ERR_UNSUPPORTED;
+  if (sparse && (half_in || d > 256 || !c->tile_mask)) return RGCN_ERR_UNSUPPORTED;
   RGCN_ALIGN_TRY(16, x, agg, workspace);
   RGCN_ALIGN_TRY(4, amax);
   if (tail) RGCN_ALIGN_TRY(16, tail->slab, tail->bias_part, tail->grad_weight, tail->grad_root, tail->grad_bias);
@@ -421,13 +424,13 @@
       else launch_level0_h<64>(c, weighted, xh, cnt, agg, partial, (int)d, stream);
       continue;
     }
-    if (q <= 1) launch_level<1>(c, l, weighted, x, cnt, agg, partial, (int)d, stream, t0, amax_out);
-    else if (q <= 2) launch_level<2>(c, l, weighted, x, cnt, agg, partial, (int)d, stream, t0, amax_out);
-    else if (q <= 4) launch_level<4>(c, l, weighted, x, cnt, agg, partial, (int)d, stream, t0, amax_out);
-    else if (q <= 8) launch_level<8>(c, l, weighted, x, cnt, agg, partial, (int)d, stream, t0, amax_out);
-    else if (q <= 16) launch_level<16>(c, l, weighted, x, cnt, agg, partial, (int)d, stream, t0, amax_out);
-    else if (q <= 32) launch_level<32>(c, l, weighted, x, cnt, agg, partial, (int)d, stream, t0, amax_out);
-    else launch_level<64>(c, l, weighted, x, cnt, agg, partial, (int)d, stream, t0, amax_out);
+    if (q <= 1) launch_level<1>(c, l, weighted, x, cnt, agg, partial, (int)d, stream, t0, amax_out, sparse);
+    else if (q <= 2) launch_level<2>(c, l, weighted, x, cnt, agg, partial, (int)d, stream, t0, amax_out, sparse);
+    else if (q <= 4) launch_level<4>(c, l, weighted, x, cnt, agg, partial, (int)d, stream, t0, amax_out, sparse);
+    else if (q <= 8) launch_level<8>(c, l, weighted, x, cnt, agg, partial, (int)d, stream, t0, amax_out, sparse);
+    else if (q <= 16) launch_level<16>(c, l, weighted, x, cnt, agg, partial, (int)d, stream, t0, amax_out, sparse);
+    else if (q <= 32) launch_level<32>(c, l, weighted, x, cnt, agg, partial, (int)d, stream, t0, amax_out, sparse);
+    else launch_level<64>(c, l, weighted, x, cnt, agg, partial, (int)d, stream, t0, amax_out, sparse);
   }
   RGCN_HIP_TRY(hipGetLastError());
   return RGCN_OK;
@@ -447,8 +450,8 @@
                       float* amax, void* stream) {
   if (!g) return RGCN_ERR_ARG;
   return aggregate_levels(g, transposed, first_level, last_level < 0 ? g->dir[transposed ? 1 : 0].num_levels : last_level,
-                          reinterpret_cast<const float*>(x), d, agg, workspace, workspace_bytes, stream, x_f16 != 0, job,
-                          amax);
+                          reinterpret_cast<const float*>(x), d, agg, workspace, workspace_bytes, stream, (x_f16 & 1) != 0, job,
+                          amax, (x_f16 & RGCN_MODE_SPARSE_ROWS) != 0);
 }
 
 int rgcn_aggregate(const rgcn_graph* g, int transposed, const float* x, int64_t d, float* agg,
diff --git a/primekg_rgcn_linkprediction_amd/csrc/rgcn_common.h b/primekg_rgcn_linkprediction_amd/csrc/rgcn_common.h
--- a/primekg_rgcn_linkprediction_amd/csrc/rgcn_common.h
+++ b/primekg_rgcn_linkprediction_amd/csrc/rgcn_common.h
@@ -82,6 +82,21 @@
 
 static_assert(offsetof(rgcn_csr, items) == offsetof(rgcn_csr, num_levels) + 8, "empty_items0 sits behind num_levels");
 
+constexpr int64_t RGCN_ROW_MASK_PAD = 96;
+static inline int64_t rgcn_row_mask_offset(int64_t n_key) { return ((n_key + 31) / 32 + 3) / 4 * 4; }
+static inline int64_t rgcn_occupancy_words(int64_t n_key) { return rgcn_row_mask_offset(n_key) + n_key + RGCN_ROW_MASK_PAD; }
+static inline void rgcn_fill_occupancy(const int32_t* rowptr, int64_t n_key, int64_t R, uint32_t* words) {
+  const int64_t off = rgcn_row_mask_offset(n_key), total = rgcn_occupancy_words(n_key);
+  for (int64_t i = 0; i < total; ++i) words[i] = 0u;
+  for (int64_t i = 0; i < n_key; ++i) {
+    uint32_t m = 0u;
+    for (int64_t r = 0; r < R; ++r)
+      if (rowptr[i * R + r + 1] > rowptr[i * R + r]) m |= 1u << r;
+    words[off + i] = m;
+    words[i >> 5] |= m;
+  }
+}
+
 struct rgcn_graph {
   int64_t E = 0, N = 0, R = 0;
   rgcn_csr dir[2];
diff --git a/primekg_rgcn_linkprediction_amd/csrc/rgcn_graph.hip b/primekg_rgcn_linkprediction_amd/csrc/rgcn_graph.hip
--- a/primekg_rgcn_linkprediction_amd/csrc/rgcn_graph.hip
+++ b/primekg_rgcn_linkprediction_amd/csrc/rgcn_graph.hip
@@ -6,6 +6,7 @@
 #include <vector>
 
 #include "rgcn_common.h"
+#include "../../include/rgcn_sparse.h"
 
 namespace {
 
@@ -202,10 +203,8 @@
   RGCN_HIP_TRY(hipStreamSynchronize(stream));
   if (R <= 32 && c->n_key > 0) {
     c->num_row_tiles = ceil_div64(c->n_key, 32);
-    std::vector<uint32_t> mask((size_t)c->num_row_tiles, 0u);
-    for (int64_t i = 0; i < c->n_key; ++i)
-      for (int64_t r = 0; r < R; ++r)
-        if (rp[i * R + r + 1] > rp[i * R + r]) mask[(size_t)(i >> 5)] |= 1u << r;
+    std::vector<uint32_t> mask((size_t)rgcn_occupancy_words(c->n_key));
+    rgcn_fill_occupancy(rp.data(), c->n_key, R, mask.data());
     RGCN_HIP_TRY(hipMalloc((void**)&c->tile_mask, mask.size() * sizeof(uint32_t)));
     RGCN_HIP_TRY(hipMemcpy(c->tile_mask, mask.data(), mask.size() * sizeof(uint32_t), hipMemcpyHostToDevice));
   }
@@ -461,6 +460,27 @@
   return c->tile_mask;
 }
 
+const uint32_t* rgcn_graph_row_mask(const rgcn_graph* g, int transposed, int64_t* num_rows) {
+  if (num_rows) *num_rows = 0;
+  if (!g) return nullptr;
+  const rgcn_csr* c = &g->dir[transposed ? 1 : 0];
+  if (!c->tile_mask) return nullptr;
+  if (num_rows) *num_rows = c->n_key;
+  return c->tile_mask + rgcn_row_mask_offset(c->n_key);
+}
+
+int64_t rgcn_occupancy_host(const int32_t* rowptr, int64_t num_rows, int64_t num_relations, uint32_t* words,
+                            int64_t* row_offset) {
+  if (num_rows < 0 || num_relations <= 0) return -1;
+  if (row_offset) *row_offset = rgcn_row_mask_offset(num_rows);
+  if (num_relations > 32) return 0;
+  if (words) {
+    if (!rowptr) return -1;
+    rgcn_fill_occupancy(rowptr, num_rows, num_relations, words);
+  }
+  return rgcn_occupancy_words(num_rows);
+}
+
 int rgcn_graph_arrays(const rgcn_graph* g, int transposed, const int32_t** rowptr, const int32_t** col,
                       const int64_t** perm, const float** val) {
   if (!g) return RGCN_ERR_ARG;
diff --git a/primekg_rgcn_linkprediction_amd/csrc/rgcn_transform_split.hip b/primekg_rgcn_linkprediction_amd/csrc/rgcn_transform_split.hip
--- a/primekg_rgcn_linkprediction_amd/csrc/rgcn_transform_split.hip
+++ b/primekg_rgcn_linkprediction_amd/csrc/rgcn_transform_split.hip
@@ -138,6 +138,8 @@
   int N2;
 };
 
+__device__ __attribute__((aligned(16))) float g_zero_row[128];
+
 template <int WM, int WN, int TN, int EPI, bool LO, bool CHAIN = false>
 __global__ __launch_bounds__(64 * WM * WN) void k_gemm_nt_split(const float* __restrict__ A1, int K1,
                                                             const float* __restrict__ A2, int K2,
@@ -149,7 +151,8 @@
                                                             const float* __restrict__ mask, float* __restrict__ C,
                                                             int M, int N, const uint32_t* __restrict__ tile_mask,
                                                             int kseg, unsigned* __restrict__ amax_out,
-                                                            const hub_fin fin, float out_scale, const nt_chain chain) {
+                                                            const hub_fin fin, float out_scale, const nt_chain chain,
+                                                            const uint32_t* __restrict__ row_mask) {
   static_assert(!CHAIN || (WM == 2 && WN == 2 && TN == 2 && LO), "the chained product is built for the 64 x 128 tile");
   constexpr int WAVES = WM * WN;
   constexpr int BM = 32 * WM, BN = 32 * TN * WN, NBUF = WM == 2 ? 3 : 4, D = NBUF - 1;
@@ -179,6 +182,16 @@
       if ((t32 + q) * 32 < M) rel_mask |= tile_mask[t32 + q];
     rel_mask = __builtin_amdgcn_readfirstlane(rel_mask);
   }
+  int a_m[A_PW], a_c4[A_PW];
+  unsigned a_rm[A_PW];
+#pragma unroll
+  for (int j = 0; j < A_PW; ++j) {
+    const int row = (wave * A_PW + j) * 8 + (lane >> 3);
+    a_m[j] = min(m0 + row, M - 1);
+    a_c4[j] = ((lane & 7) ^ ((row >> 1) & 7)) * 4;
+    a_rm[j] = row_mask ? row_mask[a_m[j]] : 0xffffffffu;
+  }
+  const float* a_zero = g_zero_row + (lane & 7) * 4;
   int fin_b = 0, fin_e = 0;
   if (WAVES == 4 && fin.ptr) {
     fin_b = fin.ptr[min(m0 >> 5, fin.tiles)];
@@ -212,13 +225,6 @@
 #pragma unroll
     for (int r = 0; r < 16; ++r) acc[b][r] = 0.f;
 
-  int a_m[A_PW], a_c4[A_PW];
-#pragma unroll
-  for (int j = 0; j < A_PW; ++j) {
-    const int row = (wave * A_PW + j) * 8 + (lane >> 3);
-    a_m[j] = min(m0 + row, M - 1);
-    a_c4[j] = ((lane & 7) ^ ((row >> 1) & 7)) * 4;
-  }
   size_t b_off[B_PW];
 #pragma unroll
   for (int j = 0; j < B_PW; ++j) {
@@ -235,9 +241,11 @@
     const bool first = kt < K1;
     const float* abase = first ? A1 + kt : A2 + (kt - K1);
     const int lda = first ? K1 : K2;
+    const bool masked = first && row_mask != nullptr;
+    const unsigned rbit = masked ? 1u << (kt / kseg) : 0u;
 #pragma unroll
     for (int j = 0; j < A_PW; ++j)
-      glds16(abase + ((size_t)a_m[j] * lda + a_c4[j]), sA + (wave * A_PW + j) * 8 * BK * 4);
+      glds16((!masked || (a_rm[j] & rbit)) ? abase + ((size_t)a_m[j] * lda + a_c4[j]) : a_zero, sA + (wave * A_PW + j) * 8 * BK * 4);
 #pragma unroll
     for (int j = 0; j < B_PW; ++j) {
       glds16(Bh + kt + b_off[j], sBh + (wave * B_PW + j) * 16 * BK * 2);
@@ -607,7 +615,8 @@
                                                                amax_ref amax1, float a1_mul, amax_ref amax2, amax_ref gmax,
                                                                float* __restrict__ slab,
                                                                float* __restrict__ bias_part,
-                                                               const uint32_t* __restrict__ tile_mask, int kseg) {
+                                                               const uint32_t* __restrict__ tile_mask, int kseg,
+                                                               const uint32_t* __restrict__ row_mask) {
   constexpr int TKC = TN_TKC, RING = 3, A_FLOATS = 32 * TKC, G_FLOATS = 32 * 128;
   constexpr int SLOT_BYTES = (A_FLOATS + G_FLOATS) * 4;
   constexpr int PLANE = 4 * 128 * 16;
@@ -661,14 +670,30 @@
   const float* a_src = a_first ? A1 + acol : A2 + (acol - K1);
   const int lda = a_first ? K1 : K2;
   const int gcol = min(n0 + d_col, N - 4);
-  auto stage = [&](int mt, int slot) {
+  struct row_words { unsigned w[2 * A_PW]; };
+  const bool a_masked = row_mask != nullptr && a_first;
+  const unsigned a_bit = a_masked ? 1u << (acol / kseg) : 0u;
+  const float* a_zero = g_zero_row + d_col;
+  auto words_of = [&](int mt) {
+    row_words q;
+#pragma unroll
+    for (int i = 0; i < 2 * A_PW; ++i) q.w[i] = 0xffffffffu;
+    if (row_mask) {
+      const uint32_t* p = row_mask + mt + wave * 2 * A_PW;
+#pragma unroll
+      for (int i = 0; i < 2 * A_PW; ++i) q.w[i] = p[i];
+    }
+    return q;
+  };
+  auto stage = [&](int mt, int slot, const row_words& rw) {
     char* sA = lds + slot * SLOT_BYTES;
     char* sG = sA + A_FLOATS * 4;
 #pragma unroll
     for (int j = 0; j < A_PW; ++j) {
       const int r0 = (wave * A_PW + j) * 2;
       const int m = min(mt + r0 + d_row, M - 1);
-      glds16(a_src + (size_t)m * lda, sA + r0 * TKC * 4);
+      const unsigned word = d_row ? rw.w[2 * j + 1] : rw.w[2 * j];
+      glds16((!a_masked || (word & a_bit)) ? a_src + (size_t)m * lda : a_zero, sA + r0 * TKC * 4);
     }
 #pragma unroll
     for (int j = 0; j < G_PW; ++j) {
@@ -679,11 +704,16 @@
   };
 
   int cur = next_mt(mbeg - 32);
-  stage(cur, 0);
+  row_words rw = words_of(cur);
   int nxt = cur < mend ? next_mt(cur) : mend;
-  stage(nxt, 1);
+  stage(cur, 0, rw);
+  rw = words_of(nxt);
   int aft = nxt < mend ? next_mt(nxt) : mend;
-  stage(aft, 2);
+  stage(nxt, 1, rw);
+  rw = words_of(aft);
+  int fut = aft < mend ? next_mt(aft) : mend;
+  stage(aft, 2, rw);
+  rw = words_of(fut);
 
   const bool conv_a = wave < 4;
   const int cp = tid & 63, mg = (tid >> 6) & 3;
@@ -756,8 +786,7 @@
     if (aft < mend) asm volatile("s_waitcnt vmcnt(%0) lgkmcnt(0)" ::"n"(P) : "memory");
     else asm volatile("s_waitcnt vmcnt(0) lgkmcnt(0)" ::: "memory");
     __builtin_amdgcn_s_barrier();
-    const int fut = aft < mend ? next_mt(aft) : mend;
-    if (fut < mend) stage(fut, t % RING);
+    if (fut < mend) stage(fut, t % RING, rw);
     const unsigned pl = kPlanes + (unsigned)((t & 1) * PBUF_BYTES);
     f32x4 qa[2][2], qg[2][2][2];
 #pragma unroll
@@ -797,6 +826,8 @@
     cur = nxt;
     nxt = aft;
     aft = fut;
+    fut = aft < mend ? next_mt(aft) : mend;
+    rw = words_of(fut);
   }
 
   RGCN_STAMP(2);
@@ -906,6 +937,7 @@
   int M = 0, N = 0;
   const uint32_t* tile_mask = nullptr;
   int kseg = 0;
+  const uint32_t* row_mask = nullptr;
   const float *a1_amax = nullptr, *a2_amax = nullptr;
   float a1_mul = 1.f, out_scale = 1.f;
   float* c_amax = nullptr;
@@ -923,7 +955,7 @@
   const dim3 grid((unsigned)ceil_div64(c.M, 64), CHAIN ? 1u : (unsigned)ceil_div64(c.N, 64 * TN));
   k_gemm_nt_split<2, 2, TN, EPI, LO, CHAIN><<<grid, 256, 0, c.stream>>>(
       c.A1, c.K1, c.A2, c.K2, c.Bh, c.Bl, c.b_inv, c.r1, c.a1_mul, c.r2, c.bias, c.mask, c.C, c.M, c.N, c.tile_mask, c.kseg,
-      reinterpret_cast<unsigned*>(c.c_amax), c.fin, c.out_scale, CHAIN ? c.chain : nt_chain{});
+      reinterpret_cast<unsigned*>(c.c_amax), c.fin, c.out_scale, CHAIN ? c.chain : nt_chain{}, c.row_mask);
 }
 
 int launch_nt_split(nt_call c) {
@@ -934,6 +966,7 @@
   const hub_fin& fin = c.fin;
   if (fin.ptr && fin.d != 64 && fin.d != 128 && fin.d != 256) return RGCN_ERR_UNSUPPORTED;
   if (fin.ptr && (!c.a1_amax || fin.d != c.kseg)) return RGCN_ERR_ARG;
+  if (c.row_mask && (!c.a1_amax || c.kseg <= 0 || c.kseg % BK != 0)) return RGCN_ERR_ARG;
   const int K1 = c.K1, K2 = c.K2;
   if (K1 % BK || K2 % BK || K1 + K2 <= 0) return RGCN_ERR_UNSUPPORTED;
   const bool scan1 = K1 && !c.a1_amax, scan2 = K2 && !c.a2_amax;
@@ -1143,7 +1176,7 @@
                              float* hub_partial) {
   if (rgcn_layer_bad_dims(N, R, d_in, d_out) || !out) return RGCN_ERR_ARG;
   if (N == 0) return RGCN_OK;
-  if (!agg || !x || !weight) return RGCN_ERR_ARG;
+  if (!agg || !x || !weight || ((half & RGCN_MODE_SPARSE_ROWS) && !tile_mask)) return RGCN_ERR_ARG;
   if (d_in % BK) return RGCN_ERR_UNSUPPORTED;
   if (rgcn_gemm_out_of_range(N, (R + 1) * d_in, d_out)) return RGCN_ERR_UNSUPPORTED;
   nt_call c;
@@ -1153,11 +1186,12 @@
                             hub_transposed, hub_partial, stream_, aligned);
   if (rc != RGCN_OK) return rc;
   c.A1 = agg; c.a1_amax = agg_amax; c.a1_mul = agg_amax_mul; c.tile_mask = tile_mask;
+  if (half & RGCN_MODE_SPARSE_ROWS) c.row_mask = tile_mask + rgcn_row_mask_offset(N);
   c.A2 = x; c.a2_amax = x_amax;
   c.Bh = v.Bh_f; c.Bl = v.Bl_f; c.b_inv = v.inv_scale;
   c.bias = bias; c.epi = relu ? EPI_RELU : EPI_NONE;
   c.C = out; c.N = (int)d_out; c.c_amax = out_amax;
-  c.half = half != 0;
+  c.half = (half & 1) != 0;
   return launch_nt_split(c);
 }
 
@@ -1170,7 +1204,7 @@
                                    float out_scale) {
   if (rgcn_layer_bad_dims(N, R, d_in, d_out) || !grad_x || !(out_scale > 0.f)) return RGCN_ERR_ARG;
   if (N == 0) return RGCN_OK;
-  if (!gagg || !g || !weight) return RGCN_ERR_ARG;
+  if (!gagg || !g || !weight || ((half & RGCN_MODE_SPARSE_ROWS) && !tile_mask)) return RGCN_ERR_ARG;
   if (d_out % BK) return RGCN_ERR_UNSUPPORTED;
   if (rgcn_gemm_out_of_range(N, (R + 1) * d_out, d_in)) return RGCN_ERR_UNSUPPORTED;
   nt_call c;
@@ -1180,11 +1214,12 @@
                             hub_transposed, hub_partial, stream_, aligned);
   if (rc != RGCN_OK) return rc;
   c.A1 = gagg; c.a1_amax = gagg_amax; c.a1_mul = gagg_amax_mul; c.tile_mask = tile_mask;
+  if (half & RGCN_MODE_SPARSE_ROWS) c.row_mask = tile_mask + rgcn_row_mask_offset(N);
   c.A2 = g; c.a2_amax = g_amax;
   c.Bh = v.Bh_b; c.Bl = v.Bl_b; c.b_inv = v.inv_scale;
   c.mask = relu_mask; c.epi = relu_mask ? EPI_MASK : EPI_NONE;
   c.C = grad_x; c.N = (int)d_in; c.c_amax = grad_x_amax; c.out_scale = out_scale;
-  c.half = half != 0;
+  c.half = (half & 1) != 0;
   return launch_nt_split(c);
 }
 
@@ -1206,6 +1241,9 @@
   if (!rgcn_transform_bwd_input_chain_supported(R, d_in, d_out, R1, d_in1)) return RGCN_ERR_UNSUPPORTED;
   if (N == 0) return RGCN_OK;
   if (!gagg || !g || !weight || !gagg_amax || !g_amax) return RGCN_ERR_ARG;
+  const bool sparse = (has_root1 & RGCN_MODE_SPARSE_ROWS) != 0;
+  has_root1 &= 1;
+  if (sparse && !tile_mask) return RGCN_ERR_ARG;
   if (rgcn_gemm_out_of_range(N, (R + 1) * d_out, (R1 + 1) * d_in1)) return RGCN_ERR_UNSUPPORTED;
   nt_call c;
   PackedWeights v;
@@ -1216,6 +1254,7 @@
   if (rc != RGCN_OK) return rc;
   const PackedWeights v1 = packed_view(const_cast<void*>(packed1), R1, d_in1, d_in);
   c.A1 = gagg; c.a1_amax = gagg_amax; c.a1_mul = gagg_amax_mul; c.tile_mask = tile_mask;
+  if (sparse) c.row_mask = tile_mask + rgcn_row_mask_offset(N);
   c.A2 = g; c.a2_amax = g_amax;
   c.Bh = v.Bh_b; c.Bl = v.Bl_b; c.b_inv = v.inv_scale;
   c.mask = relu_mask; c.epi = relu_mask ? EPI_MASK : EPI_NONE;
@@ -1263,6 +1302,7 @@
                                           rgcn_slab_job* job) {
   const int rc = rgcn_params_begin_check(job, agg, x, g, N, R, d_in, d_out, grad_weight, 64);
   if (rc != RGCN_OK) return rc;
+  if ((half & RGCN_MODE_SPARSE_ROWS) && (!tile_mask || !agg_amax)) return RGCN_ERR_ARG;
   rgcn_tn_split p = rgcn_tn_plan(N, (R + 1) * d_in, d_out, TN_TKC, kTnBlocks);
   const rgcn_slab_layout lay = rgcn_slab_layout_of(p, (R + 1) * d_in, d_out);
   if (!workspace || workspace_bytes < tn_workspace_bytes(lay)) return RGCN_ERR_WORKSPACE;
@@ -1288,10 +1328,11 @@
   dim3 grid((unsigned)(p.kc_tiles * p.n_tiles), (unsigned)p.splits);
   const uint32_t* tmask = (d_in % 64 == 0) ? tile_mask : nullptr;
   float* bp = grad_bias ? bias_part : nullptr;
+  const uint32_t* rmask = (half & RGCN_MODE_SPARSE_ROWS) ? tile_mask + rgcn_row_mask_offset(N) : nullptr;
 #define RGCN_TN_LAUNCH(KERNEL, LO_)                                                                              \
   KERNEL<LO_><<<grid, 2 * kThreads, 0, stream>>>(agg, K1, x, K2, g, (int)N, (int)d_out, p.n_tiles, p.rows_per_split, \
-                                                 r1, a1_mul, r2, rg, slab, bp, tmask, (int)d_in)
-  if (half) RGCN_TN_LAUNCH(k_gemm_tn_coop, false);
+                                                 r1, a1_mul, r2, rg, slab, bp, tmask, (int)d_in, rmask)
+  if (half & 1) RGCN_TN_LAUNCH(k_gemm_tn_coop, false);
   else RGCN_TN_LAUNCH(k_gemm_tn_coop, true);
 #undef RGCN_TN_LAUNCH
   RGCN_HIP_TRY(hipGetLastError());
diff --git a/primekg_rgcn_linkprediction_amd/ops.py b/primekg_rgcn_linkprediction_amd/ops.py
--- a/primekg_rgcn_linkprediction_amd/ops.py
+++ b/primekg_rgcn_linkprediction_amd/ops.py
@@ -456,6 +456,15 @@
             cache[transposed] = _L().rgcn_graph_tile_mask(handle, int(transposed), None) or None
         return cache[transposed]
 
+    def row_mask_ptr(self, transposed: bool) -> Optional[int]:
+        if self.bipartite and transposed:
+            raise ValueError("a shard structure has one direction only (transposed=False)")
+        handle = self.handle
+        cache = self.__dict__.setdefault("_row_mask_ptrs", {})
+        if transposed not in cache:
+            cache[transposed] = _L().rgcn_graph_row_mask(handle, int(transposed), None) or None
+        return cache[transposed]
+
     def workspace_bytes(self, transposed: bool, d: int) -> int:
         handle = self.handle
         cache = self.__dict__.setdefault("_ws_bytes", {})
@@ -696,8 +705,10 @@
 
 
 def _gather(graph: BucketedGraph, x: torch.Tensor, transposed: bool, tail: Optional[PendingParamGrads],
-            amax_out: Optional[torch.Tensor], out: Optional[torch.Tensor], levels=(0, -1)):
+            amax_out: Optional[torch.Tensor], out: Optional[torch.Tensor], levels=(0, -1), sparse: bool = False):
     half_in = isinstance(x, torch.Tensor) and x.dtype == torch.float16
+    if sparse and (half_in or graph.row_mask_ptr(transposed) is None or x.dim() != 2 or x.size(1) > 256):
+        raise ValueError("a sparse aggregate needs an fp32 table of rows up to 256 wide and a structure of <= 32 relations")
     _need_gpu("x", x, torch.float16 if half_in else torch.float32)
     if graph.bipartite and transposed:
         raise ValueError("a shard structure has one direction only (transposed=False)")
@@ -730,7 +741,8 @@
             if measure and first == 0:
                 beg, end = torch.cuda.Event(enable_timing=True), torch.cuda.Event(enable_timing=True)
                 beg.record()
-            rc = rc or lib.rgcn_aggregate_ex(graph.handle, int(transposed), _ptr(x), int(half_in), d, _ptr(out), _ptr(ws),
+            rc = rc or lib.rgcn_aggregate_ex(graph.handle, int(transposed), _ptr(x),
+                                             int(half_in) | (_lib.MODE_SPARSE_ROWS if sparse else 0), d, _ptr(out), _ptr(ws),
                                              nbytes, first, last, ctypes.byref(job) if job is not None else None,
                                              _ptr(amax_out), _stream())
             if measure and first == 0:
@@ -748,6 +760,18 @@
               tail: Optional[PendingParamGrads] = None, amax_out: Optional[torch.Tensor] = None,
               out: Optional[torch.Tensor] = None) -> torch.Tensor:
     return _gather(graph, x, transposed, tail, amax_out, out)[0]
+
+
+def aggregate_sparse(graph: BucketedGraph, x: torch.Tensor, transposed: bool = False,
+                     tail: Optional[PendingParamGrads] = None, amax_out: Optional[torch.Tensor] = None,
+                     out: Optional[torch.Tensor] = None, defer: bool = False):
+    if defer:
+        d = x.size(1) if x.dim() == 2 else 0
+        if (x.dtype == torch.float32 and GATHER_EVENTS is None and graph.num_levels(transposed) == 2
+                and graph.deferrable(transposed, d)):
+            agg, ws = _gather(graph, x, transposed, tail, amax_out, out, levels=(0, 1), sparse=True)
+            return agg, DeferredHubs(graph, transposed, ws)
+    return _gather(graph, x, transposed, tail, amax_out, out, sparse=True)[0], None
 
 
 def fused_bwd_supported(num_relations: int, d_in: int, d_out: int) -> bool:
@@ -924,11 +948,21 @@
     return graph.tile_mask_ptr(transposed and not graph.bipartite)
 
 
+def _sparse_bit(sparse: bool, graph: Optional[BucketedGraph], transposed: bool, split, amax) -> int:
+    if not sparse:
+        return 0
+    if not split or graph is None or graph.bipartite or graph.row_mask_ptr(transposed) is None or amax is None:
+        raise ValueError("a sparse aggregate needs the split-precision transform, the graph it was gathered over "
+                         "(<= 32 relations, not a shard) and the operand's amax buffer (it cannot be scanned)")
+    return _lib.MODE_SPARSE_ROWS
+
+
 def transform_fwd(agg, x, weight, root=None, bias=None, relu: bool = False,
                   graph: Optional[BucketedGraph] = None, half: bool = False, amax=None,
                   amax_out: Optional[torch.Tensor] = None, precision: Optional[str] = None,
                   packed: Optional[SplitWeights] = None, amax_mul: float = 1.0,
-                  out: Optional[torch.Tensor] = None, hubs: Optional[DeferredHubs] = None) -> torch.Tensor:
+                  out: Optional[torch.Tensor] = None, hubs: Optional[DeferredHubs] = None,
+                  sparse: bool = False) -> torch.Tensor:
     n, r, d_in, d_out = _check_layer(agg, x, weight, root, bias)
     lib = _L()
     _check_amax("amax_out", amax_out, x.device)
@@ -947,6 +981,7 @@
             raise ValueError("packed does not belong to these weights")
     elif hubs is not None:
         raise ValueError("deferred hub tails need the split-precision transform (finish them with aggregate instead)")
+    mode = _sparse_bit(sparse, graph, False, split, _pair(amax, 2)[0] if split else None)
     k = (r + (root is not None)) * d_in
     with _on(x.device):
         if out is None:
@@ -959,7 +994,7 @@
                 rc = lib.rgcn_transform_fwd_split(_ptr(agg), _ptr(x), _ptr(weight), _ptr(root),
                                                   _ptr(packed.buf) if packed is not None else None, _ptr(bias),
                                                   int(relu), _mask_for(graph, False, n, r), n, r, d_in, d_out,
-                                                  _ptr(a1), float(amax_mul), _ptr(a2), int(split == 2), _ptr(out),
+                                                  _ptr(a1), float(amax_mul), _ptr(a2), int(split == 2) | mode, _ptr(out),
                                                   _ptr(amax_out), _ptr(ws), nbytes, _stream(), *_hub_args(hubs, n, r))
         elif half and d_in % 32 == 0:
             name = "rgcn_transform_fwd_f16"
@@ -984,13 +1019,14 @@
                         graph: Optional[BucketedGraph] = None, amax=None, amax_out: Optional[torch.Tensor] = None,
                         precision: Optional[str] = None, packed: Optional[SplitWeights] = None,
                         amax_mul: float = 1.0, hubs: Optional[DeferredHubs] = None,
-                        out_scale: float = 1.0) -> torch.Tensor:
+                        out_scale: float = 1.0, sparse: bool = False) -> torch.Tensor:
     n, r, d_in, d_out = _check_bwd_input(gagg, g, weight, root, relu_mask)
     lib = _L()
     _check_amax("amax_out", amax_out, g.device)
     if d_in % 4 or d_out % 4:
         raise ValueError("in/out channels must be multiples of 4")
     split = _use_split(precision, d_out, 32)
+    mode = _sparse_bit(sparse, graph, True, split and n > 0, _pair(amax, 2)[0])
     if split and n > 0:
         a1, a2 = _pair(amax, 2)
         _check_amax("gagg_amax", a1, g.device)
@@ -1005,8 +1041,8 @@
                 rc = lib.rgcn_transform_bwd_input_split(_ptr(gagg), _ptr(g), _ptr(weight), _ptr(root),
                                                         _ptr(packed.buf) if packed is not None else None,
                                                         _ptr(relu_mask), _mask_for(graph, True, n, r), n, r, d_in,
-                                                        d_out, _ptr(a1), float(amax_mul), _ptr(a2), int(split == 2),
-                                                        _ptr(gx), _ptr(amax_out), _ptr(ws), nbytes, _stream(),
+                                                        d_out, _ptr(a1), float(amax_mul), _ptr(a2),
+                                                        int(split == 2) | mode, _ptr(gx), _ptr(amax_out), _ptr(ws), nbytes, _stream(),
                                                         *_hub_args(hubs, n, r), float(out_scale))
         _lib.check(rc, "rgcn_transform_bwd_input_split")
         return gx
@@ -1035,7 +1071,8 @@
 
 def transform_bwd_input_chain(gagg, g, weight, root, relu_mask, packed: SplitWeights, packed1: SplitWeights,
                               graph: Optional[BucketedGraph] = None, amax=None, amax_out: Optional[torch.Tensor] = None,
-                              amax_mul: float = 1.0, hubs: Optional[DeferredHubs] = None, out_scale: float = 1.0):
+                              amax_mul: float = 1.0, hubs: Optional[DeferredHubs] = None, out_scale: float = 1.0,
+                              sparse: bool = False):
     n, r, d_in, d_out = _check_bwd_input(gagg, g, weight, root, relu_mask)
     r1, d_in1, _ = packed1.shape
     if not packed.matches(weight, root) or packed1.shape[2] != d_in:
@@ -1046,6 +1083,7 @@
     _check_amax("amax_out", amax_out, g.device)
     if a1 is None or a2 is None:
         raise ValueError("the chained transform needs the operand maxima (amax=)")
+    mode = _sparse_bit(sparse, graph, True, True, a1)
     lib = _L()
     cols = (r1 + (1 if packed1.has_root else 0)) * d_in1
     with _on(g.device):
@@ -1058,7 +1096,7 @@
                                                           _ptr(relu_mask), _mask_for(graph, True, n, r), n, r, d_in, d_out,
                                                           _ptr(a1), float(amax_mul), _ptr(a2), _ptr(gz), _ptr(amax_out), _ptr(ws),
                                                           nbytes, _stream(), *_hub_args(hubs, n, r), float(out_scale),
-                                                          _ptr(packed1.buf), int(packed1.has_root), r1, d_in1, _ptr(t))
+                                                          _ptr(packed1.buf), int(packed1.has_root) | mode, r1, d_in1, _ptr(t))
     _lib.check(rc, "rgcn_transform_bwd_input_chain_split")
     return gz, t
 
@@ -1087,7 +1125,7 @@
 
 def transform_bwd_params(agg, x, g, num_relations: int, want_root: bool = True, want_bias: bool = True,
                          graph: Optional[BucketedGraph] = None, defer: bool = False, amax=None,
-                         precision: Optional[str] = None, amax_mul: float = 1.0):
+                         precision: Optional[str] = None, amax_mul: float = 1.0, sparse: bool = False):
     _need_gpu("x", x, torch.float32)
     _need_gpu("agg", agg, torch.float32)
     _need_gpu("g", g, torch.float32)
@@ -1102,6 +1140,7 @@
         groot = _empty(d_in, d_out, dtype=torch.float32, device=x.device) if want_root else None
         gbias = _empty(d_out, dtype=torch.float32, device=x.device) if want_bias else None
         split = _use_split(precision, d_in, 64)
+        mode = _sparse_bit(sparse, graph, False, split and n > 0, _pair(amax, 3)[0])
         if split and n > 0:
             a1, a2, a3 = _pair(amax, 3)
             for nm, t in (("agg_amax", a1), ("x_amax", a2), ("g_amax", a3)):
@@ -1113,7 +1152,7 @@
                 rc = lib.rgcn_transform_bwd_params_split_begin(_ptr(agg), _ptr(x), _ptr(g),
                                                                _mask_for(graph, False, n, r), n, r, d_in, d_out,
                                                                _ptr(a1), float(amax_mul), _ptr(a2), _ptr(a3),
-                                                               int(split == 2), _ptr(gw), _ptr(groot),
+                                                               int(split == 2) | mode, _ptr(gw), _ptr(groot),
                                                                _ptr(gbias), _ptr(ws), nbytes, _stream(),
                                                                ctypes.byref(job))
             _lib.check(rc, "rgcn_transform_bwd_params_split_begin")
@@ -2759,7 +2798,7 @@
 
 
 _SEQ_INDEX = {name: i for i, name in enumerate(_lib.SEQ_FUNCTIONS)}
-_SEQ_PURE = ("rgcn_graph_tile_mask", "rgcn_graph_num_levels", "rgcn_graph_weight_bound", "rgcn_aggregate_deferrable",
+_SEQ_PURE = ("rgcn_graph_tile_mask", "rgcn_graph_row_mask", "rgcn_graph_num_levels", "rgcn_graph_weight_bound", "rgcn_aggregate_deferrable",
              "rgcn_graph_num_edges", "rgcn_graph_num_nodes", "rgcn_graph_num_relations", "rgcn_abi_version", "rgcn_strerror")
 REGIONS = True
 
```

Result: faster. 7.017 billion edges/s, median of 6 (+4.7%).
